# lppllppl920/EndoscopyDepthEstimation-Pytorch

Hardware: AMD Instinct MI355X
Metric: train frame-pairs/sec at 256x320 bs=8 (higher is better)
Workload: dtype f32

## Files before the change

### endoscopydepthestimation-pytorch_amd/csrc/conv_dma_kernels.h

```cpp
#pragma once

#include "conv_kernels.h"

namespace endo {

static __device__ __attribute__((aligned(16))) float g_pad_consts[8] = {__builtin_nanf(""), __builtin_nanf(""), __builtin_nanf(""), __builtin_nanf(""),
                                                                  0.0f, 0.0f, 0.0f, 0.0f};

typedef const __attribute__((address_space(1))) void* gptr_t;
typedef __attribute__((address_space(3))) void* lptr_t;

template <int KS, int KC, int Q, int WX, int R, int NBUF, int VEC, int IN = IN_PLAIN>
struct ConvDmaSmem {
    using G = ConvGeom<KS, KC, WX, R, VEC>;
    static constexpr int kW = KS * KS * KC * 16 * Q;
    static constexpr int kUG = (G::kTileX / 2) * (G::kTileY / 2);
    static constexpr int kUI = kUG / 4;
    static constexpr int kUStride = ((kUG + kUI - 8 + 31) / 32) * 32 + 8;
    static constexpr int kChan = (IN == IN_UNPOOL) ? kUStride : G::kCS;
    static constexpr int kBuf = KC * kChan + kW;
    static constexpr int kTail = 4 * 16 * Q + 8 * 16 * Q;
    static size_t bytes(int bn_cap) { return sizeof(float) * (NBUF * kBuf + 3 * bn_cap + kTail); }
};

template <int KS, int KC, int Q, int IN, int EPI, int WX, int R, int NBUF, int MINW, int VEC, int XF, int EXP = 0, int PH = -1, int BF = 0>
__global__ void __launch_bounds__(kConvThreads, MINW) conv_dma_kernel(const ConvParams p0) {
    static_assert(BF == 0 || (PH < 0 && (KS == 3 || KS == 1) && (IN == IN_BNRELU || IN == IN_PLAIN || (IN == IN_UNPOOL && KS == 1))),
                  "bf16 operands: the ordinary 3x3 convolution and the 1x1 convolutions of the transition-down layers");
    static_assert(PH < 0 || (KS == 3 && (Q % 2) == 0 && IN == IN_PLAIN && EPI == EPI_FWD), "phase mode is the transition-up forward");
    static_assert(IN != IN_UNPOOL || (KS == 1 && R % 2 == 0), "UNPOOL is the transition-down data gradient (1x1)");
    static_assert(NBUF == 1 || NBUF == 2, "one or two LDS buffers");
    static_assert(VEC == 1 || (VEC == 4 && IN != IN_UPSAMPLE && IN != IN_UNPOOL && IN != IN_SUBPIX), "16-byte DMA needs contiguous sources");
    static_assert(IN != IN_SUBPIX || (KS == 3 && EPI == EPI_FWD && PH < 0), "sub-pixel input mode is the transition-up data gradient");
    using G = ConvGeom<KS, KC, WX, R, VEC>;
    using S = ConvDmaSmem<KS, KC, Q, WX, R, NBUF, VEC, IN>;
    constexpr int KK = KS * KS;
    constexpr int NB = 16 * Q;
    constexpr int kWElems = S::kW;
    constexpr int kWPre = (kWElems + kConvThreads - 1) / kConvThreads;
    constexpr bool kDgrad = (EPI == EPI_DGRAD_BN || EPI == EPI_DGRAD_SUMPOOL);
    constexpr int kPhW = 2 * 12 * 16 + 16;
    static_assert(PH < 0 || KC * kPhW <= kWElems, "the phase weights fit the ordinary weight buffer");
    constexpr int kSubW = 4 * 16 * Q + 16;

    extern __shared__ __attribute__((aligned(16))) float smem[];
    float* s_aux = smem + NBUF * S::kBuf;
    int grp, n;
    group_of(p0, blockIdx.z, grp, n);
    const ConvParams p = group_view(p0, grp);
    const int groups = p0.group_n > 0 ? gridDim.z / p0.group_n : 1;
    const bool first_of_group = blockIdx.x == 0 && blockIdx.y == 0 && n == 0;
    (void)groups; (void)first_of_group;
    const int cap = p.bn_cap;

    const int tid = threadIdx.x;
    const int lane = tid & 63;
    const int wave = __builtin_amdgcn_readfirstlane(tid >> 6);
    const int tile = (gridDim.x & 7) == 0 ? xcd_remap(blockIdx.x, gridDim.x) : blockIdx.x;
    const int x0 = (tile % p.tiles_x) * G::kTileX;
    const int y0 = (tile / p.tiles_x) * G::kTileY;
    const int ph = PH == 2 ? static_cast<int>(blockIdx.y) : PH;
    const int co_base = (p.ksplit > 0 || PH == 2) ? 0 : blockIdx.y * NB;

    if constexpr (IN == IN_BNRELU) {
        for (int c = tid; c < p.cin; c += kConvThreads) {
            float scale, mean, beta;
            bn_input_constants(p, p0, grp, groups, first_of_group, c, scale, mean, beta);
            s_aux[c] = scale;
            s_aux[cap + c] = mean;
            s_aux[2 * cap + c] = beta;
        }
        for (int c = p.cin + tid; c < ((p.cin + KC - 1) / KC) * KC; c += kConvThreads) {
            s_aux[c] = 0.f; s_aux[cap + c] = 0.f; s_aux[2 * cap + c] = 0.f;
        }
    }
    if constexpr (EPI == EPI_DGRAD_BN) {
        float* cst = s_aux + 3 * cap;
        if (tid < NB) {
            const int c = co_base + tid;
            float mean = 0.f, rstd = 0.f, scale = 0.f, beta = 0.f;
            if (c < p.cout) {
                mean = p.bn_saved[2 * c];
                rstd = p.bn_saved[2 * c + 1];
                scale = p.bn_gamma[c] * rstd;
                beta = p.bn_beta[c];
            }
            cst[4 * tid] = scale; cst[4 * tid + 1] = beta; cst[4 * tid + 2] = mean; cst[4 * tid + 3] = rstd;
        }
    }

    f32x4 acc[R][Q];
#pragma unroll
    for (int r = 0; r < R; ++r)
#pragma unroll
        for (int q = 0; q < Q; ++q) acc[r][q] = f32x4{0.f, 0.f, 0.f, 0.f};

    const int wx = (wave % WX) * 16;
    const int wy = (wave / WX) * R;
    const int li = lane & 15;
    const int lk = lane >> 4;

    int goff[G::kPos];
    unsigned pos_ok = 0;
#pragma unroll
    for (int k = 0; k < G::kPos; ++k) {
        const int e = tid + k * kConvThreads;
        goff[k] = 0;
        if (e < G::kUnits) {
            const int ry = e / (G::kCols / VEC);
            const int rx = (e - ry * (G::kCols / VEC)) * VEC;
            const int gy = y0 - G::kHalo + ry;
            const int gx = x0 - G::kLeft + rx;
            if (gy >= 0 && gy < p.h && gx >= 0 && gx < p.w) {
                pos_ok |= (1u << k);
                if constexpr (IN == IN_UPSAMPLE) goff[k] = (gy >> 1) * p.in_w + (gx >> 1);
                else if constexpr (IN == IN_SUBPIX) goff[k] = 2 * gy * p.in_w + 2 * gx;
                else goff[k] = gy * p.in_w + gx;
            }
        }
    }
    constexpr int kUSlots = (IN == IN_UNPOOL) ? (KC * S::kUStride + kConvThreads - 1) / kConvThreads : 1;
    int uoff[kUSlots];
    if constexpr (IN == IN_UNPOOL) {
        constexpr int PC = G::kTileX / 2;
        const int ph = p.h >> 1, pw = p.w >> 1;
#pragma unroll
        for (int k = 0; k < kUSlots; ++k) {
            const int e = tid + k * kConvThreads;
            const int u = e % S::kUStride;
            int off = -1;
            if (e < KC * S::kUStride) {
                if (u < S::kUG) {
                    const int gy = (y0 >> 1) + u / PC, gx = (x0 >> 1) + u % PC;
                    if (gy < ph && gx < pw) off = gy * p.in_w + gx;
                } else if (u < S::kUG + S::kUI) {
                    const int q = u - S::kUG;
                    const int gy = (y0 >> 1) + q / (PC / 4), gx = (x0 >> 1) + 4 * (q % (PC / 4));
                    if (gy < ph && gx < pw) off = gy * p.in_w + gx;
                }
            }
            uoff[k] = off;
        }
    }
    const float* in_n = p.in + n * p.in_ns;
    const float* pad_in = g_pad_consts + (IN == IN_BNRELU ? 0 : 4);
    const float* pad_zero = g_pad_consts + 4;
    const int nchunks_all = (p.cin + KC - 1) / KC;
    int chunk_begin = 0, nchunks = nchunks_all;
    ConvParams po = p;
    if (p.ksplit > 0) {
        const int per = (nchunks_all + p.ksplit - 1) / p.ksplit;
        chunk_begin = blockIdx.y * per;
        nchunks = min(nchunks_all, chunk_begin + per);
        po.out = p.out + blockIdx.y * p.split_stride;
    }

    auto issue_dma = [&](int chunk, int buf) {
        const int c_base = chunk * KC;
        float* s_in = smem + buf * S::kBuf;
        float* s_w = s_in + KC * S::kChan;
        if constexpr (IN == IN_UNPOOL) {
            const uint8_t* idx_n = p.in_idx + n * p.idx_ns;
#pragma unroll
            for (int k = 0; k < kUSlots; ++k) {
                const int e0 = k * kConvThreads + wave * 64;
                if (e0 < KC * S::kUStride) {
                    const int e = e0 + lane;
                    const int ch = c_base + e / S::kUStride;
                    const bool is_code = (e % S::kUStride) >= S::kUG;
                    const void* src = pad_zero;
                    if (uoff[k] >= 0 && ch < p.cin) {
                        const int64_t o = static_cast<int64_t>(ch) * p.in_cs + uoff[k];
                        src = is_code ? static_cast<const void*>(idx_n + o) : static_cast<const void*>(in_n + o);
                    }
                    if (e < KC * S::kUStride) __builtin_amdgcn_global_load_lds((gptr_t)src, (lptr_t)(s_in + e0), 4, 0, 0);
                }
            }
        }
        int sub_ph = 0;
        if constexpr (IN == IN_SUBPIX) sub_ph = c_base / p.sub_c;
#pragma unroll
        for (int c = 0; c < (IN == IN_UNPOOL ? 0 : KC); ++c) {
            const int ch = c_base + c;
            const float* plane = in_n + static_cast<int64_t>(ch) * p.in_cs;
            if constexpr (IN == IN_SUBPIX)
                plane = in_n + static_cast<int64_t>(ch - sub_ph * p.sub_c) * p.in_cs + (sub_ph >> 1) * p.in_w + (sub_ph & 1);
#pragma unroll
            for (int k = 0; k < G::kPos; ++k) {
                const int e0 = k * kConvThreads + wave * 64;
                if (e0 < G::kUnits) {
                    const bool ok = (ch < p.cin) && (pos_ok & (1u << k));
                    const float* src = ok ? plane + goff[k] : pad_in;
                    if (e0 + lane < G::kUnits) {
                        if constexpr (VEC == 4)
                            __builtin_amdgcn_global_load_lds((gptr_t)src, (lptr_t)(s_in + c * G::kCS + 4 * e0), 16, 0, 0);
                        else
                            __builtin_amdgcn_global_load_lds((gptr_t)src, (lptr_t)(s_in + c * G::kCS + e0), 4, 0, 0);
                    }
                }
            }
        }
        if constexpr (IN == IN_SUBPIX) {
            constexpr int kUnitsW = KC * kSubW / 4;
            const float* wsrc = p.wgt + static_cast<int64_t>(c_base) * kSubW;
#pragma unroll
            for (int k = 0; k < (kUnitsW + kConvThreads - 1) / kConvThreads; ++k) {
                const int u0 = k * kConvThreads + wave * 64;
                if (u0 < kUnitsW && u0 + lane < kUnitsW)
                    __builtin_amdgcn_global_load_lds((gptr_t)(wsrc + 4 * (u0 + lane)), (lptr_t)(s_w + 4 * u0), 16, 0, 0);
            }
        }
        if constexpr (PH >= 0) {
            constexpr int kUnitsW = KC * kPhW / 4;
            const float* wsrc = p.wgt + static_cast<int64_t>(c_base) * kPhW + (PH == 2 ? static_cast<int64_t>(ph) * p.cin * 400 : 0);
#pragma unroll
            for (int k = 0; k < (kUnitsW + kConvThreads - 1) / kConvThreads; ++k) {
                const int u0 = k * kConvThreads + wave * 64;
                if (u0 < kUnitsW && u0 + lane < kUnitsW)
                    __builtin_amdgcn_global_load_lds((gptr_t)(wsrc + 4 * (u0 + lane)), (lptr_t)(s_w + 4 * u0), 16, 0, 0);
            }
        }
        constexpr bool kChunked = KS == 3 && KC == 16 && Q == 1 && EPI == EPI_FWD && PH < 0 && IN != IN_SUBPIX && BF == 0;
        bool gather = !(PH >= 0 || IN == IN_SUBPIX);
        if constexpr (kChunked) {
            if (p.wgt_chunks) {
                gather = false;
                constexpr int kUnitsW = kWElems / 4;
                const float* wsrc = p.wgt_chunks + static_cast<int64_t>(chunk) * kWElems;
#pragma unroll
                for (int k = 0; k < (kUnitsW + kConvThreads - 1) / kConvThreads; ++k) {
                    const int u0 = k * kConvThreads + wave * 64;
                    if (u0 < kUnitsW && u0 + lane < kUnitsW)
                        __builtin_amdgcn_global_load_lds((gptr_t)(wsrc + 4 * (u0 + lane)), (lptr_t)(s_w + 4 * u0), 16, 0, 0);
                }
            }
        }
        if (gather)
#pragma unroll
        for (int k = 0; k < ((PH >= 0 || IN == IN_SUBPIX) ? 0 : kWPre); ++k) {
            const int e0 = k * kConvThreads + wave * 64;
            if (e0 < kWElems) {
                const int e = e0 + lane;
                const int j = e % NB;
                const int rest = e / NB;
                const int c = rest % KC;
                const int tap = rest / KC;
                const int ci = c_base + c;
                const int co = co_base + j;
                const float* src = pad_zero;
                if (e < kWElems && ci < p.cin && co < (PH >= 0 ? p.w_cout : p.cout)) {
                    if constexpr (kDgrad) src = p.wgt + (static_cast<int64_t>(ci) * p.w_cin + co) * KK + (KK - 1 - tap);
                    else src = p.wgt + (static_cast<int64_t>(co) * p.w_cin + ci) * KK + tap;
                }
                if (e < kWElems) __builtin_amdgcn_global_load_lds((gptr_t)src, (lptr_t)(s_w + e0), 4, 0, 0);
            }
        }
    };

    constexpr int PR = (EPI == EPI_DGRAD_BN) ? R : 1, PQ = (EPI == EPI_DGRAD_BN) ? Q : 1;
    f32x4 xpre[PR][PQ], dpre[PR][PQ];
    bool use_pre = false;
    if constexpr (EPI == EPI_DGRAD_BN) {
        use_pre = ((p.out_w & 3) == 0) && ((p.w & 3) == 0);
        if (use_pre) {
            const int px = x0 + wx + 4 * lk;
#pragma unroll
            for (int q = 0; q < Q; ++q) {
                const int co = co_base + q * 16 + li;
#pragma unroll
                for (int r = 0; r < R; ++r) {
                    const int y = y0 + wy + r;
                    xpre[r][q] = f32x4{0.f, 0.f, 0.f, 0.f};
                    dpre[r][q] = f32x4{0.f, 0.f, 0.f, 0.f};
                    if (co < p.cout && y < p.h && px + 3 < p.w) {
                        xpre[r][q] = *reinterpret_cast<const f32x4*>(p.x + n * p.x_ns + static_cast<int64_t>(co) * p.x_cs + y * p.out_w + px);
                        if (co >= p.acc_from)
                            dpre[r][q] = *reinterpret_cast<const f32x4*>(p.out + n * p.out_ns + static_cast<int64_t>(co) * p.out_cs + y * p.out_w + px);
                    }
                }
            }
        }
    }

    constexpr bool kInPlace = (IN == IN_BNRELU) && (XF == 1);
    auto transform_own = [&](int chunk, int buf) {
        if constexpr (kInPlace) {
            float* s_in = smem + buf * S::kBuf;
#pragma unroll
            for (int c = 0; c < KC; ++c) {
                const int ch = chunk * KC + c;
                const float sc = s_aux[ch], mn = s_aux[cap + ch], bt = s_aux[2 * cap + ch];
#pragma unroll
                for (int k = 0; k < G::kPos; ++k) {
                    const int e = tid + k * kConvThreads;
                    if (e < G::kUnits) {
                        if constexpr (VEC == 4) {
                            f32x4* q = reinterpret_cast<f32x4*>(s_in + c * G::kCS + 4 * e);
                            f32x4 v = *q;
#pragma unroll
                            for (int i = 0; i < 4; ++i) v[i] = __builtin_fmaxf(fmaf(v[i] - mn, sc, bt), 0.f);
                            *q = v;
                        } else {
                            float* q = s_in + c * G::kCS + e;
                            *q = __builtin_fmaxf(fmaf(*q - mn, sc, bt), 0.f);
                        }
                    }
                }
            }
        }
    };

    auto compute = [&](int chunk, int buf) {
        const float* s_in = smem + buf * S::kBuf;
        const float* s_w = s_in + KC * S::kChan;
        int sub_alpha = 0, sub_beta = 0;
        if constexpr (IN == IN_SUBPIX) {
            const int sub_ph = (chunk * KC) / p.sub_c;
            sub_alpha = sub_ph >> 1; sub_beta = sub_ph & 1;
        }
        (void)sub_alpha; (void)sub_beta;
        if constexpr (IN == IN_UNPOOL) {
            constexpr int PC = G::kTileX / 2;
            const int pcol = (wx + li) >> 1;
            const unsigned sh = 8u * (pcol & 3);
            const unsigned want = li & 1;
            if constexpr (BF != 0) {
                constexpr int NQ = KC / 4;
#pragma unroll
                for (int qg = 0; qg < (NQ + 3) / 4; ++qg) {
                    float a[4][R], b[4][Q];
#pragma unroll
                    for (int i = 0; i < 4; ++i) {
                        const int quad = qg * 4 + i;
                        if (quad < NQ) {
                            const float* g_base = s_in + (quad * 4 + lk) * S::kUStride + (wy >> 1) * PC + pcol;
                            const unsigned* i_base = reinterpret_cast<const unsigned*>(s_in + (quad * 4 + lk) * S::kUStride + S::kUG);
                            const float* b_base = s_w + (quad * 4 + lk) * NB + li;
#pragma unroll
                            for (int rr = 0; rr < R / 2; ++rr) {
                                const float g = g_base[rr * PC];
                                const unsigned code = (i_base[(((wy >> 1) + rr) * PC + pcol) >> 2] >> sh) & 0xffu;
                                a[i][2 * rr] = code == want ? g : 0.f;
                                a[i][2 * rr + 1] = code == want + 2u ? g : 0.f;
                            }
#pragma unroll
                            for (int q = 0; q < Q; ++q) b[i][q] = b_base[q * 16];
                        } else {
#pragma unroll
                            for (int r = 0; r < R; ++r) a[i][r] = 0.f;
#pragma unroll
                            for (int q = 0; q < Q; ++q) b[i][q] = 0.f;
                        }
                    }
                    bf16x4_bits ap[R];
#pragma unroll
                    for (int r = 0; r < R; ++r) ap[r] = pack_bf16x4(a[0][r], a[1][r], a[2][r], a[3][r]);
#pragma unroll
                    for (int q = 0; q < Q; ++q) {
                        const bf16x4_bits bp = pack_bf16x4(b[0][q], b[1][q], b[2][q], b[3][q]);
#pragma unroll
                        for (int r = 0; r < R; ++r) acc[r][q] = __builtin_amdgcn_mfma_f32_16x16x16bf16_1k(ap[r], bp, acc[r][q], 0, 0, 0);
                    }
                }
                return;
            }
#pragma unroll
            for (int quad = 0; quad < KC / 4; ++quad) {
                const float* g_base = s_in + (quad * 4 + lk) * S::kUStride + (wy >> 1) * PC + pcol;
                const unsigned* i_base = reinterpret_cast<const unsigned*>(s_in + (quad * 4 + lk) * S::kUStride + S::kUG);
                const float* b_base = s_w + (quad * 4 + lk) * NB + li;
                float a[R];
#pragma unroll
                for (int rr = 0; rr < R / 2; ++rr) {
                    const float g = g_base[rr * PC];
                    const unsigned code = (i_base[(((wy >> 1) + rr) * PC + pcol) >> 2] >> sh) & 0xffu;
                    a[2 * rr] = code == want ? g : 0.f;
                    a[2 * rr + 1] = code == want + 2u ? g : 0.f;
                }
#pragma unroll
                for (int q = 0; q < Q; ++q) {
                    const float b = b_base[q * 16];
#pragma unroll
                    for (int r = 0; r < R; ++r) acc[r][q] = __builtin_amdgcn_mfma_f32_16x16x4f32(a[r], b, acc[r][q], 0, 0, 0);
                }
            }
            return;
        }
        if constexpr (BF != 0 && KS == 1) {
            constexpr int NQ = KC / 4;
#pragma unroll
            for (int qg = 0; qg < (NQ + 3) / 4; ++qg) {
                float a[4][R], b[4][Q];
#pragma unroll
                for (int i = 0; i < 4; ++i) {
                    const int quad = qg * 4 + i;
                    if (quad < NQ) {
                        const float* a_base = s_in + (quad * 4 + lk) * G::kCS + wy * G::kCols + wx + li + G::kColOff;
                        const float* b_base = s_w + (quad * 4 + lk) * NB + li;
                        float sc = 1.f, mn = 0.f, bt = 0.f;
                        if constexpr (IN == IN_BNRELU && !kInPlace) {
                            const int ch = chunk * KC + quad * 4 + lk;
                            sc = s_aux[ch]; mn = s_aux[cap + ch]; bt = s_aux[2 * cap + ch];
                        }
#pragma unroll
                        for (int r = 0; r < R; ++r) {
// ... 67 lines not shown
#pragma unroll
                    for (int r = 0; r < R + KS - 1; ++r) a[r] = a_base[r * G::kCols + dx];
                }
                if constexpr (IN == IN_SUBPIX) {
                    if (dx == (sub_beta == 0 ? 0 : 2)) continue;
                }
#pragma unroll
                for (int dy = 0; dy < KS; ++dy) {
                    if (PH >= 0 && dy == (ph == 0 ? 2 : 0)) continue;
                    if constexpr (IN == IN_SUBPIX) {
                        if (dy == (sub_alpha == 0 ? 0 : 2)) continue;
                    }
#pragma unroll
                    for (int q = 0; q < Q; ++q) {
                        if (PH >= 0 && ((q < Q / 2 && dx == 2) || (q >= Q / 2 && dx == 0))) continue;
                        float b;
                        if constexpr (IN == IN_SUBPIX) {
                            const int tyi = dy - (sub_alpha == 0 ? 1 : 0), txi = dx - (sub_beta == 0 ? 1 : 0);
                            b = s_w[(quad * 4 + lk) * kSubW + (tyi * 2 + txi) * NB + q * 16 + li];
                        } else if constexpr (PH >= 0) {
                            const int slot = dx == 0 ? q : (dx == 1 ? Q / 2 + q : Q / 2 + Q + (q - Q / 2));
                            b = s_w[(quad * 4 + lk) * kPhW + ((dy - ph) * 2 * Q + slot) * 16 + li];
                        } else {
                            b = b_base[(dy * KS + dx) * KC * NB + q * 16];
                        }
#pragma unroll
                        for (int r = 0; r < R; ++r)
                            acc[r][q] = __builtin_amdgcn_mfma_f32_16x16x4f32(a[r + dy], b, acc[r][q], 0, 0, 0);
                    }
                }
            }
        }
    };

    issue_dma(chunk_begin, 0);
    if constexpr (kInPlace) {
        __syncthreads();
        asm volatile("s_waitcnt vmcnt(0)" ::: "memory");
        transform_own(chunk_begin, 0);
        __syncthreads();
        for (int chunk = chunk_begin; chunk < nchunks; ++chunk) {
            const int b = (chunk - chunk_begin) & 1;
            if (chunk + 1 < nchunks) issue_dma(chunk + 1, b ^ 1);
            compute(chunk, b);
            if (chunk + 1 < nchunks) {
                asm volatile("s_waitcnt vmcnt(0)" ::: "memory");
                transform_own(chunk + 1, b ^ 1);
            }
            __syncthreads();
        }
    } else {
        for (int chunk = chunk_begin; chunk < nchunks; ++chunk) {
            const int b = (chunk - chunk_begin) % NBUF;
            if (!(EXP & 4) || chunk == chunk_begin) asm volatile("s_waitcnt vmcnt(0)" ::: "memory");
            __syncthreads();
            if (NBUF == 2 && chunk + 1 < nchunks && !(EXP & 1)) issue_dma(chunk + 1, b ^ 1);
            compute(chunk, b);
            if (NBUF == 1 && chunk + 1 < nchunks) {
                __syncthreads();
                issue_dma(chunk + 1, 0);
            }
        }
    }

    if constexpr (EPI == EPI_DGRAD_BN) {
        if (use_pre) {
            const float* cst = s_aux + 3 * cap;
            float* s_red = s_aux + 3 * cap + 4 * NB;
            const int px = x0 + wx + 4 * lk;
#pragma unroll
            for (int q = 0; q < Q; ++q) {
                const int jloc = q * 16 + li;
                const int co = co_base + jloc;
                const float scale = cst[4 * jloc], beta = cst[4 * jloc + 1], mean = cst[4 * jloc + 2], rstd = cst[4 * jloc + 3];
                float s1 = 0.f, s2 = 0.f;
#pragma unroll
                for (int r = 0; r < R; ++r) {
                    const int y = y0 + wy + r;
                    if (co < p.cout && y < p.h && px + 3 < p.w) {
                        f32x4 o = dpre[r][q];
#pragma unroll
                        for (int e = 0; e < 4; ++e) {
                            const float xc = xpre[r][q][e] - mean;
                            const float z = fmaf(xc, scale, beta);
                            const float dz = z > 0.f ? acc[r][q][e] : 0.f;
                            s1 += dz;
                            s2 += dz * (xc * rstd);
                            o[e] += scale * dz;
                        }
                        *reinterpret_cast<f32x4*>(p.out + n * p.out_ns + static_cast<int64_t>(co) * p.out_cs + y * p.out_w + px) = o;
                    }
                }
                s1 += __shfl_xor(s1, 16, 64); s1 += __shfl_xor(s1, 32, 64);
                s2 += __shfl_xor(s2, 16, 64); s2 += __shfl_xor(s2, 32, 64);
                if (lk == 0) {
                    s_red[((tid >> 6) * NB + jloc) * 2] = s1;
                    s_red[((tid >> 6) * NB + jloc) * 2 + 1] = s2;
                }
            }
            __syncthreads();
            if (tid < 2 * NB) {
                const int j = tid >> 1, which = tid & 1;
                if (co_base + j < p.cout) {
                    double t = 0.0;
                    for (int wv = 0; wv < 4; ++wv) t += static_cast<double>(s_red[(wv * NB + j) * 2 + which]);
                    atomicAdd(p.bn_scratch + bn_slot_offset(p.bn_slot_stride) + 2 * (co_base + j) + which, t);
                }
            }
            return;
        }
    }
    if constexpr (PH >= 0) {
        constexpr int QH = Q / 2;
        float* s_red = s_aux + 3 * cap + 4 * NB;
        const int px = x0 + wx + 4 * lk;
#pragma unroll
        for (int q = 0; q < QH; ++q) {
            const int co = q * 16 + li;
            const bool co_ok = co < p.cout;
            const float bias = (co_ok && p.bias) ? p.bias[co] : 0.f;
            float s1 = 0.f, s2 = 0.f;
#pragma unroll
            for (int r = 0; r < R; ++r) {
                const int y = y0 + wy + r;
                if (co_ok && y < p.h && px + 3 < p.w) {
                    f32x4 lo, hi;
                    lo[0] = acc[r][q][0] + bias; lo[1] = acc[r][q + QH][0] + bias; lo[2] = acc[r][q][1] + bias; lo[3] = acc[r][q + QH][1] + bias;
                    hi[0] = acc[r][q][2] + bias; hi[1] = acc[r][q + QH][2] + bias; hi[2] = acc[r][q][3] + bias; hi[3] = acc[r][q + QH][3] + bias;
                    float* dst = p.out + n * p.out_ns + static_cast<int64_t>(co) * p.out_cs + static_cast<int64_t>(2 * y + ph) * p.out_w + 2 * px;
                    *reinterpret_cast<f32x4*>(dst) = lo;
                    *reinterpret_cast<f32x4*>(dst + 4) = hi;
#pragma unroll
                    for (int e = 0; e < 4; ++e) { s1 += lo[e] + hi[e]; s2 += lo[e] * lo[e] + hi[e] * hi[e]; }
                }
            }
            s1 += __shfl_xor(s1, 16, 64); s1 += __shfl_xor(s1, 32, 64);
            s2 += __shfl_xor(s2, 16, 64); s2 += __shfl_xor(s2, 32, 64);
            if (lk == 0) {
                s_red[((tid >> 6) * NB + q * 16 + li) * 2] = s1;
                s_red[((tid >> 6) * NB + q * 16 + li) * 2 + 1] = s2;
            }
        }
        __syncthreads();
        if (p.out_sums && tid < 2 * 16 * QH) {
            const int j = tid >> 1, which = tid & 1;
            if (j < p.cout) {
                double t = 0.0;
                for (int wv = 0; wv < 4; ++wv) t += static_cast<double>(s_red[(wv * NB + j) * 2 + which]);
                atomicAdd(p.out_sums + 2 * j + which, t);
            }
        }
        return;
    }
    conv_epilogue<Q, EPI, R>(po, acc, s_aux + 3 * cap, s_aux + 3 * cap + 4 * NB, x0, y0, wx, wy, co_base, n);
}

template <int KS, int KC, int Q, int IN, int EPI, int WX, int R, int NBUF, int MINW, int VEC, int XF = 0, int EXP = 0, int PH = -1, int BF = 0>
inline int launch_conv_dma_vec(ConvParams p, hipStream_t stream) {
    static_assert(XF == 0 || NBUF == 2 || IN != IN_BNRELU, "the in-place transform pipeline is written for two buffers");
    using G = ConvGeom<KS, KC, WX, R, VEC>;
    using S = ConvDmaSmem<KS, KC, Q, WX, R, NBUF, VEC, IN>;
    p.tiles_x = (p.w + G::kTileX - 1) / G::kTileX;
    p.bn_cap = (IN == IN_BNRELU) ? ((p.cin + KC - 1) / KC * KC + 15) / 16 * 16 : 0;
    const int tiles_y = (p.h + G::kTileY - 1) / G::kTileY;
    dim3 grid(p.tiles_x * tiles_y, p.ksplit > 0 ? p.ksplit : (PH >= 0 ? (PH == 2 ? 2 : 1) : (p.cout + 16 * Q - 1) / (16 * Q)), p.n);
    return launch_dyn(conv_dma_kernel<KS, KC, Q, IN, EPI, WX, R, NBUF, MINW, VEC, XF, EXP, PH, BF>, grid, kConvThreads, S::bytes(p.bn_cap), stream, p);
}

template <int KS, int KC, int Q, int IN, int EPI, int WX, int R, int NBUF, int MINW = 1, int BF = 0>
inline int launch_conv_dma(const ConvParams& p, hipStream_t stream) {
    if constexpr (IN != IN_UPSAMPLE && IN != IN_UNPOOL) {
        const bool aligned = (p.w % 4 == 0) && (p.in_w % 4 == 0) && (p.in_cs % 4 == 0) && (p.in_ns % 4 == 0) &&
                             (reinterpret_cast<uintptr_t>(p.in) % 16 == 0);
        if (aligned) return launch_conv_dma_vec<KS, KC, Q, IN, EPI, WX, R, NBUF, MINW, 4, 0, 0, -1, BF>(p, stream);
    }
    return launch_conv_dma_vec<KS, KC, Q, IN, EPI, WX, R, NBUF, MINW, 1, 0, 0, -1, BF>(p, stream);
}

template <int KS, int KC, int Q, int IN, int EPI, int BIG_R = 8, int NBUF = 2, int BIG_MINW = 1, int BF = 0>
inline int launch_conv_dma_auto(const ConvParams& p, hipStream_t stream) {
    const long tiles_big = static_cast<long>((p.w + 31) / 32) * ((p.h + 15) / 16) * p.n;
    if (tiles_big >= 512) return launch_conv_dma<KS, KC, Q, IN, EPI, 2, BIG_R, NBUF, BIG_MINW, BF>(p, stream);
    const long tiles_mid = static_cast<long>((p.w + 15) / 16) * ((p.h + 15) / 16) * p.n;
    if (tiles_mid >= 384) return launch_conv_dma<KS, KC, Q, IN, EPI, 1, 4, NBUF, 1, BF>(p, stream);
    constexpr int KCS = (NBUF == 2 && KS == 3 && KC <= 8) ? 16 : KC;
    return launch_conv_dma<KS, KCS, Q, IN, EPI, 1, 2, NBUF, 1, BF>(p, stream);
}

}
```

### endoscopydepthestimation-pytorch_amd/csrc/conv_kernels.h

```cpp
#pragma once

#include "common.h"

namespace endo {

enum InMode { IN_PLAIN = 0, IN_BNRELU = 1, IN_UPSAMPLE = 2, IN_UNPOOL = 3, IN_SUBPIX = 4 };
enum Epilogue { EPI_FWD = 0, EPI_FWD_POOL = 1, EPI_DGRAD_BN = 2, EPI_DGRAD_SUMPOOL = 3 };

constexpr int kConvThreads = 256;
constexpr int kMaxBnChannels = 384;

struct ConvParams {
    int n, h, w;
    int tiles_x;
    const float* in;
    int64_t in_ns;
    int in_cs;
    int in_w;
    const uint8_t* in_idx;
    int64_t idx_ns;
    int cin;
    const double* in_sums;
    const float* gamma;
    const float* beta;
    float* running_mean;
    float* running_var;
    float* saved;
    double count;
    float eps, momentum;
    int training;
    const float* wgt;
    const float* bias;
    int w_cout, w_cin;
    const float* wgt_chunks;
    float* out;
    int64_t out_ns;
    int out_cs, out_w;
    int cout;
    uint8_t* out_idx;
    double* out_sums;
    const float* x;
    int64_t x_ns;
    int x_cs;
    const float* bn_saved;
    const float* bn_gamma;
    const float* bn_beta;
    double* bn_scratch;
    int64_t bn_slot_stride;
    int acc_from;
    int bn_cap;
    int ksplit;
    int64_t split_stride;
    int group_n;
    int64_t gs, in_gs, out_gs;
    int sub_c;
    const float* fin_w;
    float* fin_out;
};

__device__ __forceinline__ void group_of(const ConvParams& p, int z, int& grp, int& n) {
    grp = p.group_n > 0 ? z / p.group_n : 0;
    n = z - grp * p.group_n;
}

__device__ __forceinline__ ConvParams group_view(const ConvParams& p, int grp) {
    ConvParams q = p;
    const int64_t o = grp * p.gs;
    q.in += grp * p.in_gs;
    q.out += grp * p.out_gs;
    if (q.x) q.x += o;
    if (q.in_idx) q.in_idx += 4 * o;
    if (q.out_idx) q.out_idx += 4 * o;
    if (q.in_sums) q.in_sums += o / 2;
    if (q.out_sums) q.out_sums += o / 2;
    if (q.bn_scratch) q.bn_scratch += o / 2;
    if (q.saved) q.saved += o;
    if (q.bn_saved) q.bn_saved += o;
    return q;
}

__device__ __forceinline__ void bn_input_constants(const ConvParams& p, const ConvParams& p0, int grp, int groups, bool first_of_group,
                                                   int c, float& scale, float& mean_f, float& beta) {
    double mean, var;
    if (p.training) {
        mean = p.in_sums[2 * c] / p.count;
        var = p.in_sums[2 * c + 1] / p.count - mean * mean;
        if (var < 0.0) var = 0.0;
    } else {
        mean = p.running_mean[c];
        var = p.running_var[c];
    }
    const double rstd = 1.0 / sqrt(var + static_cast<double>(p.eps));
    scale = p.gamma[c] * static_cast<float>(rstd);
    mean_f = static_cast<float>(mean);
    beta = p.beta[c];
    if (first_of_group) {
        if (p.saved) {
            p.saved[2 * c] = static_cast<float>(mean);
            p.saved[2 * c + 1] = static_cast<float>(rstd);
        }
        if (p.training && grp == 0) {
            float rm = p.running_mean[c], rv = p.running_var[c];
            for (int g = 0; g < groups; ++g) {
                const double* sums = p0.in_sums + g * (p0.gs / 2);
                const double m = sums[2 * c] / p.count;
                double v = sums[2 * c + 1] / p.count - m * m;
                if (v < 0.0) v = 0.0;
                const double unbiased = p.count > 1.0 ? v * p.count / (p.count - 1.0) : v;
                rm = (1.0f - p.momentum) * rm + p.momentum * static_cast<float>(m);
                rv = (1.0f - p.momentum) * rv + p.momentum * static_cast<float>(unbiased);
            }
            p.running_mean[c] = rm;
            p.running_var[c] = rv;
        }
    }
}

typedef float f32x4 __attribute__((ext_vector_type(4)));

template <int KS, int KC, int WX, int R, int VEC = 1>
struct ConvGeom {
    static constexpr int kTileX = 16 * WX;
    static constexpr int kTileY = R * (4 / WX);
    static constexpr int kHalo = KS / 2;
    static constexpr int kRows = kTileY + 2 * kHalo;
    static constexpr int kLeft = (VEC == 4 && KS == 3) ? 4 : kHalo;
    static constexpr int kCols = kTileX + 2 * kLeft;
    static constexpr int kColOff = kLeft - kHalo;
    static constexpr int kPlane = kRows * kCols;
    static constexpr int kCS = ((kPlane - 16 + 31) / 32) * 32 + 16;
    static constexpr int kUnits = kPlane / VEC;
    static constexpr int kPos = (kUnits + kConvThreads - 1) / kConvThreads;
    static constexpr int kPre = KC * kPos;
};

template <int Q, int EPI, int R>
__device__ __forceinline__ void conv_epilogue(const ConvParams& p, f32x4 (&acc)[R][Q], const float* cst, float* s_red,
                                              int x0, int y0, int wx, int wy, int co_base, int n) {
    constexpr int NB = 16 * Q;
    const int tid = threadIdx.x;
    const int lane = tid & 63;
    const int wave = tid >> 6;
    const int li = lane & 15;
    const int lk = lane >> 4;
    (void)cst; (void)s_red; (void)wave;
    const int px = x0 + wx + 4 * lk;
    const bool vec_ok = ((p.out_w & 3) == 0) && ((p.w & 3) == 0);

    if constexpr (EPI == EPI_FWD) {
#pragma unroll
        for (int q = 0; q < Q; ++q) {
            const int co = co_base + q * 16 + li;
            const bool co_ok = co < p.cout;
            const float bias = (co_ok && p.bias) ? p.bias[co] : 0.f;
            float s1 = 0.f, s2 = 0.f;
#pragma unroll
            for (int r = 0; r < R; ++r) {
                const int y = y0 + wy + r;
                f32x4 v = acc[r][q];
                v[0] += bias; v[1] += bias; v[2] += bias; v[3] += bias;
                if (co_ok && y < p.h) {
                    float* dst = p.out + n * p.out_ns + static_cast<int64_t>(co) * p.out_cs + y * p.out_w + px;
                    if (vec_ok && px + 3 < p.w) {
                        *reinterpret_cast<f32x4*>(dst) = v;
#pragma unroll
                        for (int e = 0; e < 4; ++e) { s1 += v[e]; s2 += v[e] * v[e]; }
                    } else {
#pragma unroll
                        for (int e = 0; e < 4; ++e)
                            if (px + e < p.w) { dst[e] = v[e]; s1 += v[e]; s2 += v[e] * v[e]; }
                    }
                }
            }
            if (p.out_sums) {
                s1 += __shfl_xor(s1, 16, 64); s1 += __shfl_xor(s1, 32, 64);
                s2 += __shfl_xor(s2, 16, 64); s2 += __shfl_xor(s2, 32, 64);
                if (lk == 0) {
                    s_red[(wave * NB + q * 16 + li) * 2] = s1;
                    s_red[(wave * NB + q * 16 + li) * 2 + 1] = s2;
                }
            }
        }
        if (p.out_sums) {
            __syncthreads();
            if (tid < 2 * NB) {
                const int j = tid >> 1, which = tid & 1;
                if (co_base + j < p.cout) {
                    double t = 0.0;
                    for (int wv = 0; wv < 4; ++wv) t += static_cast<double>(s_red[(wv * NB + j) * 2 + which]);
                    atomicAdd(p.out_sums + 2 * (co_base + j) + which, t);
                }
            }
        }
    } else if constexpr (EPI == EPI_FWD_POOL) {
        const int ph = p.h >> 1, pw = p.w >> 1;
#pragma unroll
        for (int q = 0; q < Q; ++q) {
            const int co = co_base + q * 16 + li;
            const bool co_ok = co < p.cout;
            const float bias = (co_ok && p.bias) ? p.bias[co] : 0.f;
            float s1 = 0.f, s2 = 0.f;
#pragma unroll
            for (int r = 0; r < R; r += 2) {
                const int yp = (y0 + wy + r) >> 1;
#pragma unroll
                for (int e = 0; e < 4; e += 2) {
                    const int xp = (px + e) >> 1;
                    float best = acc[r][q][e] + bias;
                    int code = 0;
                    float v = acc[r][q][e + 1] + bias;
                    if (v > best) { best = v; code = 1; }
                    v = acc[r + 1][q][e] + bias;
                    if (v > best) { best = v; code = 2; }
                    v = acc[r + 1][q][e + 1] + bias;
                    if (v > best) { best = v; code = 3; }
                    if (co_ok && yp < ph && xp < pw) {
                        const int64_t o = static_cast<int64_t>(co) * p.out_cs + yp * p.out_w + xp;
                        p.out[n * p.out_ns + o] = best;
                        p.out_idx[n * p.idx_ns + o] = static_cast<uint8_t>(code);
                        s1 += best; s2 += best * best;
                    }
                }
            }
            s1 += __shfl_xor(s1, 16, 64); s1 += __shfl_xor(s1, 32, 64);
            s2 += __shfl_xor(s2, 16, 64); s2 += __shfl_xor(s2, 32, 64);
            if (lk == 0) {
                s_red[(wave * NB + q * 16 + li) * 2] = s1;
                s_red[(wave * NB + q * 16 + li) * 2 + 1] = s2;
            }
        }
        __syncthreads();
        if (p.out_sums && tid < 2 * NB) {
            const int j = tid >> 1, which = tid & 1;
            if (co_base + j < p.cout) {
                double t = 0.0;
                for (int wv = 0; wv < 4; ++wv) t += static_cast<double>(s_red[(wv * NB + j) * 2 + which]);
                atomicAdd(p.out_sums + 2 * (co_base + j) + which, t);
            }
        }
    } else if constexpr (EPI == EPI_DGRAD_BN) {
#pragma unroll
        for (int q = 0; q < Q; ++q) {
            const int jloc = q * 16 + li;
            const int co = co_base + jloc;
            const bool co_ok = co < p.cout;
            const float scale = cst[4 * jloc], beta = cst[4 * jloc + 1], mean = cst[4 * jloc + 2], rstd = cst[4 * jloc + 3];
            const bool accumulate = co >= p.acc_from;
            float s1 = 0.f, s2 = 0.f;
#pragma unroll
            for (int r = 0; r < R; ++r) {
                const int y = y0 + wy + r;
                if (co_ok && y < p.h) {
                    const int64_t xo = n * p.x_ns + static_cast<int64_t>(co) * p.x_cs + y * p.out_w + px;
                    float* dst = p.out + n * p.out_ns + static_cast<int64_t>(co) * p.out_cs + y * p.out_w + px;
                    if (vec_ok && px + 3 < p.w) {
                        const f32x4 xv = *reinterpret_cast<const f32x4*>(p.x + xo);
                        f32x4 o = accumulate ? *reinterpret_cast<const f32x4*>(dst) : f32x4{0.f, 0.f, 0.f, 0.f};
#pragma unroll
                        for (int e = 0; e < 4; ++e) {
                            const float xc = xv[e] - mean;
                            const float z = fmaf(xc, scale, beta);
                            const float dz = z > 0.f ? acc[r][q][e] : 0.f;
                            s1 += dz;
                            s2 += dz * (xc * rstd);
                            o[e] += scale * dz;
                        }
                        *reinterpret_cast<f32x4*>(dst) = o;
                    } else {
#pragma unroll
                        for (int e = 0; e < 4; ++e) {
                            if (px + e < p.w) {
                                const float xv = p.x[xo + e];
                                const float xc = xv - mean;
                                const float z = fmaf(xc, scale, beta);
                                const float dz = z > 0.f ? acc[r][q][e] : 0.f;
                                s1 += dz;
                                s2 += dz * (xc * rstd);
                                dst[e] = (accumulate ? dst[e] : 0.f) + scale * dz;
                            }
                        }
                    }
                }
            }
            s1 += __shfl_xor(s1, 16, 64); s1 += __shfl_xor(s1, 32, 64);
            s2 += __shfl_xor(s2, 16, 64); s2 += __shfl_xor(s2, 32, 64);
            if (lk == 0) {
                s_red[(wave * NB + jloc) * 2] = s1;
                s_red[(wave * NB + jloc) * 2 + 1] = s2;
            }
        }
        __syncthreads();
        if (tid < 2 * NB) {
            const int j = tid >> 1, which = tid & 1;
            if (co_base + j < p.cout) {
                double t = 0.0;
                for (int wv = 0; wv < 4; ++wv) t += static_cast<double>(s_red[(wv * NB + j) * 2 + which]);
                atomicAdd(p.bn_scratch + bn_slot_offset(p.bn_slot_stride) + 2 * (co_base + j) + which, t);
            }
        }
    } else {
        const int ph = p.h >> 1, pw = p.w >> 1;
#pragma unroll
        for (int q = 0; q < Q; ++q) {
            const int co = co_base + q * 16 + li;
            if (co >= p.cout) continue;
#pragma unroll
            for (int r = 0; r < R; r += 2) {
                const int yp = (y0 + wy + r) >> 1;
#pragma unroll
                for (int e = 0; e < 4; e += 2) {
                    const int xp = (px + e) >> 1;
                    if (yp < ph && xp < pw) {
                        const float v = (acc[r][q][e] + acc[r][q][e + 1]) + (acc[r + 1][q][e] + acc[r + 1][q][e + 1]);
                        p.out[n * p.out_ns + static_cast<int64_t>(co) * p.out_cs + yp * p.out_w + xp] = v;
                    }
// ... 235 lines not shown
```

### endoscopydepthestimation-pytorch_amd/csrc/net.hip

```cpp
#include <new>
#include <vector>

#include "dgrad_kernels.h"
#include "dgrad_block_kernels.h"
#include "dgrad_newmap_kernels.h"
#include "td_dgrad_kernels.h"
#include "td_fwd_kernels.h"
#include "wgrad_taps_kernels.h"
#include "wgrad1x1_kernels.h"
#include "wgrad_nsplit_kernels.h"
#include "wgrad_x3_kernels.h"
#include "wgrad_f34_kernels.h"
#include "wgrad_subpix_kernels.h"
#include "wino_fwd_kernels.h"
#include "wino4_fwd_kernels.h"
#include "dgrad_wino_kernels.h"
#include "dgrad_wino3_kernels.h"

#include <cstdlib>

namespace endo {

int run_dgrad_wino3_nl4(const DgradBlockParams& p, const float* const* u, hipStream_t stream);
bool dgrad_wino3p_applies(const DgradBlockParams& p);
int run_dgrad_wino3p_nl4(const DgradBlockParams& p, const float* const* u, int blocks, double* fw_parts, int* blocks_used, hipStream_t stream);

constexpr int kGrowth = 12;
constexpr int kLayers = 4;
constexpr int kFirst = 48;
constexpr int kLevels = 5;
constexpr int kNew = kGrowth * kLayers;
constexpr float kBnEps = 1.0e-5f;
constexpr float kBnMomentum = 0.1f;
constexpr int kSideStreamFromLevel = 0;

struct ConvP { int64_t w, b; int cout, cin, ks; int64_t u; int64_t ud; };
struct BnP { int64_t g, b; int c; int64_t run; int64_t saved; };

struct Table {
    ConvP first, final_;
    ConvP down_conv[kLevels][kLayers], td_conv[kLevels], bott_conv[kLayers], tu_conv[kLevels], up_conv[kLevels][kLayers];
    BnP down_bn[kLevels][kLayers], td_bn[kLevels], bott_bn[kLayers], up_bn[kLevels][kLayers];
    std::vector<int64_t> param_offsets;
    std::vector<BnP*> bn_order;
    int64_t param_floats = 0, bn_floats = 0, bn_width_total = 0;
    WinoWeightTable wino;
    WinoWeightTable wino4;
    int64_t wino4_floats = 0;
    int64_t wino_floats = 0;
    WinoDgradTable wino_dgrad;
    int64_t wino_dgrad_floats = 0;
};

inline int down_in(int level) { return kFirst + kNew * level; }
inline int level_channels(int level) { return level < kLevels ? 144 + down_in(level) : 288 + kNew; }

static const Table& table() {
    static Table* t = [] {
        Table* tb = new Table();
        int64_t off = 0;
        auto conv = [&](ConvP& c, int cout, int cin, int ks) {
            c.cout = cout; c.cin = cin; c.ks = ks; c.u = -1; c.ud = -1;
            c.w = off; tb->param_offsets.push_back(off); off += static_cast<int64_t>(cout) * cin * ks * ks;
            c.b = off; tb->param_offsets.push_back(off); off += cout;
        };
        int64_t run = 0, saved = 0;
        auto bn = [&](BnP& b, int c) {
            b.c = c;
            b.g = off; tb->param_offsets.push_back(off); off += c;
            b.b = off; tb->param_offsets.push_back(off); off += c;
            b.run = run; run += 2 * c;
            b.saved = saved; saved += c;
            tb->bn_order.push_back(&b);
        };
        conv(tb->first, kFirst, 3, 3);
        for (int l = 0; l < kLevels; ++l)
            for (int j = 0; j < kLayers; ++j) { bn(tb->down_bn[l][j], down_in(l) + kGrowth * j); conv(tb->down_conv[l][j], kGrowth, down_in(l) + kGrowth * j, 3); }
        for (int l = 0; l < kLevels; ++l) { bn(tb->td_bn[l], down_in(l) + kNew); conv(tb->td_conv[l], down_in(l) + kNew, down_in(l) + kNew, 1); }
        for (int j = 0; j < kLayers; ++j) { bn(tb->bott_bn[j], 288 + kGrowth * j); conv(tb->bott_conv[j], kGrowth, 288 + kGrowth * j, 3); }
        for (int i = 0; i < kLevels; ++i) conv(tb->tu_conv[i], kNew, kNew, 3);
        for (int i = 0; i < kLevels; ++i) {
            const int l = kLevels - 1 - i;
            for (int j = 0; j < kLayers; ++j) { const int cin = 96 + down_in(l) + kGrowth * j; bn(tb->up_bn[i][j], cin); conv(tb->up_conv[i][j], kGrowth, cin, 3); }
        }
        conv(tb->final_, 1, 192, 1);
        tb->param_floats = off;
        tb->bn_floats = run;
        tb->bn_width_total = saved;
        {
            WinoWeightTable& wt = tb->wino;
            wt.layers = 0; wt.start[0] = 0;
            int64_t uoff = 0;
            auto add = [&](ConvP& c) {
                const int l = wt.layers++;
                c.u = uoff;
                wt.cin[l] = c.cin; wt.cout[l] = c.cout; wt.w_off[l] = c.w; wt.u_off[l] = uoff;
                wt.start[l + 1] = wt.start[l] + c.cin * 16;
                uoff += static_cast<int64_t>(c.cin) * kWinoUStride;
            };
            for (int l = 0; l < kLevels; ++l) for (int j = 0; j < kLayers; ++j) add(tb->down_conv[l][j]);
            for (int j = 0; j < kLayers; ++j) add(tb->bott_conv[j]);
            for (int i = 0; i < kLevels; ++i) for (int j = 0; j < kLayers; ++j) add(tb->up_conv[i][j]);
            tb->wino_floats = uoff;
            tb->wino4 = wt;
            int64_t u4 = 0;
            for (int l = 0; l < wt.layers; ++l) { tb->wino4.u_off[l] = u4; u4 += static_cast<int64_t>(wt.cin[l]) * kW4UStride; }
            tb->wino4_floats = u4;
        }
        {
            WinoDgradTable& wd = tb->wino_dgrad;
            wd.layers = 0; wd.start[0] = 0;
            int64_t uoff = 0;
            auto add = [&](ConvP& c, int base) {
                const int l = wd.layers++;
                c.ud = uoff;
                wd.cin[l] = c.cin; wd.groups[l] = base / 16; wd.w_off[l] = c.w; wd.u_off[l] = uoff;
                wd.start[l + 1] = wd.start[l] + 16 * wd.groups[l] * 12;
                uoff += static_cast<int64_t>(wd.groups[l]) * kWinoDgradSlice;
            };
            for (int l = 0; l < kLevels; ++l) for (int j = 0; j < kLayers; ++j) add(tb->down_conv[l][j], down_in(l));
            for (int j = 0; j < kLayers; ++j) add(tb->bott_conv[j], 288);
            for (int i = 0; i < kLevels; ++i) for (int j = 0; j < kLayers; ++j) add(tb->up_conv[i][j], 96 + down_in(kLevels - 1 - i));
            tb->wino_dgrad_floats = uoff;
        }
        return tb;
    }();
    return *t;
}

}

using namespace endo;

struct endo_net {
    int n, h, w;
    int groups;
    int64_t gs;
    struct Level { int h, w, t; int64_t plane; int64_t act, grad; int64_t sums; int64_t pq; } lv[kLevels + 1];
    int64_t pre_off;
    int64_t saved_off;
    int64_t idx_off[kLevels];
    int64_t sums_off;
    int64_t sums_bytes;
    int64_t tape_floats;
    int64_t partial_off;
    int64_t wino_off;
    int64_t wino4_off;
    int64_t pq_off;
    int64_t pq_floats;
    int64_t scratch_off;
    int64_t scratch_bytes;
    int64_t slot_stride;
    int64_t wg_scratch_off;
    int64_t tuw_scratch_off;
    int64_t wd_off;
    int64_t gplane_off;
    int64_t bias_parts_off;
    int64_t fw_parts_off;
    int64_t bias_parts_floats;
    int64_t gradws_floats;
    hipStream_t wstream;
    hipEvent_t ev_fork, ev_join;
    int opt[ENDO_OPT_COUNT];
};

namespace endo {


constexpr int kBiasPartChannels = 2048;
constexpr int kBiasPartLaunches = 64;
constexpr int kFwPartBlocks = 512;
struct BiasReduceTable {
    int n;
    struct Entry { const float* parts; float* bias; int count; int nparts; } e[kBiasPartLaunches];
};
struct BiasParts {
    BiasReduceTable table;
    int64_t used;
};

struct BnFin4 {
    const double* scratch[4];
    const float* saved[4];
    const float* gamma[4];
    float* ggamma[4];
    float* gbeta[4];
};

__global__ void __launch_bounds__(256) prep_dy_kernel(float* __restrict__ dbuf, const float* __restrict__ x, int64_t ns, int plane,
                                                      const float* __restrict__ pq_p, const float* __restrict__ pq_q,
                                                      float* bias_grad, int group_n, int64_t gs, const BnFin4 fin, int nl,
                                                      double count, int training, int64_t slot_stride,
                                                      const float* __restrict__ vg, const float* __restrict__ vw, float* __restrict__ parts) {
    __shared__ double scratch[4];
    const int c = blockIdx.y;
    const int grp = blockIdx.z / group_n, n = blockIdx.z - grp * group_n;
    float pc = pq_p[grp * gs + c], qc = pq_q[grp * gs + c];
    if (nl > 0) {
        const int64_t go = grp * gs;
        double dp = 0.0, dq = 0.0;
#pragma unroll
        for (int j = 0; j < 4; ++j) {
            if (j >= nl) break;
            const double s1 = bn_slot_sum(fin.scratch[j] + go / 2 + 2 * c, slot_stride);
            const double s2 = bn_slot_sum(fin.scratch[j] + go / 2 + 2 * c + 1, slot_stride);
            if (blockIdx.x == 0 && n == 0 && threadIdx.x == 0) {
                atomicAdd(fin.ggamma[j] + c, static_cast<float>(s2));
                atomicAdd(fin.gbeta[j] + c, static_cast<float>(s1));
            }
            if (training) {
                const double mean = fin.saved[j][go + 2 * c], rstd = fin.saved[j][go + 2 * c + 1];
                const double scale = fin.gamma[j][c] * rstd;
                const double k = scale * rstd * s2 / count;
                dp += static_cast<double>(static_cast<float>(-k));
                dq += static_cast<double>(static_cast<float>(-scale * s1 / count + k * mean));
            }
        }
        pc += static_cast<float>(dp);
        qc += static_cast<float>(dq);
    }
    const int64_t base = grp * gs + n * ns + static_cast<int64_t>(c) * plane;
    const float* vg_n = vg ? vg + grp * gs + static_cast<int64_t>(n) * plane : nullptr;
    const float wf = vg ? vw[c] : 0.f;
    float part = 0.f;
    if ((plane & 3) == 0 && !vg_n) {
        const int stride = gridDim.x * blockDim.x * 4;
        int i = (blockIdx.x * blockDim.x + threadIdx.x) * 4;
        for (; i + stride < plane; i += 2 * stride) {
            f32x4 g0 = *reinterpret_cast<const f32x4*>(dbuf + base + i);
            f32x4 g1 = *reinterpret_cast<const f32x4*>(dbuf + base + i + stride);
            const f32x4 x0 = *reinterpret_cast<const f32x4*>(x + base + i);
            const f32x4 x1 = *reinterpret_cast<const f32x4*>(x + base + i + stride);
#pragma unroll
            for (int e = 0; e < 4; ++e) { g0[e] += fmaf(pc, x0[e], qc); part += g0[e]; }
#pragma unroll
            for (int e = 0; e < 4; ++e) { g1[e] += fmaf(pc, x1[e], qc); part += g1[e]; }
            *reinterpret_cast<f32x4*>(dbuf + base + i) = g0;
            *reinterpret_cast<f32x4*>(dbuf + base + i + stride) = g1;
        }
        for (; i < plane; i += stride) {
            f32x4 g = *reinterpret_cast<const f32x4*>(dbuf + base + i);
            const f32x4 xv = *reinterpret_cast<const f32x4*>(x + base + i);
#pragma unroll
            for (int e = 0; e < 4; ++e) { g[e] += fmaf(pc, xv[e], qc); part += g[e]; }
            *reinterpret_cast<f32x4*>(dbuf + base + i) = g;
        }
    } else if ((plane & 3) == 0) {
        for (int i = (blockIdx.x * blockDim.x + threadIdx.x) * 4; i < plane; i += gridDim.x * blockDim.x * 4) {
            f32x4 g;
            if (vg_n) {
                const f32x4 gv = *reinterpret_cast<const f32x4*>(vg_n + i);
                g = f32x4{gv[0] * wf, gv[1] * wf, gv[2] * wf, gv[3] * wf};
            } else {
                g = *reinterpret_cast<const f32x4*>(dbuf + base + i);
            }
            const f32x4 xv = *reinterpret_cast<const f32x4*>(x + base + i);
#pragma unroll
            for (int e = 0; e < 4; ++e) { g[e] += fmaf(pc, xv[e], qc); part += g[e]; }
            *reinterpret_cast<f32x4*>(dbuf + base + i) = g;
        }
    } else {
        for (int i = blockIdx.x * blockDim.x + threadIdx.x; i < plane; i += gridDim.x * blockDim.x) {
            const float g = (vg_n ? vg_n[i] * wf : dbuf[base + i]) + fmaf(pc, x[base + i], qc);
            dbuf[base + i] = g;
            part += g;
        }
    }
    const int lane = threadIdx.x & 63, wave = threadIdx.x >> 6;
    double v = wave_sum(static_cast<double>(part));
    if (lane == 0) scratch[wave] = v;
    __syncthreads();
    if (threadIdx.x == 0 && bias_grad) {
        const float t = static_cast<float>(scratch[0] + scratch[1] + scratch[2] + scratch[3]);
        if (parts) parts[(static_cast<int64_t>(c) * gridDim.z + blockIdx.z) * gridDim.x + blockIdx.x] = t;
        else atomicAdd(bias_grad + c, t);
    }
}

__global__ void __launch_bounds__(256) bias_reduce_kernel(const BiasReduceTable tb) {
    const BiasReduceTable::Entry& e = tb.e[blockIdx.x];
    const int lane = threadIdx.x & 63, wave = threadIdx.x >> 6;
    for (int c = blockIdx.y * 4 + wave; c < e.count; c += gridDim.y * 4) {
        const float* src = e.parts + static_cast<int64_t>(c) * e.nparts;
        double t = 0.0;
        for (int i = lane; i < e.nparts; i += 64) t += static_cast<double>(src[i]);
        t = wave_sum(t);
        if (lane == 0) e.bias[c] += static_cast<float>(t);
    }
}

__global__ void bn_bwd_finalize_kernel(const double* __restrict__ scratch, const float* __restrict__ saved,
                                       const float* __restrict__ gamma, float* __restrict__ ggamma, float* __restrict__ gbeta,
                                       float* __restrict__ pq_p, float* __restrict__ pq_q, int c_count, double count, int training,
                                       int64_t gs, int64_t slot_stride) {
    scratch += blockIdx.y * (gs / 2); saved += blockIdx.y * gs; pq_p += blockIdx.y * gs; pq_q += blockIdx.y * gs;
    for (int c = blockIdx.x * blockDim.x + threadIdx.x; c < c_count; c += gridDim.x * blockDim.x) {
        const double s1 = bn_slot_sum(scratch + 2 * c, slot_stride), s2 = bn_slot_sum(scratch + 2 * c + 1, slot_stride);
        atomicAdd(ggamma + c, static_cast<float>(s2));
        atomicAdd(gbeta + c, static_cast<float>(s1));
        if (training) {
            const double mean = saved[2 * c], rstd = saved[2 * c + 1];
            const double scale = gamma[c] * rstd;
            const double k = scale * rstd * s2 / count;
            pq_p[c] += static_cast<float>(-k);
            pq_q[c] += static_cast<float>(-scale * s1 / count + k * mean);
        }
    }
}

__global__ void bn_bwd_finalize4_kernel(const BnFin4 a, int nl, float* __restrict__ pq_p, float* __restrict__ pq_q, int c_count, double count,
                                        int training, int64_t gs, int64_t slot_stride) {
    const int64_t go = blockIdx.y * gs;
    pq_p += go; pq_q += go;
    for (int c = blockIdx.x * blockDim.x + threadIdx.x; c < c_count; c += gridDim.x * blockDim.x) {
        double dp = 0.0, dq = 0.0;
// ... 70 lines not shown
                                                               int group_n, int64_t gs) {
    __shared__ double scratch[2 * 4];
    const int c = blockIdx.y;
    const int grp = blockIdx.z / group_n, n = blockIdx.z - grp * group_n;
    partial += grp * gs; out += grp * gs;
    if (out_sums) out_sums += grp * (gs / 2);
    const float b = bias[c];
    float part[2] = {0.f, 0.f};
    for (int i = blockIdx.x * blockDim.x + threadIdx.x; i < plane; i += gridDim.x * blockDim.x) {
        float v = b;
        for (int s = 0; s < ksplit; ++s) v += partial[s * split_stride + n * pns + static_cast<int64_t>(c) * plane + i];
        out[n * out_ns + static_cast<int64_t>(c) * plane + i] = v;
        part[0] += v;
        part[1] += v * v;
    }
    if (out_sums) block_sum_atomic<2>(part, out_sums + 2 * c, scratch);
}

__global__ void __launch_bounds__(256) final_fwd_kernel(const float* __restrict__ u, int64_t ns, int plane, int cin,
                                                        const float* __restrict__ wgt, const float* __restrict__ bias,
                                                        float* __restrict__ pre, float* __restrict__ out, int group_n, int64_t gs, int c_first) {
    __shared__ float s_w[192];
    for (int c = threadIdx.x; c < cin; c += blockDim.x) s_w[c] = wgt[c];
    __syncthreads();
    const int grp = blockIdx.y / group_n, n = blockIdx.y - grp * group_n;
    u += grp * gs;
    if (pre) pre += grp * gs;
    out += static_cast<int64_t>(grp) * group_n * plane;
    const bool vec = (plane & 3) == 0;
    if (vec) {
        for (int i = (blockIdx.x * blockDim.x + threadIdx.x) * 4; i < plane; i += gridDim.x * blockDim.x * 4) {
            f32x4 acc = {0.f, 0.f, 0.f, 0.f};
            if (c_first > 0) acc = *reinterpret_cast<const f32x4*>(pre + static_cast<int64_t>(n) * plane + i);
            const float* src = u + n * ns + i;
            for (int c = c_first; c < cin; ++c) {
                const f32x4 v = *reinterpret_cast<const f32x4*>(src + static_cast<int64_t>(c) * plane);
                const float wc = s_w[c];
                acc[0] = fmaf(v[0], wc, acc[0]); acc[1] = fmaf(v[1], wc, acc[1]);
                acc[2] = fmaf(v[2], wc, acc[2]); acc[3] = fmaf(v[3], wc, acc[3]);
            }
            const float b = bias[0];
            f32x4 o;
            for (int e = 0; e < 4; ++e) { acc[e] += b; o[e] = fabsf(acc[e]); }
            if (pre) *reinterpret_cast<f32x4*>(pre + static_cast<int64_t>(n) * plane + i) = acc;
            *reinterpret_cast<f32x4*>(out + static_cast<int64_t>(n) * plane + i) = o;
        }
    } else {
        for (int i = blockIdx.x * blockDim.x + threadIdx.x; i < plane; i += gridDim.x * blockDim.x) {
            float acc = c_first > 0 ? pre[static_cast<int64_t>(n) * plane + i] : 0.f;
            for (int c = c_first; c < cin; ++c) acc = fmaf(u[n * ns + static_cast<int64_t>(c) * plane + i], s_w[c], acc);
            acc += bias[0];
            if (pre) pre[static_cast<int64_t>(n) * plane + i] = acc;
            out[static_cast<int64_t>(n) * plane + i] = fabsf(acc);
        }
    }
}

__device__ __forceinline__ float sign_of(float v) { return v > 0.f ? 1.f : (v < 0.f ? -1.f : 0.f); }

__global__ void __launch_bounds__(256) final_g_kernel(const float* __restrict__ gout, const float* __restrict__ pre, float* __restrict__ g,
                                                      int plane, int group_n, int64_t gs) {
    const int grp = blockIdx.y / group_n, n = blockIdx.y - grp * group_n;
    gout += static_cast<int64_t>(blockIdx.y) * plane; pre += grp * gs + static_cast<int64_t>(n) * plane; g += grp * gs + static_cast<int64_t>(n) * plane;
    for (int i = blockIdx.x * blockDim.x + threadIdx.x; i < plane; i += gridDim.x * blockDim.x) g[i] = gout[i] * sign_of(pre[i]);
}

__global__ void __launch_bounds__(256) final_bwd_data_kernel(const float* __restrict__ gout, const float* __restrict__ pre,
                                                             const float* __restrict__ wgt, float* __restrict__ dbuf,
                                                             int64_t ns, int plane, int cin, int group_n, int64_t gs, int c_first) {
    __shared__ float s_w[192];
    for (int c = threadIdx.x; c < cin; c += blockDim.x) s_w[c] = wgt[c];
    __syncthreads();
    const int grp = blockIdx.y / group_n, n = blockIdx.y - grp * group_n;
    gout += static_cast<int64_t>(grp) * group_n * plane; pre += grp * gs; dbuf += grp * gs;
    for (int i = blockIdx.x * blockDim.x + threadIdx.x; i < plane; i += gridDim.x * blockDim.x) {
        const float g = gout[static_cast<int64_t>(n) * plane + i] * sign_of(pre[static_cast<int64_t>(n) * plane + i]);
        for (int c = c_first; c < cin; ++c) dbuf[n * ns + static_cast<int64_t>(c) * plane + i] = g * s_w[c];
    }
}

__global__ void __launch_bounds__(256) final_bwd_weight_kernel(const float* __restrict__ gout, const float* __restrict__ pre,
                                                               const float* __restrict__ u, int64_t ns, int plane, int cin,
                                                               int group_n, int64_t gs, float* __restrict__ gw, float* __restrict__ gb, int c_first) {
    __shared__ double scratch[4];
    const int c = c_first + blockIdx.x;
    const int grp = blockIdx.z / group_n, n = blockIdx.z - grp * group_n;
    const float* gp = gout + static_cast<int64_t>(blockIdx.z) * plane;
    const float* pp = pre + grp * gs + static_cast<int64_t>(n) * plane;
    const float* up = u + grp * gs + n * ns + static_cast<int64_t>(c < cin ? c : 0) * plane;
    float part = 0.f, part2 = 0.f;
    if ((plane & 3) == 0) {
        const int stride = gridDim.y * blockDim.x * 4;
        for (int i = (blockIdx.y * blockDim.x + threadIdx.x) * 4; i < plane; i += stride) {
            const f32x4 gv = *reinterpret_cast<const f32x4*>(gp + i);
            const f32x4 pv = *reinterpret_cast<const f32x4*>(pp + i);
            f32x4 uv = {1.f, 1.f, 1.f, 1.f};
            if (c < cin) uv = *reinterpret_cast<const f32x4*>(up + i);
            part += gv[0] * sign_of(pv[0]) * uv[0] + gv[1] * sign_of(pv[1]) * uv[1];
            part2 += gv[2] * sign_of(pv[2]) * uv[2] + gv[3] * sign_of(pv[3]) * uv[3];
        }
    } else {
        for (int i = blockIdx.y * blockDim.x + threadIdx.x; i < plane; i += gridDim.y * blockDim.x)
            part += gp[i] * sign_of(pp[i]) * (c < cin ? up[i] : 1.f);
    }
    const int lane = threadIdx.x & 63, wave = threadIdx.x >> 6;
    double v = wave_sum(static_cast<double>(part + part2));
    if (lane == 0) scratch[wave] = v;
    __syncthreads();
    if (threadIdx.x == 0) {
        const float t = static_cast<float>(scratch[0] + scratch[1] + scratch[2] + scratch[3]);
        if (c < cin) atomicAdd(gw + c, t); else atomicAdd(gb, t);
    }
}

__global__ void __launch_bounds__(64) final_w_reduce_kernel(const double* __restrict__ parts, int nblocks, int count, float* __restrict__ gw) {
    const int c = blockIdx.x;
    double t = 0.0;
    for (int b = threadIdx.x; b < nblocks; b += 64) t += parts[static_cast<int64_t>(b) * count + c];
    t = wave_sum(t);
    if (threadIdx.x == 0) atomicAdd(gw + c, static_cast<float>(t));
}

struct Ctx {
    const endo_net* net;
    const float* params;
    float* bn_running;
    float* tape;
    float* grads;
    float* gradws;
    int training;
    hipStream_t stream;
    BiasParts* bias_parts = nullptr;

    int nt() const { return net->n * net->groups; }
    int fork_wgrad(Ctx& side, int level) const {
        side = *this;
        if (!net->wstream || !net->opt[ENDO_OPT_WGRAD_OVERLAP] || level < kSideStreamFromLevel) return 0;
        ENDO_CHECK(hipEventRecord(net->ev_fork, stream));
        ENDO_CHECK(hipStreamWaitEvent(net->wstream, net->ev_fork, 0));
        side.stream = net->wstream;
        return 0;
    }
    float* act(int level) const { return tape + net->lv[level].act; }
    float* gbuf(int level) const { return gradws + net->lv[level].grad; }
    double* sums(int level) const { return reinterpret_cast<double*>(reinterpret_cast<char*>(tape) + net->sums_off) + net->lv[level].sums; }
    double* out_sums(int level, int channel) const { return training ? sums(level) + 2 * channel : nullptr; }
    float* saved(const BnP& b) const { return tape + net->saved_off + 2 * b.saved; }
    double* scratch(const BnP& b) const { return reinterpret_cast<double*>(reinterpret_cast<char*>(gradws) + net->scratch_off) + 2 * b.saved; }
    float* pq_p(int level) const { return gradws + net->pq_off + 2 * net->lv[level].pq; }
    float* pq_q(int level) const { return pq_p(level) + net->lv[level].t; }
    uint8_t* idx(int level) const { return reinterpret_cast<uint8_t*>(tape) + net->idx_off[level]; }
};

static void fill_bn_in(const Ctx& c, ConvParams& p, const BnP& b, int level, int ic0) {
    const auto& lv = c.net->lv[level];
    p.in_sums = c.sums(level) + 2 * ic0;
    p.gamma = c.params + b.g;
    p.beta = c.params + b.b;
    p.running_mean = c.bn_running + b.run;
    p.running_var = c.bn_running + b.run + b.c;
    p.saved = c.tape ? c.saved(b) : nullptr;
    p.count = static_cast<double>(c.net->n) * lv.h * lv.w;
    p.eps = kBnEps;
    p.momentum = kBnMomentum;
    p.training = c.training;
}

static void fill_in(const Ctx& c, ConvParams& p, const float* base, int level, int ic0, int cin) {
    const auto& lv = c.net->lv[level];
    p.in = base + ic0 * lv.plane;
    p.in_ns = lv.t * lv.plane;
    p.in_cs = static_cast<int>(lv.plane);
    p.in_w = lv.w;
    p.cin = cin;
}

static void fill_out(const Ctx& c, ConvParams& p, float* base, int level, int oc0, int cout) {
    const auto& lv = c.net->lv[level];
    p.out = base + oc0 * lv.plane;
    p.out_ns = lv.t * lv.plane;
    p.out_cs = static_cast<int>(lv.plane);
    p.out_w = lv.w;
    p.cout = cout;
}

static void fill_grid(const Ctx& c, ConvParams& p, int level) {
    const auto& lv = c.net->lv[level];
    p.n = c.nt(); p.h = lv.h; p.w = lv.w;
    p.group_n = c.net->n; p.gs = c.net->gs; p.in_gs = c.net->gs; p.out_gs = c.net->gs;
}

static double conv_flops(const endo_net* net, int level, int cin, int cout, int ks) {
    return 2.0 * net->n * net->groups * net->lv[level].plane * cin * cout * ks * ks;
}

static void default_options(int (&opt)[ENDO_OPT_COUNT]) {
    opt[ENDO_OPT_WINO_FWD] = 5;
    opt[ENDO_OPT_WINO_DGRAD] = 3;
    opt[ENDO_OPT_DGRAD_VEC] = 2;
    opt[ENDO_OPT_WINO_MIN_TILES] = 1024;
    opt[ENDO_OPT_MFMA_BF16] = 0;
    opt[ENDO_OPT_WGRAD_OVERLAP] = 1;
    opt[ENDO_OPT_MFMA_X3] = 0;
    opt[ENDO_OPT_WGRAD_F34] = 1;
    opt[ENDO_OPT_FINAL_VIRTUAL] = 1;
    opt[ENDO_OPT_TD_PERSIST] = 3;
}
static int wino_fwd_mode(const Ctx& c) { return c.net->opt[ENDO_OPT_WINO_FWD]; }
static bool wino_fwd_enabled(const Ctx& c) { return wino_fwd_mode(c) != 0; }
static int wino_dgrad_mode(const Ctx& c) { return c.net->opt[ENDO_OPT_WINO_DGRAD]; }
static bool wino_dgrad_enabled(const Ctx& c) { return wino_dgrad_mode(c) != 0; }
static bool dgrad_vec_enabled(const Ctx& c) { return c.net->opt[ENDO_OPT_DGRAD_VEC] != 0; }
static int mfma_bf16_mask(const Ctx& c) { const int v = c.net->opt[ENDO_OPT_MFMA_BF16]; return v == 1 ? 7 : (v >> 1); }
static bool mfma_bf16_wgrad(const Ctx& c) { return (mfma_bf16_mask(c) & 1) != 0; }
static int wgrad_mfma_mode(const Ctx& c) { return mfma_bf16_wgrad(c) ? 1 : ((c.net->opt[ENDO_OPT_MFMA_X3] & 1) ? 2 : 0); }
static bool mfma_bf16_fwd(const Ctx& c) { return (mfma_bf16_mask(c) & 2) != 0; }
static bool mfma_bf16_dgrad(const Ctx& c) { return (mfma_bf16_mask(c) & 4) != 0; }

static bool dense_fwd_wino4_tiles(const Ctx& c, int level) {
    const auto& lv = c.net->lv[level];
    const long t4 = static_cast<long>((lv.w + 63) / 64) * ((lv.h + 15) / 16) * c.nt();
    return wino_fwd_mode(c) == 5 && !mfma_bf16_fwd(c) && 2 * t4 >= c.net->opt[ENDO_OPT_WINO_MIN_TILES];
}
static bool dense_fwd_wino2_tiles(const Ctx& c, int level) {
    const auto& lv = c.net->lv[level];
    const long t16 = static_cast<long>((lv.w + 31) / 32) * ((lv.h + 15) / 16) * c.nt();
    const long t8 = static_cast<long>((lv.w + 31) / 32) * ((lv.h + 7) / 8) * c.nt();
    const long min_tiles = c.net->opt[ENDO_OPT_WINO_MIN_TILES];
    return wino_fwd_enabled(c) && !mfma_bf16_fwd(c) && (t16 >= min_tiles || t8 >= (min_tiles * 3) / 4);
}
static bool dense_fwd_chunk_weights(const Ctx& c, int level) {
    return !mfma_bf16_fwd(c) && !dense_fwd_wino4_tiles(c, level) && !dense_fwd_wino2_tiles(c, level);
}

static int dense_fwd(const Ctx& c, int level, int ic0, int oc0, const BnP& b, const ConvP& cv, const float* fin_w = nullptr, float* fin_pre = nullptr,
                     bool* fused_final = nullptr) {
    const auto& lv = c.net->lv[level];
    ConvParams p{};
    fill_grid(c, p, level);
    fill_in(c, p, c.act(level), level, ic0, cv.cin);
    fill_bn_in(c, p, b, level, ic0);
    p.wgt = c.params + cv.w; p.bias = c.params + cv.b; p.w_cout = cv.cout; p.w_cin = cv.cin;
    fill_out(c, p, c.act(level), level, oc0, cv.cout);
    p.out_sums = c.out_sums(level, oc0);
    ProfScope prof(kProfConv3x3Dense, c.stream, conv_flops(c.net, level, cv.cin, cv.cout, 3),
                   4.0 * c.nt() * lv.plane * (cv.cin + cv.cout));
    if (cv.u >= 0 && dense_fwd_wino4_tiles(c, level)) {
        ConvParams p4 = p;
        p4.wgt = c.tape + c.net->wino4_off + cv.u / kWinoUStride * kW4UStride;
        if (wino4_fwd_ok(p4)) {
            if (fin_w && fused_final && c.net->opt[ENDO_OPT_FINAL_VIRTUAL]) { p4.fin_w = fin_w + ic0; p4.fin_out = fin_pre; *fused_final = true; }
            return launch_wino4_fwd(p4, c.stream);
        }
    }
    if (cv.u >= 0 && dense_fwd_wino2_tiles(c, level)) {
        ConvParams pw = p;
        pw.wgt = c.tape + c.net->wino_off + cv.u;
        const long t16 = static_cast<long>((lv.w + 31) / 32) * ((lv.h + 15) / 16) * c.nt();
        const long t8 = static_cast<long>((lv.w + 31) / 32) * ((lv.h + 7) / 8) * c.nt();
        if (wino_fwd_ok(pw)) {
            const int mode = wino_fwd_mode(c);
            const long min_tiles = c.net->opt[ENDO_OPT_WINO_MIN_TILES];
            const bool big = t16 >= min_tiles, small = t8 >= (min_tiles * 3) / 4;
            if (mode == 4) {
                if (big) return launch_wino_fwd<2, 4, 2, 4>(pw, c.stream);
                if (small) return launch_wino_fwd<1, 4, 3, 4>(pw, c.stream);
            }
            if (mode == 3) {
                if (big) return launch_wino_fwd<2, 4, 2, 3>(pw, c.stream);
                if (small) return launch_wino_fwd<1, 4, 3, 3>(pw, c.stream);
            }
#ifdef ENDO_WINO_DIAG
            if (big) {
                static const int exp = [] { const char* e = std::getenv("ENDO_WINO_EXP"); return e ? std::atoi(e) : 0; }();
                switch (exp) {
                    case 14: return launch_wino_fwd<2, 4, 2, 2, 14>(pw, c.stream);
                    case 30: return launch_wino_fwd<2, 4, 2, 2, 30>(pw, c.stream);
                    case 31: return launch_wino_fwd<2, 4, 2, 2, 31>(pw, c.stream);
                    case 63: return launch_wino_fwd<2, 4, 2, 2, 63>(pw, c.stream);
                    case 64: return launch_wino_fwd<2, 4, 2, 2, 64>(pw, c.stream);
                    default: break;
                }
            }
#endif
            if (big) return launch_wino_fwd<2, 4, 2, 2>(pw, c.stream);
            if (small) return launch_wino_fwd<1, 4, 3, 2>(pw, c.stream);
        }
    }
    const long tiles_big = static_cast<long>((lv.w + 31) / 32) * ((lv.h + 15) / 16) * c.nt();
    const long tiles_mid = static_cast<long>((lv.w + 15) / 16) * ((lv.h + 15) / 16) * c.nt();
    const long tiles_small = static_cast<long>((lv.w + 15) / 16) * ((lv.h + 7) / 8) * c.nt();
    const int nchunks = (cv.cin + 15) / 16;
    const float* chunk_weights = (cv.u >= 0 && dense_fwd_chunk_weights(c, level)) ? c.tape + c.net->wino_off + cv.u : nullptr;
    if (tiles_big < 512 && tiles_mid < 384 && tiles_small < 512 && nchunks >= 4) {
        int want = static_cast<int>(((tiles_small < 256 ? 512 : 768) + tiles_small - 1) / tiles_small);
        if (want > nchunks) want = nchunks;
        const int per = (nchunks + want - 1) / want;
        const int ksplit = (nchunks + per - 1) / per;
        float* partial = c.tape + c.net->partial_off;
        p.ksplit = ksplit;
        p.split_stride = static_cast<int64_t>(c.net->n) * cv.cout * lv.plane;
        p.out = partial; p.out_ns = static_cast<int64_t>(cv.cout) * lv.plane;
        p.bias = nullptr; p.out_sums = nullptr;
        p.wgt_chunks = chunk_weights;
        int rc = mfma_bf16_fwd(c) ? launch_conv_dma<3, 16, 1, IN_BNRELU, EPI_FWD, 1, 2, 2, 1, 1>(p, c.stream)
                             : launch_conv_dma<3, 16, 1, IN_BNRELU, EPI_FWD, 1, 2, 2, 1>(p, c.stream);
        if (rc) return rc;
        int bx = static_cast<int>((lv.plane + 255) / 256);
        bx = bx > 8 ? 8 : bx;
        finalize_partial_kernel<<<dim3(bx, cv.cout, c.nt()), 256, 0, c.stream>>>(
            partial, p.split_stride, ksplit, p.out_ns, static_cast<int>(lv.plane), c.params + cv.b, c.act(level) + oc0 * lv.plane,
            lv.t * lv.plane, c.out_sums(level, oc0), c.net->n, c.net->gs);
        ENDO_LAUNCH_CHECK();
        return 0;
    }
    const long tiles_wide = static_cast<long>((lv.w + 31) / 32) * ((lv.h + 7) / 8) * c.nt();
    if (mfma_bf16_fwd(c)) {
        if (tiles_big < 1024 && tiles_wide >= 1024) return launch_conv_dma<3, 4, 1, IN_BNRELU, EPI_FWD, 2, 4, 2, 1, 1>(p, c.stream);
        if (tiles_big < 1024 && tiles_small >= 768) return launch_conv_dma<3, 8, 1, IN_BNRELU, EPI_FWD, 1, 2, 2, 1, 1>(p, c.stream);
        return launch_conv_dma_auto<3, 4, 1, IN_BNRELU, EPI_FWD, 8, 2, 1, 1>(p, c.stream);
    }
    if (tiles_big < 1024 && tiles_wide >= 1024) return launch_conv_dma<3, 4, 1, IN_BNRELU, EPI_FWD, 2, 4, 2, 1>(p, c.stream);
    if (tiles_big < 1024 && tiles_small >= 768) return launch_conv_dma<3, 8, 1, IN_BNRELU, EPI_FWD, 1, 2, 2, 1>(p, c.stream);
    p.wgt_chunks = chunk_weights;
    return launch_conv_dma_auto<3, 4, 1, IN_BNRELU, EPI_FWD, 8, 2, 1>(p, c.stream);
}

static int td_fwd(const Ctx& c, int level, const BnP& b, const ConvP& cv) {
    const int next = level + 1;
    const int oc0 = next < kLevels ? 48 : 0;
    ConvParams p{};
    fill_grid(c, p, level);
    fill_in(c, p, c.act(level), level, 48, cv.cin);
    fill_bn_in(c, p, b, level, 48);
    p.wgt = c.params + cv.w; p.bias = c.params + cv.b; p.w_cout = cv.cout; p.w_cin = cv.cin;
    fill_out(c, p, c.act(next), next, oc0, cv.cout);
    p.out_idx = c.idx(level);
    p.idx_ns = static_cast<int64_t>(cv.cout) * c.net->lv[next].plane;
    p.out_sums = c.out_sums(next, oc0);
    ProfScope prof(kProfConv1x1Pool, c.stream, conv_flops(c.net, level, cv.cin, cv.cout, 1),
                   4.0 * c.nt() * c.net->lv[level].plane * (cv.cin + cv.cout / 4.0));
    if ((c.net->opt[ENDO_OPT_TD_PERSIST] & 2) && !mfma_bf16_fwd(c) && c.training && td_fwd_ok(p)) return launch_td_fwd(p, device_cu_count(), c.stream);
    if (mfma_bf16_fwd(c)) return launch_conv_dma_auto<1, 8, 3, IN_BNRELU, EPI_FWD_POOL, 4, 2, 1, 1>(p, c.stream);
    return launch_conv_dma_auto<1, 8, 3, IN_BNRELU, EPI_FWD_POOL, 4>(p, c.stream);
}

static int tu_fwd(const Ctx& c, int level, int src_level, int src_c0, const ConvP& cv) {
    const auto& sv = c.net->lv[src_level];
    ProfScope prof(kProfConv3x3Up, c.stream, conv_flops(c.net, level, cv.cin, cv.cout, 3),
                   4.0 * c.nt() * c.net->lv[level].plane * (cv.cin / 4.0 + cv.cout));
    if (sv.w % 4 == 0 && cv.cout == kNew && cv.cin % 4 == 0) {
        float* w3 = c.tape + c.net->partial_off;
        tu_phase_weights_kernel<<<(2 * cv.cin * 384 + 255) / 256, 256, 0, c.stream>>>(c.params + cv.w, cv.cout, cv.cin, w3);
        ENDO_LAUNCH_CHECK();
        {
            ConvParams p{};
            fill_grid(c, p, src_level);
            fill_in(c, p, c.act(src_level), src_level, src_c0, cv.cin);
            p.wgt = w3; p.w_cout = 2 * cv.cout; p.w_cin = cv.cin;
            p.bias = c.params + cv.b;
            fill_out(c, p, c.act(level), level, 0, cv.cout);
            p.out_sums = c.out_sums(level, 0);
            return launch_conv_dma_vec<3, 4, 6, IN_PLAIN, EPI_FWD, 2, 4, 2, 1, 4, 0, 0, 2>(p, c.stream);
        }
    }
    ConvParams p{};
    fill_grid(c, p, level);
    fill_in(c, p, c.act(src_level), src_level, src_c0, cv.cin);
    p.wgt = c.params + cv.w; p.bias = c.params + cv.b; p.w_cout = cv.cout; p.w_cin = cv.cin;
    fill_out(c, p, c.act(level), level, 0, cv.cout);
    p.out_sums = c.out_sums(level, 0);
    return launch_conv_dma_auto<3, 4, 3, IN_UPSAMPLE, EPI_FWD>(p, c.stream);
}

struct FinalVirt { const float* vg; const float* vw; bool base; bool base_w; float* gw; };

static int prep_dy(const Ctx& c, int level, int c0, int count, float* bias_grad, const BnFin4* fin = nullptr, int nl = 0, const FinalVirt* fv = nullptr) {
    const auto& lv = c.net->lv[level];
    BnFin4 none{};
    int bx = static_cast<int>((lv.plane + 4095) / 4096);
    bx = bx < 1 ? 1 : (bx > 32 ? 32 : bx);
    float* parts = nullptr;
    if (bias_grad && c.bias_parts) {
        BiasParts& bp = *c.bias_parts;
        const int64_t need = static_cast<int64_t>(count) * c.nt() * bx;
        if (bp.table.n >= kBiasPartLaunches || bp.used + need > c.net->bias_parts_floats) return ENDO_E_UNSUPPORTED;
        parts = c.gradws + c.net->bias_parts_off + bp.used;
        bp.table.e[bp.table.n++] = {parts, bias_grad, count, c.nt() * bx};
        bp.used += need;
    }
    ProfScope prof(kProfSmall, c.stream, 0.0, 12.0 * c.nt() * lv.plane * count);
    prep_dy_kernel<<<dim3(bx, count, c.nt()), 256, 0, c.stream>>>(c.gbuf(level) + c0 * lv.plane, c.act(level) + c0 * lv.plane,
                                                                     lv.t * lv.plane, static_cast<int>(lv.plane), c.pq_p(level) + c0,
                                                                     c.pq_q(level) + c0, bias_grad, c.net->n, c.net->gs, fin ? *fin : none, fin ? nl : 0,
                                                                     static_cast<double>(c.net->n) * lv.h * lv.w, c.training, c.net->slot_stride,
                                                                     fv ? fv->vg : nullptr, fv ? fv->vw + c0 : nullptr, parts);
    ENDO_LAUNCH_CHECK();
    return 0;
}

static int bn_finalize(const Ctx& c, const BnP& b, int level, int ic0, int first = 0, int count = -1) {
    const auto& lv = c.net->lv[level];
    if (count < 0) count = b.c - first;
    if (count <= 0) return 0;
    ProfScope prof(kProfSmall, c.stream, 0.0, 0.0);
    bn_bwd_finalize_kernel<<<dim3((count + 127) / 128, c.net->groups), 128, 0, c.stream>>>(c.scratch(b) + 2 * first, c.saved(b) + 2 * first, c.params + b.g + first,
                                                                       c.grads + b.g + first, c.grads + b.b + first,
                                                                       c.pq_p(level) + ic0 + first, c.pq_q(level) + ic0 + first, count,
                                                                       static_cast<double>(c.net->n) * lv.h * lv.w, c.training, c.net->gs, c.net->slot_stride);
    ENDO_LAUNCH_CHECK();
    return 0;
}

static void fill_wgrad_grid(const Ctx& c, WgradParams& p, int level) {
    const auto& lv = c.net->lv[level];
    p.n = c.nt(); p.h = lv.h; p.w = lv.w;
    p.group_n = c.net->n; p.gs = c.net->gs; p.in_gs = c.net->gs;
    p.tiles_x = (lv.w + kWgTileX - 1) / kWgTileX;
    p.tiles_y = (lv.h + kWgTileY - 1) / kWgTileY;
}

static int dense_wgrad(const Ctx& c, int level, int ic0, int oc0, const BnP& b, const ConvP& cv, F34ReduceBatch* batch = nullptr, int slice = 0) {
    const auto& lv = c.net->lv[level];
    WgradParams p{};
    fill_wgrad_grid(c, p, level);
    p.in = c.act(level) + ic0 * lv.plane; p.in_ns = lv.t * lv.plane; p.in_cs = static_cast<int>(lv.plane); p.in_w = lv.w; p.cin = cv.cin;
    p.saved = c.saved(b); p.gamma = c.params + b.g; p.beta = c.params + b.b;
    p.dy = c.gbuf(level) + oc0 * lv.plane; p.dy_ns = lv.t * lv.plane; p.dy_cs = static_cast<int>(lv.plane); p.dy_w = lv.w; p.cout = cv.cout;
    p.dw = c.grads + cv.w;
    ProfScope prof(kProfWgradDense, c.stream, conv_flops(c.net, level, cv.cin, cv.cout, 3), 4.0 * c.nt() * lv.plane * (cv.cin + cv.cout));
    if (c.net->opt[ENDO_OPT_WGRAD_F34] && wgrad_mfma_mode(c) == 0 && wgrad_f34_ok(p, c.net->opt[ENDO_OPT_WINO_MIN_TILES] / 4l))
        return launch_wgrad_f34(p, c.gradws + c.net->wg_scratch_off + (batch ? slice : 0) * kF34ScratchFloats, c.stream,
                                c.net->opt[ENDO_OPT_WGRAD_F34] == 2 ? 256 : kF34Blocks, batch);
    if (wgrad_nsplit_ok(p)) {
        if (wgrad_mfma_mode(c) == 2) return launch_wgrad_x3(p, c.gradws + c.net->wg_scratch_off, c.stream);
        return launch_wgrad_nsplit(p, c.gradws + c.net->wg_scratch_off, c.stream, wgrad_mfma_mode(c));
    }
    if (wgrad_taps_ok(p)) return mfma_bf16_wgrad(c) ? launch_wgrad_taps<12, IN_BNRELU, 1>(p, c.stream) : launch_wgrad_taps<12, IN_BNRELU>(p, c.stream);
    return launch_wgrad<3, 1, IN_BNRELU, DY_PLAIN>(p, c.stream);
}

static int dense_bwd(const Ctx& c, int level, int ic0, int oc0, const BnP& b, const ConvP& cv, int acc_from) {
    const auto& lv = c.net->lv[level];
    int rc = prep_dy(c, level, oc0, cv.cout, c.grads + cv.b);
    if (rc) return rc;
    {
        Ctx cw;
        rc = c.fork_wgrad(cw, level);
        if (rc) return rc;
        rc = dense_wgrad(cw, level, ic0, oc0, b, cv);
        if (rc) return rc;
    }
    {
        ConvParams p{};
        fill_grid(c, p, level);
        fill_in(c, p, c.gbuf(level), level, oc0, cv.cout);
        p.wgt = c.params + cv.w; p.w_cout = cv.cout; p.w_cin = cv.cin;
        fill_out(c, p, c.gbuf(level), level, ic0, cv.cin);
        p.x = c.act(level) + ic0 * lv.plane; p.x_ns = lv.t * lv.plane; p.x_cs = static_cast<int>(lv.plane);
        p.bn_saved = c.saved(b); p.bn_gamma = c.params + b.g; p.bn_beta = c.params + b.b;
        p.bn_scratch = c.scratch(b); p.bn_slot_stride = c.net->slot_stride;
        p.acc_from = acc_from - ic0;
        ProfScope prof(kProfDgradDense, c.stream, conv_flops(c.net, level, cv.cin, cv.cout, 3), 4.0 * c.nt() * lv.plane * (3.0 * cv.cin + cv.cout));
        rc = launch_dgrad_dense_auto(p, c.stream);
        if (rc) return rc;
    }
    return bn_finalize(c, b, level, ic0);
}

static int base_pass_form(const Ctx& c, int level, const DgradBlockParams& p, const ConvP* cv) {
    const auto& lv = c.net->lv[level];
    const long wtiles = static_cast<long>(lv.w / 32) * (lv.h / 8) * c.nt();
    if (mfma_bf16_dgrad(c)) return 0;
    if (wino_dgrad_enabled(c) && dgrad_wino_ok(p) && wtiles >= c.net->opt[ENDO_OPT_WINO_MIN_TILES] && cv[0].ud >= 0)
        return ((wino_dgrad_mode(c) == 1 || wino_dgrad_mode(c) == 3) && dgrad_wino3_ok(p)) ? 1 : 2;
    return 0;
}
// ... 98 lines not shown
        }
        ProfScope prof(kProfDgradDense, c.stream, 2.0 * c.nt() * lv.plane * c0 * kGrowth * 9 * kLayers,
                       4.0 * c.nt() * lv.plane * (3.0 * c0 + kGrowth * kLayers));
        int rc;
        const int form = base_pass_form(c, level, p, cv);
        if (fv && fv->base) {
            if (form != 1) return ENDO_E_BADARG;
            p.vg = fv->vg; p.vw = fv->vw + ic0;
        }
        if (mfma_bf16_dgrad(c)) {
            rc = launch_dgrad_block8<4, 1>(p, c.stream);
        } else if (form != 0) {
            const float* ub = c.gradws + c.net->wd_off;
            const float* const u[4] = {ub + cv[0].ud, ub + cv[1].ud, ub + cv[2].ud, ub + cv[3].ud};
            if (form == 1 && wino_dgrad_mode(c) == 3 && dgrad_wino3p_applies(p)) {
                double* fwp = (fv && fv->base && fv->base_w) ? reinterpret_cast<double*>(c.gradws + c.net->fw_parts_off) : nullptr;
                int used = 0;
                rc = run_dgrad_wino3p_nl4(p, u, std::min(device_cu_count(), kFwPartBlocks), fwp, &used, c.stream);
                if (rc == 0 && fwp) {
                    final_w_reduce_kernel<<<c0, 64, 0, c.stream>>>(fwp, used, c0, fv->gw + ic0);
                    ENDO_LAUNCH_CHECK();
                }
            } else {
                if (fv && fv->base && fv->base_w) return ENDO_E_BADARG;
                rc = form == 1 ? run_dgrad_wino3_nl4(p, u, c.stream) : launch_dgrad_wino8<4>(p, u, c.stream);
            }
        } else {
            rc = launch_dgrad_block8<4>(p, c.stream);
        }
        if (rc) return rc;
    }
    {
        BnFin4 a;
        for (int j = 0; j < kLayers; ++j) {
            a.scratch[j] = c.scratch(bn[j]); a.saved[j] = c.saved(bn[j]); a.gamma[j] = c.params + bn[j].g;
            a.ggamma[j] = c.grads + bn[j].g; a.gbeta[j] = c.grads + bn[j].b;
        }
        ProfScope prof(kProfSmall, c.stream, 0.0, 0.0);
        bn_bwd_finalize4_kernel<<<dim3((c0 + 127) / 128, c.net->groups), 128, 0, c.stream>>>(a, kLayers, c.pq_p(level) + ic0, c.pq_q(level) + ic0, c0,
                                                                         static_cast<double>(c.net->n) * lv.h * lv.w, c.training, c.net->gs,
                                                                         c.net->slot_stride);
        ENDO_LAUNCH_CHECK();
    }
    return 0;
}

static int td_bwd(const Ctx& c, int level, const BnP& b, const ConvP& cv) {
    const int next = level + 1;
    const int oc0 = next < kLevels ? 48 : 0;
    const auto& lv = c.net->lv[level];
    const auto& nx = c.net->lv[next];
    int rc = prep_dy(c, next, oc0, cv.cout, c.grads + cv.b);
    if (rc) return rc;
    {
        WgradParams p{};
        fill_wgrad_grid(c, p, level);
        p.in = c.act(level) + 48 * lv.plane; p.in_ns = lv.t * lv.plane; p.in_cs = static_cast<int>(lv.plane); p.in_w = lv.w; p.cin = cv.cin;
        p.saved = c.saved(b); p.gamma = c.params + b.g; p.beta = c.params + b.b;
        p.dy = c.gbuf(next) + oc0 * nx.plane; p.dy_ns = nx.t * nx.plane; p.dy_cs = static_cast<int>(nx.plane); p.dy_w = nx.w; p.cout = cv.cout;
        p.dy_idx = c.idx(level); p.idx_ns = static_cast<int64_t>(cv.cout) * nx.plane;
        p.dw = c.grads + cv.w;
        Ctx cw;
        rc = c.fork_wgrad(cw, level);
        if (rc) return rc;
        ProfScope prof(kProfWgradOther, cw.stream, conv_flops(c.net, level, cv.cin, cv.cout, 1), 4.0 * c.nt() * lv.plane * cv.cin);
        rc = wgrad1x1_dma_ok(p) ? (mfma_bf16_wgrad(c) ? launch_wgrad1x1_dma<1>(p, cw.stream) : launch_wgrad1x1_dma<0>(p, cw.stream))
                                : launch_wgrad1x1(p, cw.stream);
        if (rc) return rc;
    }
    {
        ConvParams p{};
        fill_grid(c, p, level);
        fill_in(c, p, c.gbuf(next), next, oc0, cv.cout);
        p.in_idx = c.idx(level); p.idx_ns = static_cast<int64_t>(cv.cout) * nx.plane;
        p.wgt = c.params + cv.w; p.w_cout = cv.cout; p.w_cin = cv.cin;
        fill_out(c, p, c.gbuf(level), level, 48, cv.cin);
        p.x = c.act(level) + 48 * lv.plane; p.x_ns = lv.t * lv.plane; p.x_cs = static_cast<int>(lv.plane);
        p.bn_saved = c.saved(b); p.bn_gamma = c.params + b.g; p.bn_beta = c.params + b.b;
        p.bn_scratch = c.scratch(b); p.bn_slot_stride = c.net->slot_stride;
        p.acc_from = 0;
        ProfScope prof(kProfDgradOther, c.stream, conv_flops(c.net, level, cv.cin, cv.cout, 1), 4.0 * c.nt() * lv.plane * 3.0 * cv.cin);
        if ((c.net->opt[ENDO_OPT_TD_PERSIST] & 1) && !mfma_bf16_dgrad(c) && td_dgrad_ok(p))
            rc = launch_td_dgrad(p, device_cu_count(), c.stream);
        else if ((c.net->opt[ENDO_OPT_TD_PERSIST] & 1) && !mfma_bf16_dgrad(c) && nx.w % 4 != 0 && td_dgrad_small_ok(p))
            rc = launch_td_dgrad_small(p, c.stream);
        else
        rc = (nx.w % 4 == 0) ? (mfma_bf16_dgrad(c) ? launch_conv_dma_auto<1, 16, 2, IN_UNPOOL, EPI_DGRAD_BN, 4, 2, 1, 1>(p, c.stream)
                                                  : launch_conv_dma_auto<1, 16, 2, IN_UNPOOL, EPI_DGRAD_BN, 4>(p, c.stream))
                             : launch_conv_auto<1, 16, 3, IN_UNPOOL, EPI_DGRAD_BN, 4>(p, c.stream);
        if (rc) return rc;
    }
    return bn_finalize(c, b, level, 48);
}

static int tu_bwd(const Ctx& c, int level, int src_level, int src_c0, const ConvP& cv) {
    const auto& lv = c.net->lv[level];
    const auto& sv = c.net->lv[src_level];
    int rc = prep_dy(c, level, 0, cv.cout, c.grads + cv.b);
    if (rc) return rc;
    {
        WgradParams p{};
        fill_wgrad_grid(c, p, level);
        p.in = c.act(src_level) + src_c0 * sv.plane; p.in_ns = sv.t * sv.plane; p.in_cs = static_cast<int>(sv.plane); p.in_w = sv.w; p.cin = cv.cin;
        p.dy = c.gbuf(level); p.dy_ns = lv.t * lv.plane; p.dy_cs = static_cast<int>(lv.plane); p.dy_w = lv.w; p.cout = cv.cout;
        p.dw = c.grads + cv.w;
        Ctx cw;
        rc = c.fork_wgrad(cw, level);
        if (rc) return rc;
        ProfScope prof(kProfWgradOther, cw.stream, conv_flops(c.net, level, cv.cin, cv.cout, 3), 4.0 * c.nt() * lv.plane * (cv.cin / 4.0 + cv.cout));
        WgradParams ps = p;
        ps.h = sv.h; ps.w = sv.w;
        if (tu_wgrad_subpix_ok(ps)) rc = launch_tu_wgrad_subpix(ps, c.gradws + c.net->wg_scratch_off, cw.stream);
        else rc = wgrad_taps_ok(p, true) ? launch_wgrad_taps<12, IN_UPSAMPLE>(p, cw.stream) : launch_wgrad<3, 1, IN_UPSAMPLE, DY_PLAIN>(p, cw.stream);
        if (rc) return rc;
    }
    ProfScope prof(kProfDgradOther, c.stream, conv_flops(c.net, level, cv.cin, cv.cout, 3), 4.0 * c.nt() * lv.plane * (cv.cout + cv.cin / 4.0));
    if (sv.w % 4 == 0 && cv.cin == kNew && cv.cout == kNew) {
        float* wd = c.gradws + c.net->tuw_scratch_off;
        tu_subpix_dgrad_weights_kernel<<<(16 * cv.cout * cv.cin + 255) / 256, 256, 0, c.stream>>>(c.params + cv.w, cv.cout, cv.cin, wd);
        ENDO_LAUNCH_CHECK();
        ConvParams p{};
        fill_grid(c, p, src_level);
        fill_in(c, p, c.gbuf(level), level, 0, 4 * cv.cout);
        p.sub_c = cv.cout;
        p.wgt = wd; p.w_cout = cv.cin; p.w_cin = 4 * cv.cout;
        fill_out(c, p, c.gbuf(src_level), src_level, src_c0, cv.cin);
        const long t32 = static_cast<long>((sv.w + 31) / 32) * ((sv.h + 7) / 8) * c.nt();
        const long t16 = static_cast<long>((sv.w + 15) / 16) * ((sv.h + 7) / 8) * c.nt();
        if (t32 >= 1024) return launch_conv_dma_vec<3, 8, 3, IN_SUBPIX, EPI_FWD, 2, 4, 2, 1, 1>(p, c.stream);
        if (t16 >= 512) return launch_conv_dma_vec<3, 8, 3, IN_SUBPIX, EPI_FWD, 1, 2, 2, 1, 1>(p, c.stream);
        return launch_conv_dma_vec<3, 8, 3, IN_SUBPIX, EPI_FWD, 1, 1, 2, 1, 1>(p, c.stream);
    }
    ConvParams p{};
    fill_grid(c, p, level);
    fill_in(c, p, c.gbuf(level), level, 0, cv.cout);
    p.wgt = c.params + cv.w; p.w_cout = cv.cout; p.w_cin = cv.cin;
    fill_out(c, p, c.gbuf(src_level), src_level, src_c0, cv.cin);
    return launch_conv_dma_auto<3, 4, 3, IN_PLAIN, EPI_DGRAD_SUMPOOL, 4>(p, c.stream);
}

static int64_t align_up(int64_t v, int64_t a) { return (v + a - 1) / a * a; }

}

extern "C" int endo_net_create_grouped(endo_net** out, int n, int h, int w, int groups) {
    if (!out || n <= 0 || h <= 0 || w <= 0 || groups <= 0) return ENDO_E_BADARG;
    if (groups > kMaxGroups) return ENDO_E_UNSUPPORTED;
    if ((h % 32) != 0 || (w % 32) != 0) return ENDO_E_UNSUPPORTED;
    const Table& tb = table();
    endo_net* net = new (std::nothrow) endo_net();
    if (!net) return ENDO_E_BADARG;
    net->n = n; net->h = h; net->w = w; net->groups = groups;
    net->wstream = nullptr; net->ev_fork = nullptr; net->ev_join = nullptr;
    default_options(net->opt);
    int64_t off = 0, sums = 0, pq = 0;
    for (int l = 0; l <= kLevels; ++l) {
        auto& lv = net->lv[l];
        lv.h = h >> l; lv.w = w >> l; lv.t = level_channels(l);
        lv.plane = static_cast<int64_t>(lv.h) * lv.w;
        lv.act = off; lv.grad = off;
        off += align_up(static_cast<int64_t>(n) * lv.t * lv.plane, 64);
        lv.sums = sums; sums += 2 * lv.t;
        lv.pq = pq; pq += lv.t;
    }
    const int64_t acts = off;
    net->pre_off = off; off += align_up(static_cast<int64_t>(n) * h * w, 64);
    net->saved_off = off; off += align_up(2 * tb.bn_width_total, 64);
    int64_t byte_off = off * 4;
    for (int l = 0; l < kLevels; ++l) {
        net->idx_off[l] = byte_off;
        byte_off += align_up(static_cast<int64_t>(n) * (down_in(l) + kNew) * net->lv[l + 1].plane, 256);
    }
    net->sums_off = byte_off;
    net->sums_bytes = sums * 8;
    byte_off += align_up(net->sums_bytes, 256);
    net->partial_off = byte_off / 4;
    byte_off += static_cast<int64_t>(kGrowth) * 163840 * 4;
    net->wino_off = byte_off / 4;
    byte_off += align_up(tb.wino_floats * 4, 256);
    net->wino4_off = byte_off / 4;
    byte_off += align_up(tb.wino4_floats * 4, 256);
    net->tape_floats = byte_off / 4;
    net->pq_off = acts;
    net->pq_floats = 2 * pq;
    net->scratch_off = align_up((acts + net->pq_floats) * 4, 256);
    net->slot_stride = align_up(tb.bn_width_total * 2, 32);
    net->scratch_bytes = net->slot_stride * 8 * kBnSlots;
    net->wg_scratch_off = (net->scratch_off + align_up(net->scratch_bytes, 256)) / 4;
    net->tuw_scratch_off = net->wg_scratch_off + std::max(std::max(kNsScratchFloats, kSpScratchFloats), 4 * kF34ScratchFloats);
    net->wd_off = align_up(net->tuw_scratch_off + 4 * kNew * (4 * kNew + 16), 64);
    net->gplane_off = align_up(net->wd_off + tb.wino_dgrad_floats, 64);
    net->bias_parts_off = net->gplane_off + align_up(static_cast<int64_t>(n) * h * w, 64);
    net->bias_parts_floats = static_cast<int64_t>(kBiasPartChannels) * n * groups * 32;
    {
        int launches = 1, channels = tb.first.cout;
        for (int l = 0; l < kLevels; ++l) {
            for (int j = 0; j < kLayers; ++j) { launches += 2; channels += tb.down_conv[l][j].cout + tb.up_conv[l][j].cout; }
            launches += 2; channels += tb.td_conv[l].cout + tb.tu_conv[l].cout;
        }
        for (int j = 0; j < kLayers; ++j) { ++launches; channels += tb.bott_conv[j].cout; }
        if (launches > kBiasPartLaunches || channels > kBiasPartChannels) { delete net; return ENDO_E_UNSUPPORTED; }
    }
    net->fw_parts_off = net->bias_parts_off + align_up(net->bias_parts_floats, 64);
    net->gradws_floats = net->fw_parts_off + 2 * static_cast<int64_t>(kFwPartBlocks) * 192;
    net->gs = align_up(net->tape_floats > net->gradws_floats ? net->tape_floats : net->gradws_floats, 64);
    *out = net;
    return 0;
}

extern "C" int endo_net_create(endo_net** out, int n, int h, int w) { return endo_net_create_grouped(out, n, h, w, 1); }

extern "C" int endo_net_set_option(endo_net* net, int option_id, int value) {
    if (!net || option_id < 0 || option_id >= ENDO_OPT_COUNT) return ENDO_E_BADARG;
    const int old = net->opt[option_id];
    net->opt[option_id] = value;
    return old;
}

extern "C" int endo_net_get_option(const endo_net* net, int option_id) {
    if (!net || option_id < 0 || option_id >= ENDO_OPT_COUNT) return ENDO_E_BADARG;
    return net->opt[option_id];
}

extern "C" void endo_net_destroy(endo_net* net) {
    if (!net) return;
    if (net->ev_fork) (void)hipEventDestroy(net->ev_fork);
    if (net->ev_join) (void)hipEventDestroy(net->ev_join);
    if (net->wstream) (void)hipStreamDestroy(net->wstream);
    delete net;
}
extern "C" int64_t endo_net_param_floats(void) { return table().param_floats; }
extern "C" int64_t endo_net_bn_floats(void) { return table().bn_floats; }
extern "C" int64_t endo_net_tape_floats(const endo_net* net) { return !net ? 0 : (net->groups > 1 ? net->groups * net->gs : net->tape_floats); }
extern "C" int64_t endo_net_gradws_floats(const endo_net* net) { return !net ? 0 : (net->groups > 1 ? net->groups * net->gs : net->gradws_floats); }
extern "C" int endo_net_groups(const endo_net* net) { return net ? net->groups : 0; }
extern "C" int64_t endo_net_group_stride(const endo_net* net) { return net ? net->gs : 0; }
extern "C" int64_t endo_net_param_offset(int index) {
    const Table& tb = table();
    if (index < 0 || index >= static_cast<int>(tb.param_offsets.size())) return -1;
    return tb.param_offsets[index];
}
extern "C" int64_t endo_net_bn_offset(int bn_index, int which) {
    const Table& tb = table();
    if (bn_index < 0 || bn_index >= static_cast<int>(tb.bn_order.size()) || which < 0 || which > 1) return -1;
    return tb.bn_order[bn_index]->run + which * tb.bn_order[bn_index]->c;
}
extern "C" int endo_net_level_channels(int level) { return (level < 0 || level > kLevels) ? -1 : level_channels(level); }
extern "C" int64_t endo_net_act_offset(const endo_net* net, int level) { return (!net || level < 0 || level > kLevels) ? -1 : net->lv[level].act; }

extern "C" int64_t endo_net_tape_offset(const endo_net* net, int what, int index) {
    if (!net) return -1;
    const Table& tb = table();
    switch (what) {
        case ENDO_TAPE_PRE: return net->pre_off;
        case ENDO_TAPE_BN_SAVED:
            if (index < 0 || index >= static_cast<int>(tb.bn_order.size())) return -1;
            return net->saved_off + 2 * tb.bn_order[index]->saved;
        case ENDO_TAPE_POOL:
            if (index < 0 || index >= kLevels) return -1;
            return net->idx_off[index];
        default: return -1;
    }
}

extern "C" int endo_net_fwd(endo_net* net, const float* params, float* bn_running, const float* x, float* out, float* tape,
                            int training, void* stream_) {
    if (!net || !params || !bn_running || !x || !out || !tape) return ENDO_E_BADARG;
    const Table& tb = table();
    Ctx c{net, params, bn_running, tape, nullptr, nullptr, training, static_cast<hipStream_t>(stream_)};
    for (int g = 0; g < net->groups; ++g)
        ENDO_CHECK(hipMemsetAsync(reinterpret_cast<char*>(tape + g * net->gs) + net->sums_off, 0, net->sums_bytes, c.stream));
    if (!mfma_bf16_fwd(c)) {
        ProfScope prof(kProfSmall, c.stream, 0.0, 4.0 * (tb.wino_floats + tb.wino_floats * 9 / 16));
        WinoWeightTable wt = tb.wino;
        for (int l = 0; l < wt.layers; ++l) {
            const int level = l < kLevels * kLayers ? l / kLayers : (l < (kLevels + 1) * kLayers ? kLevels : kLevels - 1 - (l - (kLevels + 1) * kLayers) / kLayers);
            wt.mode[l] = dense_fwd_chunk_weights(c, level) ? 1 : 0;
        }
        wino_fwd_weights_kernel<<<(wt.start[wt.layers] + 255) / 256, 256, 0, c.stream>>>(wt, params, tape + net->wino_off);
        ENDO_LAUNCH_CHECK();
        if (wino_fwd_mode(c) == 5) wino4_fwd_weights_kernel<<<(tb.wino4.start[tb.wino4.layers] + 255) / 256, 256, 0, c.stream>>>(tb.wino4, params, tape + net->wino4_off);
        ENDO_LAUNCH_CHECK();
    }
    int rc;
    bool fused_final = false;
    {
        ConvParams p{};
        fill_grid(c, p, 0);
        p.in = x; p.in_ns = 3 * net->lv[0].plane; p.in_cs = static_cast<int>(net->lv[0].plane); p.in_w = net->w; p.cin = 3;
        p.in_gs = net->n * p.in_ns;
        p.wgt = params + tb.first.w; p.bias = params + tb.first.b; p.w_cout = kFirst; p.w_cin = 3;
        fill_out(c, p, c.act(0), 0, 48, kFirst);
        p.out_sums = c.out_sums(0, 48);
        ProfScope prof(kProfConvFirst, c.stream, conv_flops(net, 0, 3, kFirst, 3), 4.0 * c.nt() * net->lv[0].plane * (3 + kFirst));
        rc = launch_conv_dma_auto<3, 4, 3, IN_PLAIN, EPI_FWD>(p, c.stream);
        if (rc) return rc;
    }
    for (int l = 0; l < kLevels; ++l) {
        for (int j = 0; j < kLayers; ++j) {
            rc = dense_fwd(c, l, 48, 48 + down_in(l) + kGrowth * j, tb.down_bn[l][j], tb.down_conv[l][j]);
            if (rc) return rc;
        }
        rc = td_fwd(c, l, tb.td_bn[l], tb.td_conv[l]);
        if (rc) return rc;
    }
    for (int j = 0; j < kLayers; ++j) {
        rc = dense_fwd(c, kLevels, 0, 288 + kGrowth * j, tb.bott_bn[j], tb.bott_conv[j]);
        if (rc) return rc;
    }
    for (int i = 0; i < kLevels; ++i) {
        const int l = kLevels - 1 - i;
        const int src = l + 1;
        const int src_c0 = (i == 0) ? 288 : 96 + down_in(src);
        rc = tu_fwd(c, l, src, src_c0, tb.tu_conv[i]);
        if (rc) return rc;
        for (int j = 0; j < kLayers; ++j) {
            const bool last = l == 0 && j == kLayers - 1;
            rc = dense_fwd(c, l, 0, 96 + down_in(l) + kGrowth * j, tb.up_bn[i][j], tb.up_conv[i][j], last ? params + tb.final_.w : nullptr,
                           last ? tape + net->pre_off : nullptr, last ? &fused_final : nullptr);
            if (rc) return rc;
        }
    }
    {
        const auto& lv = net->lv[0];
        const int c_first = fused_final ? 96 + down_in(0) + kGrowth * (kLayers - 1) : 0;
        ProfScope prof(kProfConvFinal, c.stream, 2.0 * c.nt() * lv.plane * 192, 4.0 * c.nt() * lv.plane * (194 - c_first));
        int bx = static_cast<int>((lv.plane / 4 + 255) / 256);
        bx = bx < 1 ? 1 : bx;
        final_fwd_kernel<<<dim3(bx, c.nt()), 256, 0, c.stream>>>(c.act(0), lv.t * lv.plane, static_cast<int>(lv.plane), 192,
                                                                 params + tb.final_.w, params + tb.final_.b, tape + net->pre_off, out,
                                                                 net->n, net->gs, c_first);
        ENDO_LAUNCH_CHECK();
    }
    return 0;
}

extern "C" int endo_net_bwd(endo_net* net, const float* params, const float* x, const float* tape, const float* grad_out,
                            float* grads, float* gradws, int training, void* stream_) {
    if (!net || !params || !x || !tape || !grad_out || !grads || !gradws) return ENDO_E_BADARG;
    const Table& tb = table();
    Ctx c{net, params, nullptr, const_cast<float*>(tape), grads, gradws, training, static_cast<hipStream_t>(stream_)};
    BiasParts bias_parts{};
    c.bias_parts = &bias_parts;
    if (!net->wstream) {
        ENDO_CHECK(hipStreamCreateWithFlags(&net->wstream, hipStreamNonBlocking));
        ENDO_CHECK(hipEventCreateWithFlags(&net->ev_fork, hipEventDisableTiming));
        ENDO_CHECK(hipEventCreateWithFlags(&net->ev_join, hipEventDisableTiming));
    }
    for (int g = 0; g < net->groups; ++g)
        ENDO_CHECK(hipMemsetAsync(gradws + g * net->gs + net->pq_off, 0,
                                  static_cast<size_t>(net->scratch_off + net->scratch_bytes - net->pq_off * 4), c.stream));
    if (wino_dgrad_enabled(c) && !mfma_bf16_dgrad(c)) {
        ProfScope prof(kProfSmall, c.stream, 0.0, 4.0 * 2.0 * tb.wino_dgrad_floats);
        dgrad_wino_weights_kernel<<<(tb.wino_dgrad.start[tb.wino_dgrad.layers] + 255) / 256, 256, 0, c.stream>>>(
            tb.wino_dgrad, params, gradws + net->wd_off, (wino_dgrad_mode(c) == 1 || wino_dgrad_mode(c) == 3) ? DgradWino3Geom<4>::kMaxCount / 16 : 0);
        ENDO_LAUNCH_CHECK();
    }
    int rc;
    FinalVirt virt{};
    bool use_virt = false;
    {
        const auto& lv = net->lv[0];
        DgradBlockParams probe{};
        probe.n = c.nt(); probe.h = lv.h; probe.w = lv.w; probe.count = 96 + down_in(0);
        probe.cs = static_cast<int>(lv.plane); probe.ns = lv.t * lv.plane;
        probe.g_cs = static_cast<int>(lv.plane);
        probe.x = c.act(0); probe.out = c.gbuf(0);
        virt.vg = gradws + net->gplane_off; virt.vw = params + tb.final_.w; virt.base = false; virt.base_w = false; virt.gw = grads + tb.final_.w;
        int materialise = 192;
        if (c.net->opt[ENDO_OPT_FINAL_VIRTUAL] && dgrad_block_ok(probe)) {
            use_virt = true;
            virt.base = base_pass_form(c, 0, probe, tb.up_conv[kLevels - 1]) == 1;
            materialise = virt.base ? 0 : 96 + down_in(0);
            virt.base_w = virt.base && wino_dgrad_mode(c) == 3 && dgrad_wino3p_applies(probe);
        }
        {
            Ctx cw;
            rc = c.fork_wgrad(cw, 0);
            if (rc) return rc;
            const int c_first = virt.base_w ? 96 + down_in(0) : 0;
            int by = static_cast<int>((lv.plane + 256 * 16 - 1) / (256 * 16));
            by = by < 1 ? 1 : (by > 16 ? 16 : by);
            ProfScope prof(kProfConvFinal, cw.stream, 2.0 * c.nt() * lv.plane * (192 - c_first), 4.0 * c.nt() * lv.plane * (192 - c_first + 2));
            final_bwd_weight_kernel<<<dim3(192 - c_first + 1, by, c.nt()), 256, 0, cw.stream>>>(grad_out, tape + net->pre_off, c.act(0), lv.t * lv.plane,
                                                                         static_cast<int>(lv.plane), 192, net->n, net->gs, grads + tb.final_.w,
                                                                         grads + tb.final_.b, c_first);
            ENDO_LAUNCH_CHECK();
        }
        ProfScope prof(kProfConvFinal, c.stream, 2.0 * c.nt() * lv.plane * 192, 4.0 * c.nt() * lv.plane * (materialise + 2));
        if (use_virt) {
            int bx = static_cast<int>((lv.plane + 1023) / 1024);
            final_g_kernel<<<dim3(bx, c.nt()), 256, 0, c.stream>>>(grad_out, tape + net->pre_off, gradws + net->gplane_off, static_cast<int>(lv.plane), net->n, net->gs);
            ENDO_LAUNCH_CHECK();
        }
        if (materialise > 0) {
            int bx = static_cast<int>((lv.plane + 255) / 256);
            final_bwd_data_kernel<<<dim3(bx, c.nt()), 256, 0, c.stream>>>(grad_out, tape + net->pre_off, params + tb.final_.w, c.gbuf(0),
                                                                          lv.t * lv.plane, static_cast<int>(lv.plane), materialise, net->n, net->gs, 0);
            ENDO_LAUNCH_CHECK();
        }
    }
    for (int i = kLevels - 1; i >= 0; --i) {
        const int l = kLevels - 1 - i;
        rc = dense_block_bwd(c, l, 0, 96 + down_in(l), tb.up_bn[i], tb.up_conv[i], l > 0, (l == 0 && use_virt) ? &virt : nullptr);
        if (rc) return rc;
        const int src = l + 1;
        const int src_c0 = (i == 0) ? 288 : 96 + down_in(src);
        rc = tu_bwd(c, l, src, src_c0, tb.tu_conv[i]);
        if (rc) return rc;
    }
    rc = dense_block_bwd(c, kLevels, 0, 288, tb.bott_bn, tb.bott_conv, true);
    if (rc) return rc;
    for (int l = kLevels - 1; l >= 0; --l) {
        rc = td_bwd(c, l, tb.td_bn[l], tb.td_conv[l]);
        if (rc) return rc;
        rc = dense_block_bwd(c, l, 48, down_in(l), tb.down_bn[l], tb.down_conv[l], false);
        if (rc) return rc;
    }
    {
        const auto& lv = net->lv[0];
        WgradParams p{};
        fill_wgrad_grid(c, p, 0);
        p.in = x; p.in_ns = 3 * lv.plane; p.in_cs = static_cast<int>(lv.plane); p.in_w = lv.w; p.cin = 3;
        p.in_gs = net->n * p.in_ns;
        p.dy = c.gbuf(0) + 48 * lv.plane; p.dy_ns = lv.t * lv.plane; p.dy_cs = static_cast<int>(lv.plane); p.dy_w = lv.w; p.cout = kFirst;
        p.dw = grads + tb.first.w;
        const bool f34 = c.net->opt[ENDO_OPT_WGRAD_F34] && wgrad_mfma_mode(c) == 0 && wgrad_f34_raw_ok(p, c.net->opt[ENDO_OPT_WINO_MIN_TILES] / 4l);
        const bool fuse_prep = f34 && c.net->opt[ENDO_OPT_FINAL_VIRTUAL];
        if (fuse_prep) {
            p.prep_x = c.act(0) + 48 * lv.plane;
            p.prep_p = c.pq_p(0) + 48; p.prep_q = c.pq_q(0) + 48;
            p.prep_bias = grads + tb.first.b;
        } else {
            rc = prep_dy(c, 0, 48, kFirst, grads + tb.first.b);
            if (rc) return rc;
        }
        Ctx cw;
        rc = c.fork_wgrad(cw, 0);
        if (rc) return rc;
        {
            ProfScope prof(kProfWgradOther, cw.stream, conv_flops(net, 0, 3, kFirst, 3), 4.0 * c.nt() * lv.plane * (3 + kFirst));
            if (fuse_prep)
                rc = launch_wgrad_f34<0, true, true>(p, c.gradws + c.net->wg_scratch_off, cw.stream);
            else if (f34)
                rc = launch_wgrad_f34<0, true>(p, c.gradws + c.net->wg_scratch_off, cw.stream);
            else
            rc = wgrad_taps_ok(p) ? launch_wgrad_taps<12, IN_PLAIN>(p, cw.stream) : launch_wgrad<3, 3, IN_PLAIN, DY_PLAIN>(p, cw.stream);
            if (rc) return rc;
        }
    }
    if (bias_parts.table.n > 0) {
        ProfScope prof(kProfSmall, c.stream, 0.0, 4.0 * bias_parts.used);
        bias_reduce_kernel<<<dim3(bias_parts.table.n, 8), 256, 0, c.stream>>>(bias_parts.table);
        ENDO_LAUNCH_CHECK();
    }
    if (net->wstream) {
        ENDO_CHECK(hipEventRecord(net->ev_join, net->wstream));
        ENDO_CHECK(hipStreamWaitEvent(c.stream, net->ev_join, 0));
    }
    return 0;
}
```

### endoscopydepthestimation-pytorch_amd/csrc/wino4_fwd_kernels.h

```cpp
#pragma once

#include "conv_dma_kernels.h"
#include "wgrad_f34_kernels.h"
#include "wino_fwd_kernels.h"

namespace endo {

constexpr float kW4A = 0.625f, kW4B = 1.5f;
constexpr float kW4A2 = kW4A * kW4A, kW4B2 = kW4B * kW4B;
constexpr float kW4A3 = kW4A2 * kW4A, kW4B3 = kW4B2 * kW4B;
constexpr float kW4P = kW4A2 * kW4B2, kW4S = kW4A2 + kW4B2;
constexpr float kW4N0 = 1.f / kW4P;
constexpr float kW4NA = 1.f / (2.f * kW4A2 * (kW4A2 - kW4B2));
constexpr float kW4NB = 1.f / (2.f * kW4B2 * (kW4B2 - kW4A2));

constexpr int kW4UStride = 576;

__global__ void __launch_bounds__(256) wino4_fwd_weights_kernel(const WinoWeightTable t, const float* __restrict__ params, float* __restrict__ u) {
    const int total = t.start[t.layers];
    for (int item = blockIdx.x * blockDim.x + threadIdx.x; item < total; item += gridDim.x * blockDim.x) {
        int l = 0;
        while (item >= t.start[l + 1]) ++l;
        const int e = item - t.start[l];
        const int ci = e >> 4, j = e & 15;
        float g[3][3];
#pragma unroll
        for (int a = 0; a < 3; ++a)
#pragma unroll
            for (int b = 0; b < 3; ++b) g[a][b] = 0.f;
        if (j < t.cout[l]) {
            const float* src = params + t.w_off[l] + (static_cast<int64_t>(j) * t.cin[l] + ci) * 9;
#pragma unroll
            for (int a = 0; a < 3; ++a)
#pragma unroll
                for (int b = 0; b < 3; ++b) g[a][b] = src[a * 3 + b];
        }
        auto gt = [](float a, float b, float c, float (&o)[6]) {
            const float ea = fmaf(kW4A2, c, a), eb = fmaf(kW4B2, c, a);
            o[0] = kW4N0 * a;
            o[1] = kW4NA * fmaf(kW4A, b, ea);
            o[2] = kW4NA * fmaf(-kW4A, b, ea);
            o[3] = kW4NB * fmaf(kW4B, b, eb);
            o[4] = kW4NB * fmaf(-kW4B, b, eb);
            o[5] = c;
        };
        float h[6][3];
#pragma unroll
        for (int b = 0; b < 3; ++b) {
            float o[6];
            gt(g[0][b], g[1][b], g[2][b], o);
#pragma unroll
            for (int i = 0; i < 6; ++i) h[i][b] = o[i];
        }
        float* dst = u + t.u_off[l] + static_cast<int64_t>(ci) * kW4UStride + j * 12;
#pragma unroll
        for (int i = 0; i < 6; ++i) {
            float o[6];
            gt(h[i][0], h[i][1], h[i][2], o);
#pragma unroll
            for (int jj = 0; jj < 6; ++jj) dst[(i >> 1) * 192 + (i & 1) * 6 + jj] = o[jj];
        }
    }
}

struct Wino4Geom {
    static constexpr int kTileX = 64, kTileY = 16;
    static constexpr int kCols = kTileX + 8;
    static constexpr int kRows = kTileY + 2;
    static constexpr int kPlane = kRows * kCols;
    static constexpr int kKC = 4;
    static constexpr int kXUnits = kKC * kPlane / 4;
    static constexpr int kUUnits = kKC * kW4UStride / 4;
    static constexpr int kXRounds = (kXUnits + kConvThreads - 1) / kConvThreads;
    static constexpr int kURounds = (kUUnits + kConvThreads - 1) / kConvThreads;
    static constexpr int kBuf = kKC * kPlane + kKC * kW4UStride;
    static constexpr int kTail = 4 * 16 * 2;
    static size_t bytes(int bn_cap) { return sizeof(float) * (2 * kBuf + 4 * bn_cap + kTail); }
};

__device__ __forceinline__ void w4_at(const float m0, const float m1, const float m2, const float m3, const float m4, const float m5, float (&y)[4]) {
    const float s1 = m1 + m2, d1 = m1 - m2, s2 = m3 + m4, d2 = m3 - m4;
    y[0] = m0 + s1 + s2;
    y[1] = fmaf(kW4B, d2, kW4A * d1);
    y[2] = fmaf(kW4B2, s2, kW4A2 * s1);
    y[3] = fmaf(kW4B3, d2, fmaf(kW4A3, d1, m5));
}

template <typename T>
__device__ __forceinline__ void w4_bt(const T d0, const T d1, const T d2, const T d3, const T d4, const T d5, T (&t)[6]) {
    t[0] = f34_fma<T>(kW4P, d0, f34_fma<T>(-kW4S, d2, d4));
    const T pp = f34_fma<T>(-kW4B2, d2, d4), qh = f34_fma<T>(-kW4B2, d1, d3);
    t[1] = f34_fma<T>(kW4A, qh, pp);
    t[2] = f34_fma<T>(-kW4A, qh, pp);
    const T rr = f34_fma<T>(-kW4A2, d2, d4), sh = f34_fma<T>(-kW4A2, d1, d3);
    t[3] = f34_fma<T>(kW4B, sh, rr);
    t[4] = f34_fma<T>(-kW4B, sh, rr);
    t[5] = f34_fma<T>(kW4P, d1, f34_fma<T>(-kW4S, d3, d5));
}

template <bool FIN = false>
__global__ void __launch_bounds__(kConvThreads, 2) wino4_fwd_kernel(const ConvParams p0) {
    using G = Wino4Geom;
    extern __shared__ __attribute__((aligned(16))) float smem[];
    float* s_aux = smem + 2 * G::kBuf;
    int grp, n;
    group_of(p0, blockIdx.z, grp, n);
    const ConvParams p = group_view(p0, grp);
    const int groups = p0.group_n > 0 ? gridDim.z / p0.group_n : 1;
    const bool first_of_group = blockIdx.x == 0 && n == 0;
    const int cap = p.bn_cap;

    const int tid = threadIdx.x;
    const int lane = tid & 63;
    const int wave = __builtin_amdgcn_readfirstlane(tid >> 6);
    const int li = lane & 15;
    const int lk = lane >> 4;
    const int tile = (gridDim.x & 7) == 0 ? xcd_remap(blockIdx.x, gridDim.x) : blockIdx.x;
    const int x0 = (tile % p.tiles_x) * G::kTileX;
    const int y0 = (tile / p.tiles_x) * G::kTileY;

    for (int c = tid; c < p.cin; c += kConvThreads) {
        float scale, mean, beta;
        bn_input_constants(p, p0, grp, groups, first_of_group, c, scale, mean, beta);
        s_aux[c] = scale;
        s_aux[cap + c] = mean;
        s_aux[2 * cap + c] = beta;
        if constexpr (FIN) s_aux[3 * cap + G::kTail + c] = p.fin_w[c];
    }
    f32x4 fin[4];
#pragma unroll
    for (int r = 0; r < 4; ++r) fin[r] = f32x4{0.f, 0.f, 0.f, 0.f};

    f32x4 acc[36];
#pragma unroll
    for (int xi = 0; xi < 36; ++xi) acc[xi] = f32x4{0.f, 0.f, 0.f, 0.f};

    const __amdgpu_buffer_rsrc_t xr = f34_rsrc(p.in + n * p.in_ns, p.cin * p.in_cs * 4);
    const __amdgpu_buffer_rsrc_t ur = f34_rsrc(p.wgt, p.cin * kW4UStride * 4);
    unsigned x_vo[G::kXRounds];
#pragma unroll
    for (int k = 0; k < G::kXRounds; ++k) {
        const int e = tid + k * kConvThreads;
        x_vo[k] = 0x80000000u;
        if (e < G::kXUnits) {
            const int c = e / (G::kPlane / 4), u = e - c * (G::kPlane / 4);
            const int ry = u / (G::kCols / 4);
            const int rx = (u - ry * (G::kCols / 4)) * 4;
            const int gy = y0 - 1 + ry;
            const int gx = x0 - 4 + rx;
            if (gy >= 0 && gy < p.h && gx >= 0 && gx < p.w) x_vo[k] = 4u * static_cast<unsigned>(c * p.in_cs + gy * p.in_w + gx);
        }
    }
    const unsigned u_vo = 16u * static_cast<unsigned>(tid);
    const int nchunks = p.cin / G::kKC;

    auto issue_dma = [&](int chunk, int buf) {
        float* s_stage = smem + buf * G::kBuf + wave * 256;
        const unsigned xs = 4u * static_cast<unsigned>(chunk * G::kKC * p.in_cs);
        const unsigned us = 4u * static_cast<unsigned>(chunk * G::kKC * kW4UStride);
#pragma unroll
        for (int k = 0; k < G::kXRounds; ++k) {
            const int e0 = k * kConvThreads + wave * 64;
            if (e0 < G::kXUnits) {
                if (e0 + 64 <= G::kXUnits || e0 + lane < G::kXUnits)
                    __builtin_amdgcn_raw_ptr_buffer_load_lds(xr, (lptr_t)(s_stage + k * 4 * kConvThreads), 16, x_vo[k], xs, 0, 0);
            }
        }
        float* s_u = s_stage + G::kKC * G::kPlane;
#pragma unroll
        for (int k = 0; k < G::kURounds; ++k) {
            const int e0 = k * kConvThreads + wave * 64;
            if (e0 < G::kUUnits)
                __builtin_amdgcn_raw_ptr_buffer_load_lds(ur, (lptr_t)(s_u + k * 4 * kConvThreads), 16, u_vo + 16u * static_cast<unsigned>(k * kConvThreads), us, 0, 0);
        }
    };

    const bool l_out = x0 + 4 * li == 0, r_out = x0 + 4 * li + 4 >= p.w;
    const int py = y0 + 4 * wave - 1;
    const bool top_out = py < 0, bottom_out = py + 5 >= p.h;

    auto compute = [&](int chunk, int buf) {
        const float* s_in = smem + buf * G::kBuf;
        const float* s_u = s_in + G::kKC * G::kPlane;
        const int ch = chunk * G::kKC + lk;
        const float sc = s_aux[ch], mn = s_aux[cap + ch], bt = s_aux[2 * cap + ch];
        const float sh = fmaf(-mn, sc, bt);
        const f32x2 sc_m = {sc, sc}, sh_m = {sh, sh};
        const f32x2 sc_e = {l_out ? 0.f : sc, r_out ? 0.f : sc}, sh_e = {l_out ? 0.f : sh, r_out ? 0.f : sh};
        const float* a_base = s_in + lk * G::kPlane + (4 * wave) * G::kCols + 4 * li + 4;
        float wfin = 0.f;
        if constexpr (FIN) wfin = s_aux[3 * cap + G::kTail + ch];
        float d[6][6];
#pragma unroll
        for (int r = 0; r < 6; ++r) {
            const f32x4 m = *reinterpret_cast<const f32x4*>(a_base + r * G::kCols);
            if constexpr (FIN) {
                if (r >= 1 && r <= 4) {
#pragma unroll
                    for (int k = 0; k < 4; ++k) fin[r - 1][k] = fmaf(wfin, m[k], fin[r - 1][k]);
                }
            }
            const float hl = a_base[r * G::kCols - 1], hr = a_base[r * G::kCols + 4];
            const f32x2 e = __builtin_elementwise_fma(f32x2{hl, hr}, sc_e, sh_e);
            const f32x2 a = __builtin_elementwise_fma(f32x2{m[0], m[1]}, sc_m, sh_m);
            const f32x2 b = __builtin_elementwise_fma(f32x2{m[2], m[3]}, sc_m, sh_m);
            d[r][0] = fmaxf(e[0], 0.f); d[r][1] = fmaxf(e[1], 0.f);
            d[r][2] = fmaxf(a[0], 0.f); d[r][3] = fmaxf(a[1], 0.f);
            d[r][4] = fmaxf(b[0], 0.f); d[r][5] = fmaxf(b[1], 0.f);
        }
        if (top_out) {
#pragma unroll
            for (int e = 0; e < 6; ++e) d[0][e] = 0.f;
        }
        if (bottom_out) {
#pragma unroll
            for (int e = 0; e < 6; ++e) d[5][e] = 0.f;
        }
        f32x2 t05[6], t12[6], t34[6];
        w4_bt(f32x2{d[0][0], d[0][1]}, f32x2{d[1][0], d[1][1]}, f32x2{d[2][0], d[2][1]}, f32x2{d[3][0], d[3][1]}, f32x2{d[4][0], d[4][1]},
              f32x2{d[5][0], d[5][1]}, t05);
        w4_bt(f32x2{d[0][2], d[0][3]}, f32x2{d[1][2], d[1][3]}, f32x2{d[2][2], d[2][3]}, f32x2{d[3][2], d[3][3]}, f32x2{d[4][2], d[4][3]},
              f32x2{d[5][2], d[5][3]}, t12);
        w4_bt(f32x2{d[0][4], d[0][5]}, f32x2{d[1][4], d[1][5]}, f32x2{d[2][4], d[2][5]}, f32x2{d[3][4], d[3][5]}, f32x2{d[4][4], d[4][5]},
              f32x2{d[5][4], d[5][5]}, t34);
        const float* b_base = s_u + lk * kW4UStride + li * 12;
#pragma unroll
        for (int ip = 0; ip < 3; ++ip) {
            const f32x4 u0 = *reinterpret_cast<const f32x4*>(b_base + ip * 192);
            const f32x4 u1 = *reinterpret_cast<const f32x4*>(b_base + ip * 192 + 4);
            const f32x4 u2 = *reinterpret_cast<const f32x4*>(b_base + ip * 192 + 8);
            const float uu[12] = {u0[0], u0[1], u0[2], u0[3], u1[0], u1[1], u1[2], u1[3], u2[0], u2[1], u2[2], u2[3]};
#pragma unroll
            for (int h = 0; h < 2; ++h) {
                const int i = 2 * ip + h;
                const f32x2 p05 = t05[i], p12 = t12[i], p34 = t34[i];
                const float x0v = fmaf(kW4P, p05[0], fmaf(-kW4S, p12[1], p34[1]));
                const float x5v = fmaf(kW4P, p12[0], fmaf(-kW4S, p34[0], p05[1]));
                const f32x2 qp = f34_fma<f32x2>(-kW4B2, p12, p34);
                const f32x2 sr = f34_fma<f32x2>(-kW4A2, p12, p34);
                const float x1v = fmaf(kW4A, qp[0], qp[1]), x2v = fmaf(-kW4A, qp[0], qp[1]);
                const float x3v = fmaf(kW4B, sr[0], sr[1]), x4v = fmaf(-kW4B, sr[0], sr[1]);
                acc[6 * i + 0] = __builtin_amdgcn_mfma_f32_16x16x4f32(x0v, uu[6 * h + 0], acc[6 * i + 0], 0, 0, 0);
                acc[6 * i + 1] = __builtin_amdgcn_mfma_f32_16x16x4f32(x1v, uu[6 * h + 1], acc[6 * i + 1], 0, 0, 0);
                acc[6 * i + 2] = __builtin_amdgcn_mfma_f32_16x16x4f32(x2v, uu[6 * h + 2], acc[6 * i + 2], 0, 0, 0);
                acc[6 * i + 3] = __builtin_amdgcn_mfma_f32_16x16x4f32(x3v, uu[6 * h + 3], acc[6 * i + 3], 0, 0, 0);
                acc[6 * i + 4] = __builtin_amdgcn_mfma_f32_16x16x4f32(x4v, uu[6 * h + 4], acc[6 * i + 4], 0, 0, 0);
                acc[6 * i + 5] = __builtin_amdgcn_mfma_f32_16x16x4f32(x5v, uu[6 * h + 5], acc[6 * i + 5], 0, 0, 0);
            }
        }
    };

    if (nchunks > 0) issue_dma(0, 0);
    for (int chunk = 0; chunk < nchunks; ++chunk) {
        const int b = chunk & 1;
        asm volatile("s_waitcnt vmcnt(0)" ::: "memory");
        __syncthreads();
        if (chunk + 1 < nchunks) issue_dma(chunk + 1, b ^ 1);
        compute(chunk, b);
    }

    if constexpr (FIN) {
        f32x4 mine = fin[0];
#pragma unroll
        for (int r = 0; r < 4; ++r) {
#pragma unroll
            for (int k = 0; k < 4; ++k) {
                float v = fin[r][k];
                v += __shfl_xor(v, 16, 64);
                v += __shfl_xor(v, 32, 64);
                if (r == lk) mine[k] = v;
            }
        }
        const int fx = x0 + 4 * li, fy = y0 + 4 * wave + lk;
        if (fx < p.w && fy < p.h)
            *reinterpret_cast<f32x4*>(p.fin_out + static_cast<int64_t>(grp) * p0.gs + static_cast<int64_t>(n) * p.h * p.w + static_cast<int64_t>(fy) * p.w + fx) = mine;
    }

    float* s_red = s_aux + 3 * cap;
    const int co = li;
    const bool co_ok = co < p.cout;
    const float bias = (co_ok && p.bias) ? p.bias[co] : 0.f;
    const int y = y0 + 4 * wave;
    float s1 = 0.f, s2 = 0.f;
#pragma unroll
    for (int e = 0; e < 4; ++e) {
        float c4[4][6];
#pragma unroll
        for (int c = 0; c < 6; ++c) {
            float o[4];
            w4_at(acc[c][e], acc[6 + c][e], acc[12 + c][e], acc[18 + c][e], acc[24 + c][e], acc[30 + c][e], o);
#pragma unroll
            for (int a = 0; a < 4; ++a) c4[a][c] = o[a];
        }
        const int px = x0 + 4 * (4 * lk + e);
#pragma unroll
        for (int a = 0; a < 4; ++a) {
            float o[4];
            w4_at(c4[a][0], c4[a][1], c4[a][2], c4[a][3], c4[a][4], c4[a][5], o);
            const f32x4 v = {o[0] + bias, o[1] + bias, o[2] + bias, o[3] + bias};
            if (co_ok && px < p.w && y + a < p.h) {
                *reinterpret_cast<f32x4*>(p.out + n * p.out_ns + static_cast<int64_t>(co) * p.out_cs + static_cast<int64_t>(y + a) * p.out_w + px) = v;
#pragma unroll
                for (int k = 0; k < 4; ++k) { s1 += v[k]; s2 += v[k] * v[k]; }
            }
        }
    }
    if (p.out_sums) {
        s1 += __shfl_xor(s1, 16, 64); s1 += __shfl_xor(s1, 32, 64);
        s2 += __shfl_xor(s2, 16, 64); s2 += __shfl_xor(s2, 32, 64);
        if (lk == 0) {
            s_red[(wave * 16 + li) * 2] = s1;
            s_red[(wave * 16 + li) * 2 + 1] = s2;
        }
        __syncthreads();
        if (tid < 32) {
            const int j = tid >> 1, which = tid & 1;
            if (j < p.cout) {
                double t = 0.0;
                for (int wv = 0; wv < 4; ++wv) t += static_cast<double>(s_red[(wv * 16 + j) * 2 + which]);
                atomicAdd(p.out_sums + 2 * j + which, t);
            }
        }
    }
}

inline bool wino4_fwd_ok(const ConvParams& p) {
    return wino_fwd_ok(p) && (p.h % 4 == 0) && static_cast<int64_t>(p.cin) * p.in_cs * 4 < (1ll << 31);
}

template <bool FIN>
inline int launch_wino4_fwd_t(ConvParams p, hipStream_t stream) {
    using G = Wino4Geom;
    p.tiles_x = (p.w + G::kTileX - 1) / G::kTileX;
    p.bn_cap = (p.cin + 15) / 16 * 16;
    const int tiles_y = (p.h + G::kTileY - 1) / G::kTileY;
    return launch_dyn(wino4_fwd_kernel<FIN>, dim3(p.tiles_x * tiles_y, 1, p.n), kConvThreads, G::bytes(p.bn_cap), stream, p);
}
inline int launch_wino4_fwd(const ConvParams& p, hipStream_t stream) {
    return p.fin_w ? launch_wino4_fwd_t<true>(p, stream) : launch_wino4_fwd_t<false>(p, stream);
}

}
```

### endoscopydepthestimation-pytorch_amd/csrc/wino_fwd_kernels.h

```cpp
#pragma once

#include "conv_dma_kernels.h"

namespace endo {

constexpr int kWinoUStride = 16 * 16 + 16;
constexpr int kWinoMaxLayers = 48;

struct WinoWeightTable {
    int layers;
    int start[kWinoMaxLayers + 1];
    int cin[kWinoMaxLayers];
    int cout[kWinoMaxLayers];
    int64_t w_off[kWinoMaxLayers];
    int64_t u_off[kWinoMaxLayers];
    int mode[kWinoMaxLayers];
};
constexpr int kDenseChunkFloats = 9 * 16 * 16;

__global__ void __launch_bounds__(256) wino_fwd_weights_kernel(const WinoWeightTable t, const float* __restrict__ params, float* __restrict__ u) {
    const int total = t.start[t.layers];
    for (int item = blockIdx.x * blockDim.x + threadIdx.x; item < total; item += gridDim.x * blockDim.x) {
        int l = 0;
        while (item >= t.start[l + 1]) ++l;
        const int e = item - t.start[l];
        const int ci = e >> 4, j = e & 15;
        float g[3][3];
#pragma unroll
        for (int a = 0; a < 3; ++a)
#pragma unroll
            for (int b = 0; b < 3; ++b) g[a][b] = 0.f;
        if (j < t.cout[l]) {
            const float* src = params + t.w_off[l] + (static_cast<int64_t>(j) * t.cin[l] + ci) * 9;
#pragma unroll
            for (int a = 0; a < 3; ++a)
#pragma unroll
                for (int b = 0; b < 3; ++b) g[a][b] = src[a * 3 + b];
        }
        if (t.mode[l] == 1) {
            float* dst = u + t.u_off[l] + static_cast<int64_t>(ci >> 4) * kDenseChunkFloats + (ci & 15) * 16 + j;
#pragma unroll
            for (int tap = 0; tap < 9; ++tap) dst[tap * 256] = g[tap / 3][tap % 3];
            if (ci == t.cin[l] - 1)
                for (int cz = (ci & 15) + 1; cz < 16; ++cz)
#pragma unroll
                    for (int tap = 0; tap < 9; ++tap) dst[tap * 256 + (cz - (ci & 15)) * 16] = 0.f;
            continue;
        }
        float h[4][3];
#pragma unroll
        for (int b = 0; b < 3; ++b) {
            h[0][b] = g[0][b];
            h[1][b] = 0.5f * (g[0][b] + g[1][b] + g[2][b]);
            h[2][b] = 0.5f * (g[0][b] - g[1][b] + g[2][b]);
            h[3][b] = g[2][b];
        }
        float* dst = u + t.u_off[l] + static_cast<int64_t>(ci) * kWinoUStride + j;
#pragma unroll
        for (int a = 0; a < 4; ++a) {
            dst[(4 * a + 0) * 16] = h[a][0];
            dst[(4 * a + 1) * 16] = 0.5f * (h[a][0] + h[a][1] + h[a][2]);
            dst[(4 * a + 2) * 16] = 0.5f * (h[a][0] - h[a][1] + h[a][2]);
            dst[(4 * a + 3) * 16] = h[a][2];
        }
        if (j == 0) {
#pragma unroll
            for (int k = 0; k < 16; ++k) dst[256 + k] = 0.f;
        }
    }
}

template <int R, int KC, int NS = 2>
struct WinoFwdGeom {
    static constexpr int kTileX = 32;
    static constexpr int kTileY = 8 * R;
    static constexpr int kLeft = 4;
    static constexpr int kCols = kTileX + 2 * kLeft;
    static constexpr int kRows = kTileY + 2;
    static constexpr int kPlane = kRows * kCols;
    static constexpr int kCS = ((kPlane - 32 + 63) / 64) * 64 + 32;
    static constexpr int kUnits = kCS / 4;
    static constexpr int kPos = (kUnits + kConvThreads - 1) / kConvThreads;
    static constexpr int kUUnits = KC * kWinoUStride / 4;
    static constexpr int kUPos = (kUUnits + kConvThreads - 1) / kConvThreads;
    static constexpr int kFlat = KC * kUnits + kUUnits;
    static constexpr int kDma = (kFlat + kConvThreads - 1) / kConvThreads;
    static constexpr int kDmaMin = (kFlat - (kDma - 1) * kConvThreads > 3 * 64) ? kDma : kDma - 1;
    static_assert(kCS == 4 * kUnits, "a stage is one contiguous array of DMA units");
    static constexpr int kBuf = KC * kCS + KC * kWinoUStride;
    static constexpr int kTail = 4 * 16 * 2;
    static size_t bytes(int bn_cap) { return sizeof(float) * (NS * kBuf + 3 * bn_cap + kTail); }
};

template <int R, int KC, int MINW, int NS, int EXP = 0>
__global__ void __launch_bounds__(kConvThreads, MINW) wino_fwd_kernel(const ConvParams p0) {
    using G = WinoFwdGeom<R, KC, NS>;
    typedef float f32x2 __attribute__((ext_vector_type(2)));
    extern __shared__ __attribute__((aligned(16))) float smem[];
    float* s_aux = smem + NS * G::kBuf;
    int grp, n;
    group_of(p0, blockIdx.z, grp, n);
    const ConvParams p = group_view(p0, grp);
    const int groups = p0.group_n > 0 ? gridDim.z / p0.group_n : 1;
    const bool first_of_group = blockIdx.x == 0 && n == 0;
    const int cap = p.bn_cap;

    const int tid = threadIdx.x;
    const int lane = tid & 63;
    const int wave = __builtin_amdgcn_readfirstlane(tid >> 6);
    const int li = lane & 15;
    const int lk = lane >> 4;
    const int tile = (gridDim.x & 7) == 0 ? xcd_remap(blockIdx.x, gridDim.x) : blockIdx.x;
    const int x0 = (tile % p.tiles_x) * G::kTileX;
    const int y0 = (tile / p.tiles_x) * G::kTileY;

    for (int c = tid; c < p.cin; c += kConvThreads) {
        float scale, mean, beta;
        bn_input_constants(p, p0, grp, groups, first_of_group, c, scale, mean, beta);
        s_aux[c] = scale;
        s_aux[cap + c] = mean;
        s_aux[2 * cap + c] = beta;
    }
    for (int c = p.cin + tid; c < ((p.cin + KC - 1) / KC) * KC; c += kConvThreads) {
        s_aux[c] = 0.f; s_aux[cap + c] = 0.f; s_aux[2 * cap + c] = 0.f;
    }

    f32x4 acc[R][16];
#pragma unroll
    for (int r = 0; r < R; ++r)
#pragma unroll
        for (int xi = 0; xi < 16; ++xi) acc[r][xi] = f32x4{0.f, 0.f, 0.f, 0.f};

    const float* d_ptr[G::kDma];
    unsigned d_stride[G::kDma];
    {
        const float* in_n = p.in + n * p.in_ns;
#pragma unroll
        for (int k = 0; k < G::kDma; ++k) {
            const int e = tid + k * kConvThreads;
            d_ptr[k] = g_pad_consts;
            d_stride[k] = 0;
            if (e < KC * G::kUnits) {
                const int c = e / G::kUnits, u = e - c * G::kUnits;
                const int ry = u / (G::kCols / 4);
                const int rx = (u - ry * (G::kCols / 4)) * 4;
                const int gy = y0 - 1 + ry;
                const int gx = x0 - G::kLeft + rx;
                if (ry < G::kRows && gy >= 0 && gy < p.h && gx >= 0 && gx < p.w) {
                    d_ptr[k] = in_n + static_cast<int64_t>(c) * p.in_cs + gy * p.in_w + gx;
                    d_stride[k] = static_cast<unsigned>(KC) * static_cast<unsigned>(p.in_cs) * 4u;
                }
            } else if (e < G::kFlat) {
                d_ptr[k] = p.wgt + 4 * (e - KC * G::kUnits);
                d_stride[k] = KC * kWinoUStride * 4u;
            }
        }
    }
    const int nchunks = p.cin / KC;

    auto issue_dma = [&](int buf) {
        float* s_stage = smem + buf * G::kBuf + wave * 256;
#pragma unroll
        for (int k = 0; k < G::kDma; ++k) {
            if (k + 1 < G::kDma) {
                __builtin_amdgcn_global_load_lds((gptr_t)d_ptr[k], (lptr_t)(s_stage + k * 4 * kConvThreads), 16, 0, 0);
            } else {
                const int e0 = k * kConvThreads + wave * 64;
                if (e0 < G::kFlat && e0 + lane < G::kFlat)
                    __builtin_amdgcn_global_load_lds((gptr_t)d_ptr[k], (lptr_t)(s_stage + k * 4 * kConvThreads), 16, 0, 0);
            }
            d_ptr[k] = reinterpret_cast<const float*>(reinterpret_cast<const char*>(d_ptr[k]) + d_stride[k]);
        }
    };

    auto compute = [&](int chunk, int buf) {
        const float* s_in = smem + buf * G::kBuf;
        const float* s_u = s_in + KC * G::kCS;
#pragma unroll
        for (int quad = 0; quad < KC / 4; ++quad) {
            const int ch = chunk * KC + quad * 4 + lk;
            const float sc = s_aux[ch], mn = s_aux[cap + ch], bt = s_aux[2 * cap + ch];
            const f32x2 mn2 = {mn, mn}, sc2 = {sc, sc}, bt2 = {bt, bt};
            const float* b_base = s_u + (quad * 4 + lk) * kWinoUStride + li;
            float b[16];
#pragma unroll
            for (int xi = 0; xi < 16; ++xi) b[xi] = (EXP & 16) ? static_cast<float>(xi + lane) : b_base[xi * 16];
            const float* a_base = s_in + (quad * 4 + lk) * G::kCS + (2 * wave * R) * G::kCols + 2 * li + 2;
            f32x2 mid[2 * R + 2], end[2 * R + 2];
#pragma unroll
            for (int row = 0; row < 2 * R + 2; ++row) {
                f32x2 m, e;
                if constexpr ((EXP & 8) != 0) {
                    m = f32x2{sc + row, mn + row}; e = f32x2{bt + row, sc - row};
                } else {
                    const f32x2 left = *reinterpret_cast<const f32x2*>(a_base + row * G::kCols);
                    const f32x2 right = *reinterpret_cast<const f32x2*>(a_base + row * G::kCols + 4);
                    m = *reinterpret_cast<const f32x2*>(a_base + row * G::kCols + 2);
                    e = f32x2{left[1], right[0]};
                }
                if constexpr ((EXP & 2) == 0) {
                    m = __builtin_elementwise_fma(m - mn2, sc2, bt2);
                    e = __builtin_elementwise_fma(e - mn2, sc2, bt2);
                    mid[row] = f32x2{__builtin_fmaxf(m[0], 0.f), __builtin_fmaxf(m[1], 0.f)};
                    end[row] = f32x2{__builtin_fmaxf(e[0], 0.f), __builtin_fmaxf(e[1], 0.f)};
                } else {
                    mid[row] = m; end[row] = e;
                }
            }
#pragma unroll
            for (int r = 0; r < R; ++r) {
                f32x2 tm[4], te[4];
                if constexpr ((EXP & 4) == 0) {
                    tm[0] = mid[2 * r] - mid[2 * r + 2];     te[0] = end[2 * r] - end[2 * r + 2];
                    tm[1] = mid[2 * r + 1] + mid[2 * r + 2]; te[1] = end[2 * r + 1] + end[2 * r + 2];
                    tm[2] = mid[2 * r + 2] - mid[2 * r + 1]; te[2] = end[2 * r + 2] - end[2 * r + 1];
                    tm[3] = mid[2 * r + 1] - mid[2 * r + 3]; te[3] = end[2 * r + 1] - end[2 * r + 3];
                } else {
#pragma unroll
                    for (int a = 0; a < 4; ++a) { tm[a] = mid[2 * r + a]; te[a] = end[2 * r + a]; }
                }
#pragma unroll
                for (int a = 0; a < 4; ++a) {
                    const float c0 = te[a][0], c1 = tm[a][0], c2 = tm[a][1], c3 = te[a][1];
                    float v0 = c0 - c2, v1 = c1 + c2, v2 = c2 - c1, v3 = c1 - c3;
                    if constexpr ((EXP & 4) != 0) { v0 = c0; v1 = c1; v2 = c2; v3 = c3; }
                    if constexpr ((EXP & 64) != 0) {
                        acc[r][4 * a + 0][0] += v0 * b[4 * a]; acc[r][4 * a + 1][0] += v1 * b[4 * a + 1];
                        acc[r][4 * a + 2][0] += v2 * b[4 * a + 2]; acc[r][4 * a + 3][0] += v3 * b[4 * a + 3];
                    } else {
                        acc[r][4 * a + 0] = __builtin_amdgcn_mfma_f32_16x16x4f32(v0, b[4 * a + 0], acc[r][4 * a + 0], 0, 0, 0);
                        acc[r][4 * a + 1] = __builtin_amdgcn_mfma_f32_16x16x4f32(v1, b[4 * a + 1], acc[r][4 * a + 1], 0, 0, 0);
                        acc[r][4 * a + 2] = __builtin_amdgcn_mfma_f32_16x16x4f32(v2, b[4 * a + 2], acc[r][4 * a + 2], 0, 0, 0);
                        acc[r][4 * a + 3] = __builtin_amdgcn_mfma_f32_16x16x4f32(v3, b[4 * a + 3], acc[r][4 * a + 3], 0, 0, 0);
                    }
                }
            }
        }
    };

#pragma unroll
    for (int s0 = 0; s0 < NS - 1; ++s0)
        if (s0 < nchunks) issue_dma(s0);
    for (int chunk = 0; chunk < nchunks; ++chunk) {
        const int b = chunk % NS;
        const int newer = min(nchunks - 1 - chunk, NS - 2);
        if ((EXP & 32) && chunk > 0) {}
        else if (newer >= NS - 2 && NS > 2) asm volatile("s_waitcnt vmcnt(%0)" ::"n"((NS - 2) * G::kDmaMin) : "memory");
        else if (newer == 1 && NS > 3) asm volatile("s_waitcnt vmcnt(%0)" ::"n"(G::kDmaMin) : "memory");
        else asm volatile("s_waitcnt vmcnt(0)" ::: "memory");
        if (!(EXP & 32) || chunk == 0) __syncthreads();
        if (chunk + NS - 1 < nchunks && !(EXP & 1)) issue_dma((chunk + NS - 1) % NS);
        compute(chunk, b);
    }

    float* s_red = s_aux + 3 * cap;
    const int co = li;
    const bool co_ok = co < p.cout;
    const float bias = (co_ok && p.bias) ? p.bias[co] : 0.f;
    const int px = x0 + 8 * lk;
    float s1 = 0.f, s2 = 0.f;
#pragma unroll
    for (int r = 0; r < R; ++r) {
        const int y = y0 + 2 * (wave * R + r);
        f32x4 row0[2], row1[2];
#pragma unroll
        for (int e = 0; e < 4; ++e) {
            float u0[4], u1[4];
#pragma unroll
            for (int c = 0; c < 4; ++c) {
                const float m0 = acc[r][c][e], m1 = acc[r][4 + c][e], m2 = acc[r][8 + c][e], m3 = acc[r][12 + c][e];
                u0[c] = m0 + m1 + m2;
                u1[c] = m1 - m2 - m3;
            }
            row0[e >> 1][2 * (e & 1)] = u0[0] + u0[1] + u0[2] + bias;
            row0[e >> 1][2 * (e & 1) + 1] = u0[1] - u0[2] - u0[3] + bias;
            row1[e >> 1][2 * (e & 1)] = u1[0] + u1[1] + u1[2] + bias;
            row1[e >> 1][2 * (e & 1) + 1] = u1[1] - u1[2] - u1[3] + bias;
        }
        if (co_ok) {
#pragma unroll
            for (int half = 0; half < 2; ++half) {
                if (px + 4 * half + 3 < p.w) {
                    float* dst = p.out + n * p.out_ns + static_cast<int64_t>(co) * p.out_cs + static_cast<int64_t>(y) * p.out_w + px + 4 * half;
                    if (y < p.h) {
                        *reinterpret_cast<f32x4*>(dst) = row0[half];
#pragma unroll
                        for (int e = 0; e < 4; ++e) { s1 += row0[half][e]; s2 += row0[half][e] * row0[half][e]; }
                    }
                    if (y + 1 < p.h) {
                        *reinterpret_cast<f32x4*>(dst + p.out_w) = row1[half];
#pragma unroll
                        for (int e = 0; e < 4; ++e) { s1 += row1[half][e]; s2 += row1[half][e] * row1[half][e]; }
                    }
                }
            }
        }
    }
    if (p.out_sums) {
        s1 += __shfl_xor(s1, 16, 64); s1 += __shfl_xor(s1, 32, 64);
        s2 += __shfl_xor(s2, 16, 64); s2 += __shfl_xor(s2, 32, 64);
        if (lk == 0) {
            s_red[(wave * 16 + li) * 2] = s1;
            s_red[(wave * 16 + li) * 2 + 1] = s2;
        }
        __syncthreads();
        if (tid < 32) {
            const int j = tid >> 1, which = tid & 1;
            if (j < p.cout) {
                double t = 0.0;
                for (int wv = 0; wv < 4; ++wv) t += static_cast<double>(s_red[(wv * 16 + j) * 2 + which]);
                atomicAdd(p.out_sums + 2 * j + which, t);
            }
        }
    }
}

inline bool wino_fwd_ok(const ConvParams& p) {
    return p.cout <= 16 && (p.w % 4 == 0) && (p.in_w % 4 == 0) && (p.out_w % 4 == 0) && (p.in_cs % 4 == 0) && (p.in_ns % 4 == 0) &&
           (p.out_cs % 4 == 0) && (p.out_ns % 4 == 0) && (reinterpret_cast<uintptr_t>(p.in) % 16 == 0) &&
           (reinterpret_cast<uintptr_t>(p.out) % 16 == 0) && (reinterpret_cast<uintptr_t>(p.wgt) % 16 == 0) && p.ksplit == 0 &&
           p.cin % 4 == 0 && p.cin >= 8;
}

template <int R, int KC, int MINW, int NS, int EXP = 0>
inline int launch_wino_fwd(ConvParams p, hipStream_t stream) {
    using G = WinoFwdGeom<R, KC, NS>;
    p.tiles_x = (p.w + G::kTileX - 1) / G::kTileX;
    p.bn_cap = ((p.cin + KC - 1) / KC * KC + 15) / 16 * 16;
    const int tiles_y = (p.h + G::kTileY - 1) / G::kTileY;
    return launch_dyn(wino_fwd_kernel<R, KC, MINW, NS, EXP>, dim3(p.tiles_x * tiles_y, 1, p.n), kConvThreads, G::bytes(p.bn_cap), stream, p);
}


}
```

### endoscopydepthestimation-pytorch_amd/models.py

```python

import ctypes

import torch
from torch import nn

from . import _lib

GROWTH = 12
LAYERS = 4
FIRST = 48
LEVELS = 5


class ConvParams(nn.Module):

    def __init__(self, cin, cout, k):
        super().__init__()
        self.weight = nn.Parameter(torch.empty(cout, cin, k, k))
        self.bias = nn.Parameter(torch.zeros(cout))
        nn.init.kaiming_uniform_(self.weight, a=5 ** 0.5)


class FusedBatchNorm2d(nn.Module):

# ... 80 lines not shown
        ctx.net = net
        ctx.training = net.training
        ctx.tape = tape
        ctx.shape = tuple(x.shape)
        return out

    @staticmethod
    def backward(ctx, grad_out):
        if ctx.needs_input_grad[0]:
            raise RuntimeError("FCDenseNet57 on the MI355X path does not produce a gradient for its input image; detach the input")
        if ctx.tape is None:
            raise RuntimeError("FCDenseNet57: the forward tape of this call was released by its first backward pass")
        ctx.net._run_backward16(ctx.shape, ctx.tape, grad_out, ctx.training, 1, ctx.half)
        ctx.tape = None
        return None, None, None, None


class FCDenseNet(nn.Module):

    def __init__(self, n_classes=1):
        super().__init__()
        if n_classes != 1:
            raise ValueError("the MI355X path implements the depth network (n_classes=1) only")
        self.firstconv = ConvParams(3, FIRST, 3)
        c = FIRST
        skips = []
        self.denseBlocksDown = nn.ModuleList()
        self.transDownBlocks = nn.ModuleList()
        for _ in range(LEVELS):
            self.denseBlocksDown.append(DenseBlock(c))
            c += GROWTH * LAYERS
            skips.insert(0, c)
            self.transDownBlocks.append(TransitionDown(c))
        self.bottleneck = Bottleneck(c)
        new = GROWTH * LAYERS
        self.transUpBlocks = nn.ModuleList()
        self.denseBlocksUp = nn.ModuleList()
        for i in range(LEVELS):
            self.transUpBlocks.append(TransitionUp(new))
            self.denseBlocksUp.append(DenseBlock(new + skips[i]))
        self.finalConv = ConvParams(new + skips[-1] + new, 1, 1)

        self._flat = None
        self._flat_grad = None
        self._flat_grad_full = None
        self._flat_bn = None
        self._nbt = None
        self._handles = {}
        self._gradws = {}
        self._anchor = None
        self._flatten()

    def _bn_modules(self):
        return [m for m in self.modules() if isinstance(m, FusedBatchNorm2d)]

    def _flatten(self):
        params = list(self.parameters())
        device = params[0].device
        total = sum(p.numel() for p in params)
        flat = torch.empty(total, dtype=torch.float32, device=device)
        off = 0
        offsets = []
        for p in params:
            n = p.numel()
            flat[off:off + n].copy_(p.data.reshape(-1).float())
            p.data = flat[off:off + n].view(p.shape)
            p.grad = None
            offsets.append(off)
            off += n
        self._flat, self._offsets, self._params = flat, offsets, params
        self._flat_grad = None
        self._flat_grad_full = None
        bns = self._bn_modules()
        width = sum(2 * m.num_features for m in bns)
        flat_bn = torch.empty(width, dtype=torch.float32, device=device)
        nbt = torch.empty(len(bns), dtype=torch.long, device=device)
        off = 0
        for i, m in enumerate(bns):
            c = m.num_features
            flat_bn[off:off + c].copy_(m.running_mean)
            flat_bn[off + c:off + 2 * c].copy_(m.running_var)
            nbt[i] = m.num_batches_tracked
            m._buffers["running_mean"] = flat_bn[off:off + c]
            m._buffers["running_var"] = flat_bn[off + c:off + 2 * c]
            m._buffers["num_batches_tracked"] = nbt[i]
            off += 2 * c
        self._flat_bn, self._nbt, self._bns = flat_bn, nbt, bns
        self._anchor = torch.zeros(1, device=device, requires_grad=True)
        self._gradws = {}

    def _apply(self, fn, recurse=True):
        super()._apply(fn, recurse)
        self._flatten()
        return self

    def _views_intact(self):
        base = self._flat.data_ptr()
        for p, off in zip(self._params, self._offsets):
            if p.data_ptr() != base + 4 * off:
                return False
        off = 0
        base = self._flat_bn.data_ptr()
        for m in self._bns:
            if m.running_mean.data_ptr() != base + 4 * off:
                return False
            off += 2 * m.num_features
        return True

    def flat_parameters(self):
        return self._flat

    def flat_gradients(self, create=True):
        self._attach_grads(create)
        return self._flat_grad

    def flat_gradient_bucket(self):
        self._attach_grads(True)
        return self._flat_grad_full

    def _attach_grads(self, create=True):
        if self._flat_grad is None or self._flat_grad.device != self._flat.device:
            if not create:
                return
            self._flat_grad_full = torch.zeros(self._flat.numel() + 1, dtype=torch.float32, device=self._flat.device)
            self._flat_grad = self._flat_grad_full[:self._flat.numel()]
            for p, off in zip(self._params, self._offsets):
                p.grad = self._flat_grad[off:off + p.numel()].view(p.shape)
            return
        base = self._flat_grad.data_ptr()
        intact = True
        for p, off in zip(self._params, self._offsets):
            g = p.grad
            if g is None or g.data_ptr() != base + 4 * off:
                intact = False
                break
        if not intact:
            self._flat_grad.zero_()
            for p, off in zip(self._params, self._offsets):
                p.grad = self._flat_grad[off:off + p.numel()].view(p.shape)

    def _handle(self, n, h, w, groups=1):
        key = (n, h, w, groups)
        if key not in self._handles:
            lib = _lib.load()
            if lib.endo_net_param_floats() != self._flat.numel():
                raise RuntimeError("parameter packing mismatch between Python and libendo_hip.so")
            hnd = ctypes.c_void_p()
            _lib.check(lib.endo_net_create_grouped(ctypes.byref(hnd), n, h, w, groups), "endo_net_create_grouped(%d,%d,%d,%d)" % key)
            for option_id, value in getattr(self, "_kernel_options", {}).items():
                lib.endo_net_set_option(hnd, option_id, value)
            self._handles[key] = (hnd, int(lib.endo_net_tape_floats(hnd)), int(lib.endo_net_gradws_floats(hnd)))
        return self._handles[key]

    _OPTION_DEFAULTS = {0: 5, 1: 3, 2: 2, 3: 1024, 4: 0, 5: 1, 6: 0, 7: 1, 8: 1, 9: 3}

    def set_kernel_option(self, option_id, value):
        option_id, value = int(option_id), int(value)
        if option_id not in self._OPTION_DEFAULTS:
            raise ValueError("unknown kernel option %d" % option_id)
        options = self.__dict__.setdefault("_kernel_options", {})
        old = options.get(option_id, self._OPTION_DEFAULTS[option_id])
        options[option_id] = value
        lib = _lib.load()
        for key, (hnd, _, _) in self._handles.items():
            if key[0] in ("bf16", "fp16"):
                continue
            rc = lib.endo_net_set_option(hnd, option_id, value)
            if rc < 0:
                raise RuntimeError("endo_net_set_option(%d, %d) failed: %d" % (option_id, value, rc))
        return old

    def kernel_option(self, option_id):
        return self.__dict__.get("_kernel_options", {}).get(int(option_id), self._OPTION_DEFAULTS[int(option_id)])

    def __del__(self):
        try:
            lib = _lib.load()
            for key, (hnd, _, _) in self._handles.items():
                {"bf16": lib.endo_net16_destroy, "fp16": lib.endo_net16h_destroy}.get(key[0], lib.endo_net_destroy)(hnd)
            self._handles = {}
        except Exception:
            pass

    def __getstate__(self):
        state = dict(self.__dict__)
        for key in ("_handles", "_gradws"):
            state[key] = {}
        for key in ("_flat_grad", "_flat_grad_full", "_anchor"):
            state[key] = None
        return state

    def __setstate__(self, state):
        self.__dict__.update(state)
        self._handles, self._gradws = {}, {}
        self._flatten()

    def __deepcopy__(self, memo):
        import copy
        clone = self.__class__.__new__(self.__class__)
        memo[id(self)] = clone
        state = self.__getstate__()
        for key in ("_flat", "_flat_bn", "_nbt", "_params", "_bns", "_offsets"):
            state.pop(key, None)
        clone.__dict__.update(copy.deepcopy(state, memo))
        clone._handles, clone._gradws = {}, {}
        for p in clone.parameters():
            p.grad = None
        clone._flatten()
        return clone

    def _run_forward(self, x, groups=1):
        lib = _lib.load()
        x = _lib.dev_f32(x, "FCDenseNet57 input")
        if x.dim() != 4 or x.shape[1] != 3:
            raise RuntimeError("expected N x 3 x H x W input")
        if x.device != self._flat.device:
            raise RuntimeError("model and input are on different devices; call model.cuda() first")
        if not self._views_intact():
            self._flatten()
        n, _, h, w = x.shape
        if n % groups:
            raise RuntimeError("batch of %d samples does not split into %d groups" % (n, groups))
        hnd, tape_floats, _ = self._handle(n // groups, h, w, groups)
        tape = torch.empty(tape_floats, dtype=torch.float32, device=x.device)
        out = torch.empty((n, 1, h, w), dtype=torch.float32, device=x.device)
        _lib.check(lib.endo_net_fwd(hnd, _lib.ptr(self._flat), _lib.ptr(self._flat_bn), _lib.ptr(x), _lib.ptr(out),
                                    _lib.ptr(tape), 1 if self.training else 0, _lib.stream()), "endo_net_fwd")
        if self.training:
            self._nbt.add_(groups)
        return out, tape

    def _run_backward(self, x, tape, grad_out, training, groups=1):
        lib = _lib.load()
        n, _, h, w = x.shape
        hnd, _, gradws_floats = self._handle(n // groups, h, w, groups)
        key = (n, h, w, groups)
        if key not in self._gradws:
            self._gradws[key] = torch.empty(gradws_floats, dtype=torch.float32, device=x.device)
        self._attach_grads()
        grad_out = _lib.dev_f32(grad_out, "grad_output")
        _lib.check(lib.endo_net_bwd(hnd, _lib.ptr(self._flat), _lib.ptr(x), _lib.ptr(tape), _lib.ptr(grad_out),
                                    _lib.ptr(self._flat_grad), _lib.ptr(self._gradws[key]),
                                    1 if training else 0, _lib.stream()), "endo_net_bwd")

    def forward(self, x):
        if torch.is_grad_enabled():
            return _NetFunction.apply(x, self._anchor, self)
        out, _ = self._run_forward(x)
        return out

    def forward_bf16_storage(self, x):
        if torch.is_grad_enabled():
            return _Net16Function.apply(x, self._anchor, self)
        out, _ = self._run_forward16(_lib.dev_f32(x, "FCDenseNet57 input"))
        return out

    def forward_fp16_storage(self, x):
        if torch.is_grad_enabled():
            return _Net16Function.apply(x, self._anchor, self, True)
        out, _ = self._run_forward16(_lib.dev_f32(x, "FCDenseNet57 input"), 1, True)
        return out

    @staticmethod
    def _api16(half):
        lib = _lib.load()
        prefix = "endo_net16h_" if half else "endo_net16_"
        return lambda name: getattr(lib, prefix + name)

    def set_wgrad_overlap16(self, on):
        self.__dict__["_wgrad_overlap16"] = int(on)
        for key, (hnd, _, _) in self._handles.items():
            if key[0] in ("bf16", "fp16"):
                self._api16(key[0] == "fp16")("set_wgrad_overlap")(hnd, int(on))

    def _handle16(self, n, h, w, groups=1, half=False):
        api = self._api16(half)
        key = ("fp16" if half else "bf16", n, h, w, groups)
        if key not in self._handles:
            hnd = ctypes.c_void_p()
            _lib.check(api("create")(ctypes.byref(hnd), n, h, w, groups), "endo_net16_create(%d,%d,%d,%d)" % (n, h, w, groups))
            api("set_wgrad_overlap")(hnd, int(self.__dict__.get("_wgrad_overlap16", 1)))
            self._handles[key] = (hnd, int(api("tape_bytes")(hnd)), int(api("bwd_workspace_bytes")(hnd)))
        return self._handles[key]

    def forward_pair_bf16_storage(self, x1, x2):
        x = torch.cat([_lib.dev_f32(x1, "FCDenseNet57 input"), _lib.dev_f32(x2, "FCDenseNet57 input")], dim=0)
        out, _ = self._run_forward16(x, 2)
        n = x1.shape[0]
        return out[:n], out[n:]

    def _run_forward16(self, x, groups=1, half=False):
        api = self._api16(half)
        if x.dim() != 4 or x.shape[1] != 3:
            raise RuntimeError("expected N x 3 x H x W input")
        if x.device != self._flat.device:
            raise RuntimeError("model and input are on different devices; call model.cuda() first")
        if not self._views_intact():
            self._flatten()
        n, _, h, w = x.shape
        hnd, tape_bytes, _ = self._handle16(n // groups, h, w, groups, half)
        tape = torch.empty(tape_bytes, dtype=torch.uint8, device=x.device)
        out = torch.empty((n, 1, h, w), dtype=torch.float32, device=x.device)
        with torch.no_grad():
            _lib.check(api("fwd")(hnd, _lib.ptr(self._flat), _lib.ptr(self._flat_bn), _lib.ptr(x), _lib.ptr(out), _lib.ptr(tape),
                                  1 if self.training else 0, _lib.stream()), "endo_net16_fwd")
        if self.training:
            self._nbt.add_(groups)
# ... 196 lines not shown
```

### include/endo_hip.h

```cpp
#ifndef ENDO_HIP_H
#define ENDO_HIP_H

#include <stdint.h>

#ifdef __cplusplus
extern "C" {
#endif

#define ENDO_E_BADARG (-1)
#define ENDO_E_UNSUPPORTED (-2)

#define ENDO_ABI_VERSION 6
int endo_abi_version(void);
const char* endo_error_string(int code);

int endo_depth_scale_fwd(const float* pred, const float* sparse_depth, const float* sparse_mask,
                         float* scaled, float* ratio, double* stats,
                         int n, int hw, float eps, void* stream);
int endo_depth_scale_bwd(const float* grad_scaled, const float* grad_ratio,
                         const float* pred, const float* sparse_depth, const double* stats,
                         float* grad_pred, double* work,
                         int n, int hw, float eps, void* stream);

int endo_flow_from_depth_fwd(const float* depth, const float* mask, const float* t, const float* R,
                             const float* K, float* flow, int n, int h, int w, void* stream);
int endo_flow_from_depth_bwd(const float* grad_flow, const float* depth, const float* mask,
                             const float* t, const float* R, const float* K, float* grad_depth,
                             int n, int h, int w, void* stream);

int endo_depth_warp_fwd(const float* depth_1, const float* depth_2, const float* mask,
                        const float* t, const float* R, const float* K,
                        float* warped, float* intersect,
                        int n, int h, int w, float eps, void* stream);
int endo_depth_warp_bwd(const float* grad_warped, const float* depth_1, const float* depth_2,
                        const float* mask, const float* t, const float* R, const float* K,
                        float* grad_d1, float* grad_d2,
                        int n, int h, int w, float eps, void* stream);
int endo_depth_warp_fwd_tiled(const float* depth_1, const float* depth_2, const float* mask,
                              const float* t, const float* R, const float* K,
                              float* warped, float* intersect,
                              int n, int h, int w, float eps, int tile_h, int tile_w, void* stream);
int endo_depth_warp_bwd_tiled(const float* grad_warped, const float* depth_1, const float* depth_2,
                              const float* mask, const float* t, const float* R, const float* K,
                              float* grad_d1, float* grad_d2,
                              int n, int h, int w, float eps, int tile_h, int tile_w, void* stream);
int endo_warp_fallback_blocks(long long* forward, long long* backward, int reset);


int endo_sparse_l1_fwd(const float* flows, const float* flows_hat, const float* mask,
                       float* loss, double* stats, int n, int c, int hw, float eps, void* stream);
int endo_sparse_l1_bwd(const float* grad_loss, const float* flows, const float* flows_hat,
                       const float* mask, const double* stats, float* grad_flows, float* grad_hat,
                       int n, int c, int hw, float eps, void* stream);

int endo_norm_dist_fwd(const float* depth, const float* warped, const float* intersect,
                       const float* K, float* loss, double* stats,
                       int n, int h, int w, float eps, void* stream);
int endo_norm_dist_bwd(const float* grad_loss, const float* depth, const float* warped,
                       const float* intersect, const float* K, const double* stats,
                       float* grad_depth, float* grad_warped,
                       int n, int h, int w, float eps, void* stream);

int endo_scale_inv_fwd(const float* pred, const float* goal, const float* boundary,
                       float* loss, double* stats, int n, int hw, float eps, void* stream);
int endo_scale_inv_bwd(const float* grad_loss, const float* pred, const float* goal,
                       const float* boundary, const double* stats,
                       float* grad_pred, float* grad_goal, int n, int hw, float eps, void* stream);

int64_t endo_loss_head_workspace_floats(int n, int h, int w);
int endo_loss_head(const float* pred_1, const float* pred_2, const float* boundaries,
                   const float* sparse_depths_1, const float* sparse_depths_2,
                   const float* sparse_depth_masks_1, const float* sparse_depth_masks_2,
                   const float* sparse_flows_1, const float* sparse_flows_2,
                   const float* sparse_flow_masks_1, const float* sparse_flow_masks_2,
                   const float* t_1_wrt_2, const float* r_1_wrt_2, const float* t_2_wrt_1, const float* r_2_wrt_1,
                   const float* intrinsics, float sfl_weight, float dcl_weight, float eps,
                   float* losses, float* grad_pred_1, float* grad_pred_2, float* workspace,
                   int n, int h, int w, void* stream);
int endo_loss_head_planes(int n, int h, int w, int64_t* offsets);

int64_t endo_warp_consistency_workspace_floats(int n, int h, int w);
int64_t endo_warp_consistency_bytes(int n, int h, int w);
int endo_warp_consistency(const float* depth_1, const float* depth_2, const float* boundaries, const float* t_1_wrt_2,
                          const float* r_1_wrt_2, const float* t_2_wrt_1, const float* r_2_wrt_1, const float* intrinsics,
                          float dcl_weight, float eps, float* loss, float* grad_depth_1, float* grad_depth_2,
                          float* workspace, int n, int h, int w, void* stream);


int endo_mask_mul(const float* a, const float* mask, float* out, int n, int c, int hw, void* stream);

typedef struct endo_net endo_net;

int endo_net_create(endo_net** out, int n, int h, int w);
int endo_net_create_grouped(endo_net** out, int n, int h, int w, int groups);
int endo_net_groups(const endo_net* net);
#define ENDO_OPT_WINO_FWD 0
#define ENDO_OPT_WINO_DGRAD 1
#define ENDO_OPT_DGRAD_VEC 2
#define ENDO_OPT_WINO_MIN_TILES 3
#define ENDO_OPT_MFMA_BF16 4
#define ENDO_OPT_WGRAD_OVERLAP 5
#define ENDO_OPT_MFMA_X3 6
#define ENDO_OPT_WGRAD_F34 7
#define ENDO_OPT_FINAL_VIRTUAL 8
#define ENDO_OPT_TD_PERSIST 9
#define ENDO_OPT_COUNT 10
int endo_net_set_option(endo_net* net, int option_id, int value);
int endo_net_get_option(const endo_net* net, int option_id);
int64_t endo_net_group_stride(const endo_net* net);
void endo_net_destroy(endo_net* net);
int64_t endo_net_param_floats(void);
int64_t endo_net_bn_floats(void);
int64_t endo_net_tape_floats(const endo_net* net);
int64_t endo_net_gradws_floats(const endo_net* net);
int64_t endo_net_param_offset(int index);
int64_t endo_net_bn_offset(int bn_index, int which );

int endo_net_fwd(endo_net* net, const float* params, float* bn_running, const float* x, float* out,
                 float* tape, int training, void* stream);
int endo_net_bwd(endo_net* net, const float* params, const float* x, const float* tape,
                 const float* grad_out, float* grads, float* gradws, int training, void* stream);
int endo_net_level_channels(int level);
int64_t endo_net_act_offset(const endo_net* net, int level);
#define ENDO_TAPE_PRE 0
#define ENDO_TAPE_BN_SAVED 1
#define ENDO_TAPE_POOL 2
int64_t endo_net_tape_offset(const endo_net* net, int what, int index);

int endo_sgd_clip_step(float* params, float* grads, float* momentum, double* norm_out,
                       int64_t count, float lr, float mu, float max_norm, float grad_scale,
                       int first_step, const float* skip_flag, void* stream);

int endo_sparse_scatter(const double* points, int n_points, const double* projections, const double* extrinsics,
                        const float* visibility, const float* clean, const uint8_t* mask, int batch, int height, int width,
                        float depth_multiplier, int32_t* winner_scratch, float* depth_masks, float* depths, float* flow_masks,
                        float* flows, void* stream);

int endo_relative_poses(const double* pair_extrinsics, int batch, double scale,
                        float* r_1_wrt_2, float* t_1_wrt_2, float* r_2_wrt_1, float* t_2_wrt_1, void* stream);

int endo_point_cloud(const float* depth, const uint8_t* color_bgr, const float* mask, const float* intrinsics, int height,
                     int width, int downsampling, int use_threshold, float min_threshold, float max_threshold,
                     int32_t* row_offsets, float* points, int32_t* count_out, void* stream);

int endo_jpeg_info(const uint8_t* data, int64_t size, int32_t* info);
int endo_jpeg_entropy_decode(const uint8_t* data, int64_t size, int16_t* blocks, int64_t capacity_blocks, uint16_t* quant);
int64_t endo_jpeg_workspace_bytes(const uint8_t* data, int64_t size);
int endo_jpeg_decode_crop(const uint8_t* data, int64_t size, double downsampling, int start_h, int end_h, int start_w,
                          int end_w, int rgb_order, uint8_t* out_hwc, float* out_chw, void* staging, void* workspace,
                          int64_t workspace_bytes, void* stream);

int endo_point_brightness(const uint8_t* imgs, int frames, int height, int width, const double* points, int n_points,
                          const double* projections, const double* extrinsics, const float* visibility, const uint8_t* mask,
                          int d, double sigma_color, double sigma_space, int32_t* valid, double* depth, float* brightness,
                          void* stream);

int endo_hsv_full(const uint8_t* src, int64_t pixels, int blue_index, uint8_t* out_u8, float* out_f32, void* stream);

typedef struct endo_augment_frame {
    int32_t colour;
    int32_t spatial;
    int32_t ksize;
    int32_t jpeg;
    int32_t noise;
    float sigma;
    uint32_t seed[2];
    uint32_t motion[2];
    int32_t reserved[6];
    uint8_t rgb_lut[256];
    uint8_t hsv_lut[3][256];
    uint16_t quant[2][64];
} endo_augment_frame;
int endo_augment_frame_bytes(void);
int64_t endo_augment_workspace_bytes(int frames, int height, int width);
int endo_augment(const uint8_t* src, const endo_augment_frame* params, int frames, int height, int width, uint8_t* out_u8,
                 float* out_f32, void* workspace, int64_t workspace_bytes, void* stream);

int64_t endo_evaluate_workspace_bytes(int frames, int height, int width);
int endo_evaluate(const float* colors, const float* boundaries, const float* predictions, const float* intrinsics, int frames,
                  int height, int width, int is_hsv, int point_cloud_downsampling, float* depth, uint8_t* panels, float* points,
                  int64_t* frame_offsets, void* workspace, int64_t workspace_bytes, void* stream);

int64_t endo_display_workspace_bytes(int n, int h, int w);
int endo_display_panel_shape(int n, int h, int w, int* rows, int* cols);
int endo_display(const float* colors_1, const float* colors_2, const float* depths_1, const float* depths_2, const float* boundaries,
                 const float* sparse_flows_1, const float* sparse_flows_2, const float* flows_1, const float* flows_2, int n, int h, int w,
                 uint8_t* out, void* workspace, int64_t workspace_bytes, void* stream);

int endo_validation_accumulate(const float* losses, int batch_index, double* means, double* history, void* stream);

#define ENDO_PROF_FAMILIES 16
int endo_prof_enable(int family_mask);
int endo_prof_sample(int period);
int endo_prof_seen(int family, int64_t* launches);
int endo_prof_read(int family, double* total_ms, int64_t* launches, double* total_flops, double* total_bytes);
const char* endo_prof_family_name(int family);

int endo_bf16_pack_nhwc(const float* x, void* out, int n, int c, int h, int w, int t, int blk, int oc0, void* stream);
int endo_bf16_unpack_nhwc(const void* in, float* x, int n, int c, int h, int w, int t, int blk, int ic0, void* stream);
int64_t endo_bf16_conv_weight_elems(int cout, int cin, int ks);
int endo_bf16_conv_weights(const float* w, int cout, int cin, int ks, void* out, void* stream);
int endo_bf16_conv(const void* in, int in_t, int in_blk, int ic0, int cin, const float* bn, const void* wgt, const float* bias, void* out,
                   int out_t, int out_blk, int oc0, int cout, double* out_sums, int n, int h, int w, int ks, int ups, void* stream);
typedef struct endo_net16 endo_net16;
int endo_net16_create(endo_net16** out, int n_per_group, int h, int w, int groups);
void endo_net16_destroy(endo_net16* net);
int64_t endo_net16_tape_bytes(const endo_net16* net);
int endo_net16_fwd(endo_net16* net, const float* params, float* bn_running, const float* x, float* out, void* tape, int training,
                   void* stream);
int64_t endo_net16_bwd_workspace_bytes(const endo_net16* net);
int endo_net16_set_wgrad_overlap(endo_net16* net, int on);
int endo_net16h_create(endo_net16** out, int n_per_group, int h, int w, int groups);
void endo_net16h_destroy(endo_net16* net);
int64_t endo_net16h_tape_bytes(const endo_net16* net);
int endo_net16h_fwd(endo_net16* net, const float* params, float* bn_running, const float* x, float* out, void* tape, int training,
                    void* stream);
int64_t endo_net16h_bwd_workspace_bytes(const endo_net16* net);
int endo_net16h_set_wgrad_overlap(endo_net16* net, int on);
int64_t endo_net16h_offset(const endo_net16* net, int what, int index);
int endo_net16h_bwd(endo_net16* net, const float* params, const void* tape, const float* grad_out, float* grads, void* ws, int training,
                    void* stream);
int endo_f16_pack_nhwc(const float* x, void* out, int n, int c, int h, int w, int t, int blk, int oc0, void* stream);
int endo_f16_unpack_nhwc(const void* in, float* x, int n, int c, int h, int w, int t, int blk, int ic0, void* stream);
int64_t endo_net16_offset(const endo_net16* net, int what, int index);
int endo_net16_bwd(endo_net16* net, const float* params, const void* tape, const float* grad_out, float* grads, void* ws, int training,
                   void* stream);

#ifdef __cplusplus
}
#endif
#endif
```

Measured before the change: 515.2.

## Split dense-layer forward K into skip and rest segments to overlap on side stream

Adds a two-segment K mode to the direct, Winograd and F(4,3) forward convolution kernels. The input channels coming from the skip connection can then be convolved separately, presumably early on a side stream synchronised by per-level events, and the remaining channels are accumulated into the same output later. The aim is to hide part of the dense-layer forward behind other work. In exchange it adds an extra read-modify-write of the output, more kernel launches and event syncs, and new template instantiations. It is enabled by default through a new option.

```diff
diff --git a/endoscopydepthestimation-pytorch_amd/csrc/conv_dma_kernels.h b/endoscopydepthestimation-pytorch_amd/csrc/conv_dma_kernels.h
--- a/endoscopydepthestimation-pytorch_amd/csrc/conv_dma_kernels.h
+++ b/endoscopydepthestimation-pytorch_amd/csrc/conv_dma_kernels.h
@@ -23,8 +23,9 @@
     static size_t bytes(int bn_cap) { return sizeof(float) * (NBUF * kBuf + 3 * bn_cap + kTail); }
 };
 
-template <int KS, int KC, int Q, int IN, int EPI, int WX, int R, int NBUF, int MINW, int VEC, int XF, int EXP = 0, int PH = -1, int BF = 0>
+template <int KS, int KC, int Q, int IN, int EPI, int WX, int R, int NBUF, int MINW, int VEC, int XF, int EXP = 0, int PH = -1, int BF = 0, int SEG = 0>
 __global__ void __launch_bounds__(kConvThreads, MINW) conv_dma_kernel(const ConvParams p0) {
+    static_assert(SEG == 0 || (IN == IN_BNRELU && EPI == EPI_FWD && PH < 0 && BF == 0 && XF == 0), "two-segment K is the dense layers' forward");
     static_assert(BF == 0 || (PH < 0 && (KS == 3 || KS == 1) && (IN == IN_BNRELU || IN == IN_PLAIN || (IN == IN_UNPOOL && KS == 1))),
                   "bf16 operands: the ordinary 3x3 convolution and the 1x1 convolutions of the transition-down layers");
     static_assert(PH < 0 || (KS == 3 && (Q % 2) == 0 && IN == IN_PLAIN && EPI == EPI_FWD), "phase mode is the transition-up forward");
@@ -65,7 +66,7 @@
     if constexpr (IN == IN_BNRELU) {
         for (int c = tid; c < p.cin; c += kConvThreads) {
             float scale, mean, beta;
-            bn_input_constants(p, p0, grp, groups, first_of_group, c, scale, mean, beta);
+            bn_input_constants(p, p0, grp, groups, first_of_group, (SEG != 0 && c >= p.k_seg) ? c + p.k_jump : c, scale, mean, beta);
             s_aux[c] = scale;
             s_aux[cap + c] = mean;
             s_aux[2 * cap + c] = beta;
@@ -157,6 +158,7 @@
 
     auto issue_dma = [&](int chunk, int buf) {
         const int c_base = chunk * KC;
+        const int jump = (SEG != 0 && c_base >= p.k_seg) ? p.k_jump : 0;
         float* s_in = smem + buf * S::kBuf;
         float* s_w = s_in + KC * S::kChan;
         if constexpr (IN == IN_UNPOOL) {
@@ -182,7 +184,7 @@
 #pragma unroll
         for (int c = 0; c < (IN == IN_UNPOOL ? 0 : KC); ++c) {
             const int ch = c_base + c;
-            const float* plane = in_n + static_cast<int64_t>(ch) * p.in_cs;
+            const float* plane = in_n + static_cast<int64_t>(ch + jump) * p.in_cs;
             if constexpr (IN == IN_SUBPIX)
                 plane = in_n + static_cast<int64_t>(ch - sub_ph * p.sub_c) * p.in_cs + (sub_ph >> 1) * p.in_w + (sub_ph & 1);
 #pragma unroll
@@ -226,7 +228,7 @@
             if (p.wgt_chunks) {
                 gather = false;
                 constexpr int kUnitsW = kWElems / 4;
-                const float* wsrc = p.wgt_chunks + static_cast<int64_t>(chunk) * kWElems;
+                const float* wsrc = p.wgt_chunks + static_cast<int64_t>(chunk + jump / KC) * kWElems;
 #pragma unroll
                 for (int k = 0; k < (kUnitsW + kConvThreads - 1) / kConvThreads; ++k) {
                     const int u0 = k * kConvThreads + wave * 64;
@@ -250,7 +252,7 @@
                 const float* src = pad_zero;
                 if (e < kWElems && ci < p.cin && co < (PH >= 0 ? p.w_cout : p.cout)) {
                     if constexpr (kDgrad) src = p.wgt + (static_cast<int64_t>(ci) * p.w_cin + co) * KK + (KK - 1 - tap);
-                    else src = p.wgt + (static_cast<int64_t>(co) * p.w_cin + ci) * KK + tap;
+                    else src = p.wgt + (static_cast<int64_t>(co) * p.w_cin + ci + jump) * KK + tap;
                 }
                 if (e < kWElems) __builtin_amdgcn_global_load_lds((gptr_t)src, (lptr_t)(s_w + e0), 4, 0, 0);
             }
@@ -624,10 +626,10 @@
         }
         return;
     }
-    conv_epilogue<Q, EPI, R>(po, acc, s_aux + 3 * cap, s_aux + 3 * cap + 4 * NB, x0, y0, wx, wy, co_base, n);
+    conv_epilogue<Q, EPI, R, SEG != 0>(po, acc, s_aux + 3 * cap, s_aux + 3 * cap + 4 * NB, x0, y0, wx, wy, co_base, n);
 }
 
-template <int KS, int KC, int Q, int IN, int EPI, int WX, int R, int NBUF, int MINW, int VEC, int XF = 0, int EXP = 0, int PH = -1, int BF = 0>
+template <int KS, int KC, int Q, int IN, int EPI, int WX, int R, int NBUF, int MINW, int VEC, int XF = 0, int EXP = 0, int PH = -1, int BF = 0, int SEG = 0>
 inline int launch_conv_dma_vec(ConvParams p, hipStream_t stream) {
     static_assert(XF == 0 || NBUF == 2 || IN != IN_BNRELU, "the in-place transform pipeline is written for two buffers");
     using G = ConvGeom<KS, KC, WX, R, VEC>;
@@ -636,27 +638,28 @@
     p.bn_cap = (IN == IN_BNRELU) ? ((p.cin + KC - 1) / KC * KC + 15) / 16 * 16 : 0;
     const int tiles_y = (p.h + G::kTileY - 1) / G::kTileY;
     dim3 grid(p.tiles_x * tiles_y, p.ksplit > 0 ? p.ksplit : (PH >= 0 ? (PH == 2 ? 2 : 1) : (p.cout + 16 * Q - 1) / (16 * Q)), p.n);
-    return launch_dyn(conv_dma_kernel<KS, KC, Q, IN, EPI, WX, R, NBUF, MINW, VEC, XF, EXP, PH, BF>, grid, kConvThreads, S::bytes(p.bn_cap), stream, p);
+    return launch_dyn(conv_dma_kernel<KS, KC, Q, IN, EPI, WX, R, NBUF, MINW, VEC, XF, EXP, PH, BF, SEG>, grid, kConvThreads, S::bytes(p.bn_cap), stream, p);
 }
 
-template <int KS, int KC, int Q, int IN, int EPI, int WX, int R, int NBUF, int MINW = 1, int BF = 0>
+template <int KS, int KC, int Q, int IN, int EPI, int WX, int R, int NBUF, int MINW = 1, int BF = 0, int SEG = 0>
 inline int launch_conv_dma(const ConvParams& p, hipStream_t stream) {
     if constexpr (IN != IN_UPSAMPLE && IN != IN_UNPOOL) {
         const bool aligned = (p.w % 4 == 0) && (p.in_w % 4 == 0) && (p.in_cs % 4 == 0) && (p.in_ns % 4 == 0) &&
                              (reinterpret_cast<uintptr_t>(p.in) % 16 == 0);
-        if (aligned) return launch_conv_dma_vec<KS, KC, Q, IN, EPI, WX, R, NBUF, MINW, 4, 0, 0, -1, BF>(p, stream);
-    }
-    return launch_conv_dma_vec<KS, KC, Q, IN, EPI, WX, R, NBUF, MINW, 1, 0, 0, -1, BF>(p, stream);
+        if (aligned) return launch_conv_dma_vec<KS, KC, Q, IN, EPI, WX, R, NBUF, MINW, 4, 0, 0, -1, BF, SEG>(p, stream);
+    }
+    if constexpr (SEG != 0) return ENDO_E_UNSUPPORTED;
+    else return launch_conv_dma_vec<KS, KC, Q, IN, EPI, WX, R, NBUF, MINW, 1, 0, 0, -1, BF>(p, stream);
 }
 
-template <int KS, int KC, int Q, int IN, int EPI, int BIG_R = 8, int NBUF = 2, int BIG_MINW = 1, int BF = 0>
+template <int KS, int KC, int Q, int IN, int EPI, int BIG_R = 8, int NBUF = 2, int BIG_MINW = 1, int BF = 0, int SEG = 0>
 inline int launch_conv_dma_auto(const ConvParams& p, hipStream_t stream) {
     const long tiles_big = static_cast<long>((p.w + 31) / 32) * ((p.h + 15) / 16) * p.n;
-    if (tiles_big >= 512) return launch_conv_dma<KS, KC, Q, IN, EPI, 2, BIG_R, NBUF, BIG_MINW, BF>(p, stream);
+    if (tiles_big >= 512) return launch_conv_dma<KS, KC, Q, IN, EPI, 2, BIG_R, NBUF, BIG_MINW, BF, SEG>(p, stream);
     const long tiles_mid = static_cast<long>((p.w + 15) / 16) * ((p.h + 15) / 16) * p.n;
-    if (tiles_mid >= 384) return launch_conv_dma<KS, KC, Q, IN, EPI, 1, 4, NBUF, 1, BF>(p, stream);
+    if (tiles_mid >= 384) return launch_conv_dma<KS, KC, Q, IN, EPI, 1, 4, NBUF, 1, BF, SEG>(p, stream);
     constexpr int KCS = (NBUF == 2 && KS == 3 && KC <= 8) ? 16 : KC;
-    return launch_conv_dma<KS, KCS, Q, IN, EPI, 1, 2, NBUF, 1, BF>(p, stream);
+    return launch_conv_dma<KS, KCS, Q, IN, EPI, 1, 2, NBUF, 1, BF, SEG>(p, stream);
 }
 
 }
diff --git a/endoscopydepthestimation-pytorch_amd/csrc/conv_kernels.h b/endoscopydepthestimation-pytorch_amd/csrc/conv_kernels.h
--- a/endoscopydepthestimation-pytorch_amd/csrc/conv_kernels.h
+++ b/endoscopydepthestimation-pytorch_amd/csrc/conv_kernels.h
@@ -56,6 +56,8 @@
     int sub_c;
     const float* fin_w;
     float* fin_out;
+    int k_seg, k_jump;
+    int acc_out;
 };
 
 __device__ __forceinline__ void group_of(const ConvParams& p, int z, int& grp, int& n) {
@@ -134,7 +136,7 @@
     static constexpr int kPre = KC * kPos;
 };
 
-template <int Q, int EPI, int R>
+template <int Q, int EPI, int R, bool ACC = false>
 __device__ __forceinline__ void conv_epilogue(const ConvParams& p, f32x4 (&acc)[R][Q], const float* cst, float* s_red,
                                               int x0, int y0, int wx, int wy, int co_base, int n) {
     constexpr int NB = 16 * Q;
@@ -161,6 +163,17 @@
                 v[0] += bias; v[1] += bias; v[2] += bias; v[3] += bias;
                 if (co_ok && y < p.h) {
                     float* dst = p.out + n * p.out_ns + static_cast<int64_t>(co) * p.out_cs + y * p.out_w + px;
+                    if constexpr (ACC) {
+                        if (vec_ok && px + 3 < p.w) {
+                            const f32x4 prev = *reinterpret_cast<const f32x4*>(dst);
+#pragma unroll
+                            for (int e = 0; e < 4; ++e) v[e] += prev[e];
+                        } else {
+#pragma unroll
+                            for (int e = 0; e < 4; ++e)
+                                if (px + e < p.w) v[e] += dst[e];
+                        }
+                    }
                     if (vec_ok && px + 3 < p.w) {
                         *reinterpret_cast<f32x4*>(dst) = v;
 #pragma unroll
diff --git a/endoscopydepthestimation-pytorch_amd/csrc/net.hip b/endoscopydepthestimation-pytorch_amd/csrc/net.hip
--- a/endoscopydepthestimation-pytorch_amd/csrc/net.hip
+++ b/endoscopydepthestimation-pytorch_amd/csrc/net.hip
@@ -160,7 +160,7 @@
     int64_t bias_parts_floats;
     int64_t gradws_floats;
     hipStream_t wstream;
-    hipEvent_t ev_fork, ev_join;
+    hipEvent_t ev_fork, ev_join, ev_skip[kLevels];
     int opt[ENDO_OPT_COUNT];
 };
 
@@ -537,14 +537,14 @@
     uint8_t* idx(int level) const { return reinterpret_cast<uint8_t*>(tape) + net->idx_off[level]; }
 };
 
-static void fill_bn_in(const Ctx& c, ConvParams& p, const BnP& b, int level, int ic0) {
-    const auto& lv = c.net->lv[level];
-    p.in_sums = c.sums(level) + 2 * ic0;
-    p.gamma = c.params + b.g;
-    p.beta = c.params + b.b;
-    p.running_mean = c.bn_running + b.run;
-    p.running_var = c.bn_running + b.run + b.c;
-    p.saved = c.tape ? c.saved(b) : nullptr;
+static void fill_bn_in(const Ctx& c, ConvParams& p, const BnP& b, int level, int ic0, int first = 0) {
+    const auto& lv = c.net->lv[level];
+    p.in_sums = c.sums(level) + 2 * (ic0 + first);
+    p.gamma = c.params + b.g + first;
+    p.beta = c.params + b.b + first;
+    p.running_mean = c.bn_running + b.run + first;
+    p.running_var = c.bn_running + b.run + b.c + first;
+    p.saved = c.tape ? c.saved(b) + 2 * first : nullptr;
     p.count = static_cast<double>(c.net->n) * lv.h * lv.w;
     p.eps = kBnEps;
     p.momentum = kBnMomentum;
@@ -590,6 +590,7 @@
     opt[ENDO_OPT_WGRAD_F34] = 1;
     opt[ENDO_OPT_FINAL_VIRTUAL] = 1;
     opt[ENDO_OPT_TD_PERSIST] = 3;
+    opt[ENDO_OPT_FWD_SKIP_OVERLAP] = 1;
 }
 static int wino_fwd_mode(const Ctx& c) { return c.net->opt[ENDO_OPT_WINO_FWD]; }
 static bool wino_fwd_enabled(const Ctx& c) { return wino_fwd_mode(c) != 0; }
@@ -618,9 +619,33 @@
     return !mfma_bf16_fwd(c) && !dense_fwd_wino4_tiles(c, level) && !dense_fwd_wino2_tiles(c, level);
 }
 
+static bool dense_fwd_splitk_tiles(const Ctx& c, int level) {
+    const auto& lv = c.net->lv[level];
+    const long tiles_big = static_cast<long>((lv.w + 31) / 32) * ((lv.h + 15) / 16) * c.nt();
+    const long tiles_mid = static_cast<long>((lv.w + 15) / 16) * ((lv.h + 15) / 16) * c.nt();
+    const long tiles_small = static_cast<long>((lv.w + 15) / 16) * ((lv.h + 7) / 8) * c.nt();
+    return tiles_big < 512 && tiles_mid < 384 && tiles_small < 512;
+}
+
+enum DensePart { kWhole = 0, kSkipPart = 1, kRestPart = 2 };
+constexpr int kSkipFirst = 48;
+inline int skip_channels(int level) { return kFirst + down_in(level); }
+
+static bool dense_fwd_split_ok(const Ctx& c, int level) {
+    if (level >= kLevels || mfma_bf16_fwd(c) || wino_fwd_mode(c) == 3 || wino_fwd_mode(c) == 4) return false;
+    const auto& lv = c.net->lv[level];
+    if (lv.w % 4 != 0) return false;
+    if (dense_fwd_wino4_tiles(c, level) && lv.h % 4 == 0 && static_cast<int64_t>(lv.t) * lv.plane * 4 < (1ll << 31)) return true;
+    if (dense_fwd_wino2_tiles(c, level)) return true;
+    return !dense_fwd_splitk_tiles(c, level);
+}
+
 static int dense_fwd(const Ctx& c, int level, int ic0, int oc0, const BnP& b, const ConvP& cv, const float* fin_w = nullptr, float* fin_pre = nullptr,
-                     bool* fused_final = nullptr) {
-    const auto& lv = c.net->lv[level];
+                     bool* fused_final = nullptr, int part = kWhole) {
+    const auto& lv = c.net->lv[level];
+    if (part != kWhole && (ic0 != 0 || !dense_fwd_split_ok(c, level) || fin_w)) return ENDO_E_BADARG;
+    const int skipc = skip_channels(level);
+    const int kc = part == kSkipPart ? skipc : (part == kRestPart ? cv.cin - skipc : cv.cin);
     ConvParams p{};
     fill_grid(c, p, level);
     fill_in(c, p, c.act(level), level, ic0, cv.cin);
@@ -628,13 +653,26 @@
     p.wgt = c.params + cv.w; p.bias = c.params + cv.b; p.w_cout = cv.cout; p.w_cin = cv.cin;
     fill_out(c, p, c.act(level), level, oc0, cv.cout);
     p.out_sums = c.out_sums(level, oc0);
-    ProfScope prof(kProfConv3x3Dense, c.stream, conv_flops(c.net, level, cv.cin, cv.cout, 3),
-                   4.0 * c.nt() * lv.plane * (cv.cin + cv.cout));
+    auto shape = [&](ConvParams& q, int64_t w_per_ch) {
+        if (part == kSkipPart) {
+            fill_in(c, q, c.act(level), level, ic0 + kSkipFirst, skipc);
+            fill_bn_in(c, q, b, level, ic0, kSkipFirst);
+            q.wgt += kSkipFirst * w_per_ch;
+            if (q.wgt_chunks) q.wgt_chunks += kSkipFirst / 16 * kDenseChunkFloats;
+            q.bias = nullptr; q.out_sums = nullptr;
+        } else if (part == kRestPart) {
+            q.cin = kc; q.k_seg = kSkipFirst; q.k_jump = skipc; q.acc_out = 1;
+        }
+    };
+    const bool rest = part == kRestPart;
+    ProfScope prof(kProfConv3x3Dense, c.stream, conv_flops(c.net, level, kc, cv.cout, 3),
+                   4.0 * c.nt() * lv.plane * (kc + (rest ? 2 : 1) * cv.cout));
     if (cv.u >= 0 && dense_fwd_wino4_tiles(c, level)) {
         ConvParams p4 = p;
         p4.wgt = c.tape + c.net->wino4_off + cv.u / kWinoUStride * kW4UStride;
         if (wino4_fwd_ok(p4)) {
             if (fin_w && fused_final && c.net->opt[ENDO_OPT_FINAL_VIRTUAL]) { p4.fin_w = fin_w + ic0; p4.fin_out = fin_pre; *fused_final = true; }
+            shape(p4, kW4UStride);
             return launch_wino4_fwd(p4, c.stream);
         }
     }
@@ -647,6 +685,8 @@
             const int mode = wino_fwd_mode(c);
             const long min_tiles = c.net->opt[ENDO_OPT_WINO_MIN_TILES];
             const bool big = t16 >= min_tiles, small = t8 >= (min_tiles * 3) / 4;
+            if (big || small) shape(pw, kWinoUStride);
+            if (rest) return big ? launch_wino_fwd<2, 4, 2, 2, 0, true>(pw, c.stream) : launch_wino_fwd<1, 4, 3, 2, 0, true>(pw, c.stream);
             if (mode == 4) {
                 if (big) return launch_wino_fwd<2, 4, 2, 4>(pw, c.stream);
                 if (small) return launch_wino_fwd<1, 4, 3, 4>(pw, c.stream);
@@ -676,6 +716,7 @@
     const long tiles_mid = static_cast<long>((lv.w + 15) / 16) * ((lv.h + 15) / 16) * c.nt();
     const long tiles_small = static_cast<long>((lv.w + 15) / 16) * ((lv.h + 7) / 8) * c.nt();
     const int nchunks = (cv.cin + 15) / 16;
+    if (part != kWhole && tiles_big < 512 && tiles_mid < 384 && tiles_small < 512) return ENDO_E_BADARG;
     const float* chunk_weights = (cv.u >= 0 && dense_fwd_chunk_weights(c, level)) ? c.tape + c.net->wino_off + cv.u : nullptr;
     if (tiles_big < 512 && tiles_mid < 384 && tiles_small < 512 && nchunks >= 4) {
         int want = static_cast<int>(((tiles_small < 256 ? 512 : 768) + tiles_small - 1) / tiles_small);
@@ -705,9 +746,15 @@
         if (tiles_big < 1024 && tiles_small >= 768) return launch_conv_dma<3, 8, 1, IN_BNRELU, EPI_FWD, 1, 2, 2, 1, 1>(p, c.stream);
         return launch_conv_dma_auto<3, 4, 1, IN_BNRELU, EPI_FWD, 8, 2, 1, 1>(p, c.stream);
     }
+    p.wgt_chunks = (tiles_big < 1024 && (tiles_wide >= 1024 || tiles_small >= 768)) ? nullptr : chunk_weights;
+    shape(p, 9);
+    if (rest) {
+        if (tiles_big < 1024 && tiles_wide >= 1024) return launch_conv_dma<3, 4, 1, IN_BNRELU, EPI_FWD, 2, 4, 2, 1, 0, 1>(p, c.stream);
+        if (tiles_big < 1024 && tiles_small >= 768) return launch_conv_dma<3, 8, 1, IN_BNRELU, EPI_FWD, 1, 2, 2, 1, 0, 1>(p, c.stream);
+        return launch_conv_dma_auto<3, 4, 1, IN_BNRELU, EPI_FWD, 8, 2, 1, 0, 1>(p, c.stream);
+    }
     if (tiles_big < 1024 && tiles_wide >= 1024) return launch_conv_dma<3, 4, 1, IN_BNRELU, EPI_FWD, 2, 4, 2, 1>(p, c.stream);
     if (tiles_big < 1024 && tiles_small >= 768) return launch_conv_dma<3, 8, 1, IN_BNRELU, EPI_FWD, 1, 2, 2, 1>(p, c.stream);
-    p.wgt_chunks = chunk_weights;
     return launch_conv_dma_auto<3, 4, 1, IN_BNRELU, EPI_FWD, 8, 2, 1>(p, c.stream);
 }
 
@@ -1112,6 +1159,7 @@
     if (!net) return ENDO_E_BADARG;
     net->n = n; net->h = h; net->w = w; net->groups = groups;
     net->wstream = nullptr; net->ev_fork = nullptr; net->ev_join = nullptr;
+    for (int l = 0; l < kLevels; ++l) net->ev_skip[l] = nullptr;
     default_options(net->opt);
     int64_t off = 0, sums = 0, pq = 0;
     for (int l = 0; l <= kLevels; ++l) {
@@ -1186,6 +1234,8 @@
     if (!net) return;
     if (net->ev_fork) (void)hipEventDestroy(net->ev_fork);
     if (net->ev_join) (void)hipEventDestroy(net->ev_join);
+    for (int l = 0; l < kLevels; ++l)
+        if (net->ev_skip[l]) (void)hipEventDestroy(net->ev_skip[l]);
     if (net->wstream) (void)hipStreamDestroy(net->wstream);
     delete net;
 }
@@ -1221,6 +1271,17 @@
             return net->idx_off[index];
         default: return -1;
     }
+}
+
+static int ensure_side_stream(endo_net* net) {
+    if (net->wstream) return 0;
+    int least = 0, greatest = 0;
+    ENDO_CHECK(hipDeviceGetStreamPriorityRange(&least, &greatest));
+    ENDO_CHECK(hipStreamCreateWithPriority(&net->wstream, hipStreamNonBlocking, least));
+    ENDO_CHECK(hipEventCreateWithFlags(&net->ev_fork, hipEventDisableTiming));
+    ENDO_CHECK(hipEventCreateWithFlags(&net->ev_join, hipEventDisableTiming));
+    for (int l = 0; l < kLevels; ++l) ENDO_CHECK(hipEventCreateWithFlags(&net->ev_skip[l], hipEventDisableTiming));
+    return 0;
 }
 
 extern "C" int endo_net_fwd(endo_net* net, const float* params, float* bn_running, const float* x, float* out, float* tape,
@@ -1256,6 +1317,35 @@
         rc = launch_conv_dma_auto<3, 4, 3, IN_PLAIN, EPI_FWD>(p, c.stream);
         if (rc) return rc;
     }
+    const int overlap = net->opt[ENDO_OPT_FWD_SKIP_OVERLAP];
+    bool split[kLevels] = {};
+    int deepest = -1;
+    if (overlap) {
+        rc = ensure_side_stream(net);
+        if (rc) return rc;
+        for (int l = 0; l < kLevels; ++l) {
+            split[l] = dense_fwd_split_ok(c, l);
+            if (split[l]) deepest = l;
+        }
+    }
+    auto fork_side = [&]() -> int {
+        ENDO_CHECK(hipEventRecord(net->ev_fork, c.stream));
+        ENDO_CHECK(hipStreamWaitEvent(net->wstream, net->ev_fork, 0));
+        return 0;
+    };
+    auto skip_parts = [&](int l) -> int {
+        Ctx cs = c;
+        cs.stream = net->wstream;
+        const int i = kLevels - 1 - l;
+        for (int j = 0; j < kLayers; ++j) {
+            if (l == 0 && j == kLayers - 1) continue;
+            const int rcs = dense_fwd(cs, l, 0, 96 + down_in(l) + kGrowth * j, tb.up_bn[i][j], tb.up_conv[i][j], nullptr, nullptr, nullptr, kSkipPart);
+            if (rcs) return rcs;
+        }
+        ENDO_CHECK(hipEventRecord(net->ev_skip[l], net->wstream));
+        return 0;
+    };
+    const int held = (overlap == 3 && deepest > 0 && deepest + 1 < kLevels) ? deepest + 1 : -1;
     for (int l = 0; l < kLevels; ++l) {
         for (int j = 0; j < kLayers; ++j) {
             rc = dense_fwd(c, l, 48, 48 + down_in(l) + kGrowth * j, tb.down_bn[l][j], tb.down_conv[l][j]);
@@ -1263,6 +1353,19 @@
         }
         rc = td_fwd(c, l, tb.td_bn[l], tb.td_conv[l]);
         if (rc) return rc;
+        if (overlap == 2) {
+            if (split[l]) { rc = fork_side(); if (rc) return rc; rc = skip_parts(l); if (rc) return rc; }
+        } else if (l == deepest) {
+            rc = fork_side();
+            if (rc) return rc;
+            for (int ll = deepest; ll >= (held >= 0 ? 1 : 0); --ll)
+                if (split[ll]) { rc = skip_parts(ll); if (rc) return rc; }
+        } else if (l == held && split[0]) {
+            rc = fork_side();
+            if (rc) return rc;
+            rc = skip_parts(0);
+            if (rc) return rc;
+        }
     }
     for (int j = 0; j < kLayers; ++j) {
         rc = dense_fwd(c, kLevels, 0, 288 + kGrowth * j, tb.bott_bn[j], tb.bott_conv[j]);
@@ -1274,10 +1377,11 @@
         const int src_c0 = (i == 0) ? 288 : 96 + down_in(src);
         rc = tu_fwd(c, l, src, src_c0, tb.tu_conv[i]);
         if (rc) return rc;
+        if (split[l]) ENDO_CHECK(hipStreamWaitEvent(c.stream, net->ev_skip[l], 0));
         for (int j = 0; j < kLayers; ++j) {
             const bool last = l == 0 && j == kLayers - 1;
             rc = dense_fwd(c, l, 0, 96 + down_in(l) + kGrowth * j, tb.up_bn[i][j], tb.up_conv[i][j], last ? params + tb.final_.w : nullptr,
-                           last ? tape + net->pre_off : nullptr, last ? &fused_final : nullptr);
+                           last ? tape + net->pre_off : nullptr, last ? &fused_final : nullptr, (split[l] && !last) ? kRestPart : kWhole);
             if (rc) return rc;
         }
     }
@@ -1302,10 +1406,9 @@
     Ctx c{net, params, nullptr, const_cast<float*>(tape), grads, gradws, training, static_cast<hipStream_t>(stream_)};
     BiasParts bias_parts{};
     c.bias_parts = &bias_parts;
-    if (!net->wstream) {
-        ENDO_CHECK(hipStreamCreateWithFlags(&net->wstream, hipStreamNonBlocking));
-        ENDO_CHECK(hipEventCreateWithFlags(&net->ev_fork, hipEventDisableTiming));
-        ENDO_CHECK(hipEventCreateWithFlags(&net->ev_join, hipEventDisableTiming));
+    {
+        const int rc_side = ensure_side_stream(net);
+        if (rc_side) return rc_side;
     }
     for (int g = 0; g < net->groups; ++g)
         ENDO_CHECK(hipMemsetAsync(gradws + g * net->gs + net->pq_off, 0,
diff --git a/endoscopydepthestimation-pytorch_amd/csrc/wino4_fwd_kernels.h b/endoscopydepthestimation-pytorch_amd/csrc/wino4_fwd_kernels.h
--- a/endoscopydepthestimation-pytorch_amd/csrc/wino4_fwd_kernels.h
+++ b/endoscopydepthestimation-pytorch_amd/csrc/wino4_fwd_kernels.h
@@ -98,8 +98,9 @@
     t[5] = f34_fma<T>(kW4P, d1, f34_fma<T>(-kW4S, d3, d5));
 }
 
-template <bool FIN = false>
+template <bool FIN = false, bool SEG = false>
 __global__ void __launch_bounds__(kConvThreads, 2) wino4_fwd_kernel(const ConvParams p0) {
+    static_assert(!(FIN && SEG), "the last dense layer runs whole");
     using G = Wino4Geom;
     extern __shared__ __attribute__((aligned(16))) float smem[];
     float* s_aux = smem + 2 * G::kBuf;
@@ -121,7 +122,7 @@
 
     for (int c = tid; c < p.cin; c += kConvThreads) {
         float scale, mean, beta;
-        bn_input_constants(p, p0, grp, groups, first_of_group, c, scale, mean, beta);
+        bn_input_constants(p, p0, grp, groups, first_of_group, (SEG && c >= p.k_seg) ? c + p.k_jump : c, scale, mean, beta);
         s_aux[c] = scale;
         s_aux[cap + c] = mean;
         s_aux[2 * cap + c] = beta;
@@ -135,8 +136,9 @@
 #pragma unroll
     for (int xi = 0; xi < 36; ++xi) acc[xi] = f32x4{0.f, 0.f, 0.f, 0.f};
 
-    const __amdgpu_buffer_rsrc_t xr = f34_rsrc(p.in + n * p.in_ns, p.cin * p.in_cs * 4);
-    const __amdgpu_buffer_rsrc_t ur = f34_rsrc(p.wgt, p.cin * kW4UStride * 4);
+    const int planes = SEG ? p.cin + p.k_jump : p.cin;
+    const __amdgpu_buffer_rsrc_t xr = f34_rsrc(p.in + n * p.in_ns, planes * p.in_cs * 4);
+    const __amdgpu_buffer_rsrc_t ur = f34_rsrc(p.wgt, planes * kW4UStride * 4);
     unsigned x_vo[G::kXRounds];
 #pragma unroll
     for (int k = 0; k < G::kXRounds; ++k) {
@@ -156,8 +158,9 @@
 
     auto issue_dma = [&](int chunk, int buf) {
         float* s_stage = smem + buf * G::kBuf + wave * 256;
-        const unsigned xs = 4u * static_cast<unsigned>(chunk * G::kKC * p.in_cs);
-        const unsigned us = 4u * static_cast<unsigned>(chunk * G::kKC * kW4UStride);
+        const int c0 = chunk * G::kKC + ((SEG && chunk * G::kKC >= p.k_seg) ? p.k_jump : 0);
+        const unsigned xs = 4u * static_cast<unsigned>(c0 * p.in_cs);
+        const unsigned us = 4u * static_cast<unsigned>(c0 * kW4UStride);
 #pragma unroll
         for (int k = 0; k < G::kXRounds; ++k) {
             const int e0 = k * kConvThreads + wave * 64;
@@ -297,9 +300,14 @@
         for (int a = 0; a < 4; ++a) {
             float o[4];
             w4_at(c4[a][0], c4[a][1], c4[a][2], c4[a][3], c4[a][4], c4[a][5], o);
-            const f32x4 v = {o[0] + bias, o[1] + bias, o[2] + bias, o[3] + bias};
+            f32x4 v = {o[0] + bias, o[1] + bias, o[2] + bias, o[3] + bias};
             if (co_ok && px < p.w && y + a < p.h) {
-                *reinterpret_cast<f32x4*>(p.out + n * p.out_ns + static_cast<int64_t>(co) * p.out_cs + static_cast<int64_t>(y + a) * p.out_w + px) = v;
+                float* dst = p.out + n * p.out_ns + static_cast<int64_t>(co) * p.out_cs + static_cast<int64_t>(y + a) * p.out_w + px;
+                if constexpr (SEG) {
+                    const f32x4 prev = *reinterpret_cast<const f32x4*>(dst);
+                    v = f32x4{o[0] + prev[0] + bias, o[1] + prev[1] + bias, o[2] + prev[2] + bias, o[3] + prev[3] + bias};
+                }
+                *reinterpret_cast<f32x4*>(dst) = v;
 #pragma unroll
                 for (int k = 0; k < 4; ++k) { s1 += v[k]; s2 += v[k] * v[k]; }
             }
@@ -328,15 +336,16 @@
     return wino_fwd_ok(p) && (p.h % 4 == 0) && static_cast<int64_t>(p.cin) * p.in_cs * 4 < (1ll << 31);
 }
 
-template <bool FIN>
+template <bool FIN, bool SEG = false>
 inline int launch_wino4_fwd_t(ConvParams p, hipStream_t stream) {
     using G = Wino4Geom;
     p.tiles_x = (p.w + G::kTileX - 1) / G::kTileX;
     p.bn_cap = (p.cin + 15) / 16 * 16;
     const int tiles_y = (p.h + G::kTileY - 1) / G::kTileY;
-    return launch_dyn(wino4_fwd_kernel<FIN>, dim3(p.tiles_x * tiles_y, 1, p.n), kConvThreads, G::bytes(p.bn_cap), stream, p);
+    return launch_dyn(wino4_fwd_kernel<FIN, SEG>, dim3(p.tiles_x * tiles_y, 1, p.n), kConvThreads, G::bytes(p.bn_cap), stream, p);
 }
 inline int launch_wino4_fwd(const ConvParams& p, hipStream_t stream) {
+    if (p.k_jump > 0 || p.acc_out) return p.fin_w ? ENDO_E_BADARG : launch_wino4_fwd_t<false, true>(p, stream);
     return p.fin_w ? launch_wino4_fwd_t<true>(p, stream) : launch_wino4_fwd_t<false>(p, stream);
 }
 
diff --git a/endoscopydepthestimation-pytorch_amd/csrc/wino_fwd_kernels.h b/endoscopydepthestimation-pytorch_amd/csrc/wino_fwd_kernels.h
--- a/endoscopydepthestimation-pytorch_amd/csrc/wino_fwd_kernels.h
+++ b/endoscopydepthestimation-pytorch_amd/csrc/wino_fwd_kernels.h
@@ -92,7 +92,7 @@
     static size_t bytes(int bn_cap) { return sizeof(float) * (NS * kBuf + 3 * bn_cap + kTail); }
 };
 
-template <int R, int KC, int MINW, int NS, int EXP = 0>
+template <int R, int KC, int MINW, int NS, int EXP = 0, bool SEG = false>
 __global__ void __launch_bounds__(kConvThreads, MINW) wino_fwd_kernel(const ConvParams p0) {
     using G = WinoFwdGeom<R, KC, NS>;
     typedef float f32x2 __attribute__((ext_vector_type(2)));
@@ -116,7 +116,7 @@
 
     for (int c = tid; c < p.cin; c += kConvThreads) {
         float scale, mean, beta;
-        bn_input_constants(p, p0, grp, groups, first_of_group, c, scale, mean, beta);
+        bn_input_constants(p, p0, grp, groups, first_of_group, (SEG && c >= p.k_seg) ? c + p.k_jump : c, scale, mean, beta);
         s_aux[c] = scale;
         s_aux[cap + c] = mean;
         s_aux[2 * cap + c] = beta;
@@ -158,6 +158,7 @@
     }
     const int nchunks = p.cin / KC;
 
+    int seg_left = SEG ? p.k_seg / KC : 0;
     auto issue_dma = [&](int buf) {
         float* s_stage = smem + buf * G::kBuf + wave * 256;
 #pragma unroll
@@ -170,6 +171,13 @@
                     __builtin_amdgcn_global_load_lds((gptr_t)d_ptr[k], (lptr_t)(s_stage + k * 4 * kConvThreads), 16, 0, 0);
             }
             d_ptr[k] = reinterpret_cast<const float*>(reinterpret_cast<const char*>(d_ptr[k]) + d_stride[k]);
+        }
+        if constexpr (SEG) {
+            if (--seg_left == 0) {
+#pragma unroll
+                for (int k = 0; k < G::kDma; ++k)
+                    d_ptr[k] = reinterpret_cast<const float*>(reinterpret_cast<const char*>(d_ptr[k]) + static_cast<size_t>(d_stride[k] / KC) * p.k_jump);
+            }
         }
     };
 
@@ -282,6 +290,10 @@
             for (int half = 0; half < 2; ++half) {
                 if (px + 4 * half + 3 < p.w) {
                     float* dst = p.out + n * p.out_ns + static_cast<int64_t>(co) * p.out_cs + static_cast<int64_t>(y) * p.out_w + px + 4 * half;
+                    if constexpr (SEG) {
+                        if (y < p.h) row0[half] += *reinterpret_cast<const f32x4*>(dst);
+                        if (y + 1 < p.h) row1[half] += *reinterpret_cast<const f32x4*>(dst + p.out_w);
+                    }
                     if (y < p.h) {
                         *reinterpret_cast<f32x4*>(dst) = row0[half];
 #pragma unroll
@@ -322,14 +334,14 @@
            p.cin % 4 == 0 && p.cin >= 8;
 }
 
-template <int R, int KC, int MINW, int NS, int EXP = 0>
+template <int R, int KC, int MINW, int NS, int EXP = 0, bool SEG = false>
 inline int launch_wino_fwd(ConvParams p, hipStream_t stream) {
     using G = WinoFwdGeom<R, KC, NS>;
     p.tiles_x = (p.w + G::kTileX - 1) / G::kTileX;
     p.bn_cap = ((p.cin + KC - 1) / KC * KC + 15) / 16 * 16;
     const int tiles_y = (p.h + G::kTileY - 1) / G::kTileY;
-    return launch_dyn(wino_fwd_kernel<R, KC, MINW, NS, EXP>, dim3(p.tiles_x * tiles_y, 1, p.n), kConvThreads, G::bytes(p.bn_cap), stream, p);
-}
-
-
-}
+    return launch_dyn(wino_fwd_kernel<R, KC, MINW, NS, EXP, SEG>, dim3(p.tiles_x * tiles_y, 1, p.n), kConvThreads, G::bytes(p.bn_cap), stream, p);
+}
+
+
+}
diff --git a/endoscopydepthestimation-pytorch_amd/models.py b/endoscopydepthestimation-pytorch_amd/models.py
--- a/endoscopydepthestimation-pytorch_amd/models.py
+++ b/endoscopydepthestimation-pytorch_amd/models.py
@@ -256,7 +256,7 @@
             self._handles[key] = (hnd, int(lib.endo_net_tape_floats(hnd)), int(lib.endo_net_gradws_floats(hnd)))
         return self._handles[key]
 
-    _OPTION_DEFAULTS = {0: 5, 1: 3, 2: 2, 3: 1024, 4: 0, 5: 1, 6: 0, 7: 1, 8: 1, 9: 3}
+    _OPTION_DEFAULTS = {0: 5, 1: 3, 2: 2, 3: 1024, 4: 0, 5: 1, 6: 0, 7: 1, 8: 1, 9: 3, 10: 1}
 
     def set_kernel_option(self, option_id, value):
         option_id, value = int(option_id), int(value)
diff --git a/include/endo_hip.h b/include/endo_hip.h
--- a/include/endo_hip.h
+++ b/include/endo_hip.h
@@ -104,7 +104,8 @@
 #define ENDO_OPT_WGRAD_F34 7
 #define ENDO_OPT_FINAL_VIRTUAL 8
 #define ENDO_OPT_TD_PERSIST 9
-#define ENDO_OPT_COUNT 10
+#define ENDO_OPT_FWD_SKIP_OVERLAP 10
+#define ENDO_OPT_COUNT 11
 int endo_net_set_option(endo_net* net, int option_id, int value);
 int endo_net_get_option(const endo_net* net, int option_id);
 int64_t endo_net_group_stride(const endo_net* net);
```

Result: faster. 522.8 (median of 6 runs) (+1.5%).
